# jeffersonfparil/poolgen

Hardware: NVIDIA B200
Metric: loci/sec for ols_iter (f64) (higher is better)
Workload: dtype f64

## Files before the change

poolgen_b200/csrc/pg_api.cu:

```cuda
#include <math.h>
#include <stdarg.h>
#include <stdio.h>
#include <stdlib.h>
#include <string.h>

#include <algorithm>
#include <new>

#include "pg_internal.h"
#include "pg_ptable.h"

namespace pg {
cudaError_t launch_scan_a2(const ScanParams &, int, cudaStream_t);
cudaError_t launch_scan_a3(const ScanParams &, int, cudaStream_t);
cudaError_t launch_scan_a4(const ScanParams &, int, cudaStream_t);
cudaError_t launch_scan_a5(const ScanParams &, int, cudaStream_t);
cudaError_t launch_scan_a6(const ScanParams &, int, cudaStream_t);

cudaError_t launch_scan(const ScanParams &p, int sm_count, cudaStream_t s) {
    switch (p.lay.A) {
        case 2: return launch_scan_a2(p, sm_count, s);
        case 3: return launch_scan_a3(p, sm_count, s);
        case 4: return launch_scan_a4(p, sm_count, s);
        case 5: return launch_scan_a5(p, sm_count, s);
// ... 163 lines not shown
    s->lay = pg::make_layout(n_pools, s->A_dev);
    s->n_slots = regression ? s->A_dev - 1 : 1;
    double S = 0.0;
    for (int i = 0; i < n_pools; i++) S = S + filter->pool_sizes[i];
    s->w_host.assign(s->lay.n_pad, 0.0);
    for (int i = 0; i < n_pools; i++) s->w_host[i] = filter->pool_sizes[i] / S;
    s->weighted = 0;
    for (int i = 1; i < n_pools; i++)
        if (s->w_host[i] != s->w_host[0]) s->weighted = 1;
    s->w_uniform = s->w_host[0];

    if (regression) {
        const int n = n_pools, np = s->lay.n_pad;
        s->yc_host.assign((size_t)k * np, 0.0);
        s->ysum.assign(k, 0.0);
        s->syy.assign(k, 0.0);
        s->ymean.assign(k, 0.0);
        for (int j = 0; j < k; j++) {
            double sum = 0.0;
            int n_valid = 0;
            for (int i = 0; i < n; i++) {
                const double v = phen[(size_t)i * k + j];
                if (v != v) {
                    s->y_has_nan = 1;
                    continue;
                }
                sum += v;
                n_valid++;
            }
            const double mean = n_valid ? sum / n_valid : 0.0;
            double s1 = 0.0, s2 = 0.0;
            for (int i = 0; i < n; i++) {
                const double c = phen[(size_t)i * k + j] - mean;
                s->yc_host[(size_t)j * np + i] = c;
                s1 += c;
                s2 += c * c;
            }
            s->ysum[j] = s1;
            s->ymean[j] = mean;
            s->syy[j] = s2 - s1 * s1 / n;
        }
        if (s->y_has_nan && (kind == PG_KIND_OLS || kind == PG_KIND_MLE)) {
            delete s;
            return fail(ctx, PG_ERR_UNSUPPORTED,
                        "pg_scan_open: missing phenotype values (the reference's ols_iter panics on them, "
                        "src/base/sync.rs:254-257)");
        }
        s->df = (kind != PG_KIND_CORR) ? (double)n - 1.0 : (double)n - 2.0;
        if (kind != PG_KIND_CORR && !(s->df > 0.0)) {
            delete s;
            return fail(ctx, PG_ERR_UNSUPPORTED, "pg_scan_open: ols_iter needs at least 2 pools");
        }
        s->ln_beta = s->df > 0.0 ? pg::statrs::ln_gamma(s->df / 2.0 + 0.5) - pg::statrs::ln_gamma(s->df / 2.0) - pg::statrs::ln_gamma(0.5) : 0.0;
        if ((size_t)2 * np * 8 > 96 * 1024) {
            delete s;
            return fail(ctx, PG_ERR_UNSUPPORTED, "pg_scan_open: %d pools exceed the shared-memory resident phenotype budget (6,144 pools)", n);
        }
        const char *pv_mode = getenv("PG_PVALUE");
        if (s->df > 0.0 && !(pv_mode && strcmp(pv_mode, "cf") == 0)) {
            pg::PTable tab = pg::build_ptable(s->df);
            if (tab.max_err < 2e-9) {
                cudaError_t et = s->d_ptab.reserve(tab.coef.size(), nullptr);
                if (et == cudaSuccess)
                    et = cudaMemcpy(s->d_ptab.get(), tab.coef.data(), tab.coef.size() * 8, cudaMemcpyHostToDevice);
                if (et != cudaSuccess) {
                    delete s;
                    return fail(ctx, PG_ERR_CUDA, "pg_scan_open: p-value table upload: %s", cudaGetErrorString(et));
                }
                s->ptab_M = tab.M;
                s->ptab_isd = tab.inv_sqrt_df;
                s->ptab_bits = tab.bits;
                s->ptab_t1 = tab.t_one;
                s->ptab_t0 = tab.t_zero;
                s->ptab_err = tab.max_err;
            }
        }
        cudaError_t e = s->d_yc.reserve(s->yc_host.size(), nullptr);
        if (e == cudaSuccess) e = cudaMemcpy(s->d_yc.get(), s->yc_host.data(), s->yc_host.size() * 8, cudaMemcpyHostToDevice);
        if (e != cudaSuccess) {
            delete s;
            return fail(ctx, PG_ERR_CUDA, "pg_scan_open: phenotype upload: %s", cudaGetErrorString(e));
        }
    }
    {
        cudaError_t e = s->d_w.reserve(s->w_host.size(), nullptr);
        if (e == cudaSuccess) e = cudaMemcpy(s->d_w.get(), s->w_host.data(), s->w_host.size() * 8, cudaMemcpyHostToDevice);
        if (e != cudaSuccess) {
            delete s;
            return fail(ctx, PG_ERR_CUDA, "pg_scan_open: weight upload: %s", cudaGetErrorString(e));
        }
    }
    if (kind == PG_KIND_MLE || gwalpha) {
        const int np = s->lay.n_pad;
        std::vector<double> raw((size_t)(gwalpha ? 2 : k) * np, 0.0);
        if (gwalpha) {
            for (int i = 0; i < n_pools; i++) {
                raw[i] = gw_bins[i];
                raw[(size_t)np + i] = gw_q[i];
            }
            s->gw_sig = gw_fmt[0 * 3 + 2];
            s->gw_min = gw_fmt[1 * 3 + 2];
            s->gw_max = gw_fmt[2 * 3 + 2];
            (void)gw_rows;
        } else {
            for (int j = 0; j < k; j++)
                for (int i = 0; i < n_pools; i++) raw[(size_t)j * np + i] = phen[(size_t)i * k + j];
        }
        cudaError_t e = s->d_yraw.reserve(raw.size(), nullptr);
        if (e == cudaSuccess) e = cudaMemcpy(s->d_yraw.get(), raw.data(), raw.size() * 8, cudaMemcpyHostToDevice);
        if (e != cudaSuccess) {
            delete s;
            return fail(ctx, PG_ERR_CUDA, "pg_scan_open: phenotype upload: %s", cudaGetErrorString(e));
        }
    }
    {
        cudaError_t e = cudaDeviceSynchronize();
        if (e != cudaSuccess) {
            delete s;
            return fail(ctx, PG_ERR_CUDA, "pg_scan_open: %s", cudaGetErrorString(e));
        }
    }
    *out = s;
    return PG_OK;
}

int pg_scan_close(pg_scan *s) {
    delete s;
    return PG_OK;
}

static bool is_nm(const pg_scan *s) { return s->kind == PG_KIND_MLE || s->kind == PG_KIND_GWALPHA_LS || s->kind == PG_KIND_GWALPHA_ML; }
static bool is_regression(const pg_scan *s) { return s->kind == PG_KIND_OLS || s->kind == PG_KIND_CORR || is_nm(s); }

int pg_batch_create(pg_scan *s, int64_t cap, pg_batch **out) {
    if (!s || !out || cap < 1 || cap > 0x7FFFFFFFLL) return fail(s ? s->ctx : nullptr, PG_ERR_ARG, "pg_batch_create: bad argument (1 <= capacity < 2^31 loci)");
    pg_ctx *ctx = s->ctx;
    *out = nullptr;
    PG_CUDA(ctx, cudaSetDevice(ctx->device));
    pg_batch *b = new (std::nothrow) pg_batch();
    if (!b) return fail(ctx, PG_ERR_ARG, "out of host memory");
    b->scan = s;
    b->cap = cap;
    cudaError_t e = cudaStreamCreateWithFlags(&b->stream, cudaStreamNonBlocking);
    if (e == cudaSuccess) e = cudaEventCreate(&b->ev0);
    if (e == cudaSuccess) e = cudaEventCreate(&b->ev1);
    if (e == cudaSuccess && is_regression(s)) {
        e = b->d_freq.reserve((size_t)cap * s->lay.freq_stride(), b->stream);
        if (e == cudaSuccess) e = b->d_depth.reserve((size_t)cap * s->lay.depth_stride(), b->stream);
        if (e == cudaSuccess) e = b->d_dmin.reserve((size_t)cap, b->stream);
        if (e == cudaSuccess) e = b->d_defer.reserve((size_t)cap + 1, b->stream);
        if (e == cudaSuccess) e = b->d_hint.reserve((size_t)cap, b->stream);
    }
    const size_t S = s->n_slots, K = s->k;
    if (e == cudaSuccess) e = b->d_meta.reserve((size_t)cap, b->stream);
    if (e == cudaSuccess) e = b->d_fmean.reserve((size_t)cap * S, b->stream);
    if (e == cudaSuccess) e = b->d_stats.reserve((size_t)cap * S * K * 4, b->stream);
    if (e != cudaSuccess) {
        delete b;
        return fail(ctx, PG_ERR_CUDA, "pg_batch_create(%lld loci): %s", (long long)cap, cudaGetErrorString(e));
    }
    *out = b;
    return PG_OK;
}

int pg_batch_destroy(pg_batch *b) {
    delete b;
    return PG_OK;
}

static pg::IngestOut ingest_out(pg_batch *b, int64_t first_locus) {
    pg_scan *s = b->scan;
    pg::IngestOut o;
    o.freq = b->d_freq.get() + (size_t)first_locus * s->lay.freq_stride();
    o.depth = b->d_depth.get() + (size_t)first_locus * s->lay.depth_stride();
    o.dmin = b->d_dmin.get() + first_locus;
    o.hint = b->d_hint.get() + first_locus;
    o.w = s->d_w.get();
    o.maf = s->maf;
    o.one_minus_maf = 1.00 - s->maf;
    o.min_depth_f = (double)s->min_depth;
    return o;
}

}

static int ensure_stage(pg_batch *b, size_t bytes) {
    PG_CUDA(b->scan->ctx, b->d_stage.reserve(bytes, b->stream));
    return PG_OK;
}

template <typename CT>
static int upload_counts_t(pg_batch *b, const CT *counts, int64_t n_loci) {
    if (!b || (!counts && n_loci > 0)) return PG_ERR_ARG;
    pg_scan *s = b->scan;
    pg_ctx *ctx = s->ctx;
    if (n_loci < 0 || n_loci > b->cap) return fail(ctx, PG_ERR_ARG, "upload: %lld loci > capacity %lld", (long long)n_loci, (long long)b->cap);
    PG_CUDA(ctx, cudaSetDevice(ctx->device));
    b->n_loci = n_loci;
    b->have_input = 1;
    if (n_loci == 0) return PG_OK;
    const size_t bytes = (size_t)n_loci * s->A_in * s->n * sizeof(CT);
    const bool reg = is_regression(s);
    const size_t wide_bytes = (size_t)b->cap * s->A_in * s->n * 4;
    int rc = ensure_stage(b, reg ? (size_t)b->cap * s->A_in * s->n * sizeof(CT) : wide_bytes + (sizeof(CT) == 4 ? 0 : bytes));
    if (rc) return rc;
    if (reg) {
        PG_CUDA(ctx, cudaMemcpyAsync(b->d_stage.get(), counts, bytes, cudaMemcpyHostToDevice, b->stream));
        if constexpr (sizeof(CT) == 4)
            PG_CUDA(ctx, pg::launch_ingest_u32((const uint32_t *)b->d_stage.get(), n_loci, s->n, s->A_in, s->drop_col, s->lay,
                                               ingest_out(b, 0), b->stream));
        else if constexpr (sizeof(CT) == 1)
            PG_CUDA(ctx, pg::launch_ingest_u8((const uint8_t *)b->d_stage.get(), n_loci, s->n, s->A_in, s->drop_col, s->lay,
                                              ingest_out(b, 0), b->stream));
        else
            PG_CUDA(ctx, pg::launch_ingest_u16((const uint16_t *)b->d_stage.get(), n_loci, s->n, s->A_in, s->drop_col, s->lay,
                                               ingest_out(b, 0), b->stream));
    } else if constexpr (sizeof(CT) == 4) {
        PG_CUDA(ctx, cudaMemcpyAsync(b->d_stage.get(), counts, bytes, cudaMemcpyHostToDevice, b->stream));
    } else {
        void *narrow = (char *)b->d_stage.get() + wide_bytes;
        PG_CUDA(ctx, cudaMemcpyAsync(narrow, counts, bytes, cudaMemcpyHostToDevice, b->stream));
        PG_CUDA(ctx, pg::launch_widen(narrow, (int)sizeof(CT), (uint32_t *)b->d_stage.get(), (size_t)n_loci * s->A_in * s->n,
                                      b->stream));
    }
    b->input_is_counts = 1;
    return PG_OK;
}

extern "C" {

int pg_batch_upload_counts(pg_batch *b, const uint32_t *counts, int64_t n_loci) {
    return upload_counts_t<uint32_t>(b, counts, n_loci);
}
int pg_batch_upload_counts_u16(pg_batch *b, const uint16_t *counts, int64_t n_loci) {
    return upload_counts_t<uint16_t>(b, counts, n_loci);
}
int pg_batch_upload_counts_u8(pg_batch *b, const uint8_t *counts, int64_t n_loci) {
    return upload_counts_t<uint8_t>(b, counts, n_loci);
}

int pg_batch_upload_freq(pg_batch *b, const double *freq, const uint32_t *depth, int64_t n_loci) {
    if (!b || ((!freq || !depth) && n_loci > 0)) return PG_ERR_ARG;
    pg_scan *s = b->scan;
    pg_ctx *ctx = s->ctx;
    if (!is_regression(s)) return fail(ctx, PG_ERR_UNSUPPORTED, "upload_freq: the table tests need counts");
    if (s->drop_col >= 0)
        return fail(ctx, PG_ERR_ARG, "upload_freq: the frequency matrix must not contain the N column when remove_ns is set");
    if (n_loci < 0 || n_loci > b->cap) return fail(ctx, PG_ERR_ARG, "upload: %lld loci > capacity %lld", (long long)n_loci, (long long)b->cap);
    PG_CUDA(ctx, cudaSetDevice(ctx->device));
    b->n_loci = n_loci;
    b->have_input = 1;
    if (n_loci == 0) return PG_OK;
    const size_t fbytes_cap = (size_t)b->cap * s->A_dev * s->n * 8, dbytes_cap = (size_t)b->cap * s->n * 4;
    int rc = ensure_stage(b, fbytes_cap + dbytes_cap);
    if (rc) return rc;
    double *sf = (double *)b->d_stage.get();
    uint32_t *sd = (uint32_t *)((char *)b->d_stage.get() + fbytes_cap);
    PG_CUDA(ctx, cudaMemcpyAsync(sf, freq, (size_t)n_loci * s->A_dev * s->n * 8, cudaMemcpyHostToDevice, b->stream));
    PG_CUDA(ctx, cudaMemcpyAsync(sd, depth, (size_t)n_loci * s->n * 4, cudaMemcpyHostToDevice, b->stream));
    PG_CUDA(ctx, pg::launch_ingest_freq(sf, sd, n_loci, s->n, s->lay, ingest_out(b, 0), b->stream));
    b->input_is_counts = 0;
    return PG_OK;
}

static int text_stage_a(pg_batch *b, const char *text, size_t n_bytes, size_t line_cap) {
    if (!b || (!text && n_bytes > 0)) return PG_ERR_ARG;
    pg_scan *s = b->scan;
    pg_ctx *ctx = s->ctx;
    if (s->A_in != 6) return fail(ctx, PG_ERR_ARG, "upload_sync_text: the scan must be opened with the six sync columns A:T:C:G:N:D");
    for (int j = 0; j < 6; j++)
        if (s->codes_in[j] != j) return fail(ctx, PG_ERR_ARG, "upload_sync_text: allele codes must be 0..5 in sync order");
    PG_CUDA(ctx, cudaSetDevice(ctx->device));
    b->n_loci = 0;
    b->have_input = 1;
    b->input_is_counts = 1;
    b->text_src = text;
    b->text_bytes = n_bytes;
    int rc = ensure_stage(b, (size_t)b->cap * 6 * s->n * 4);
    if (rc) return rc;
    const cudaError_t pe = pg::text_parse_async(&b->text, text, n_bytes, s->n, (uint32_t *)b->d_stage.get(), b->cap, line_cap,
                                                ctx->sm_count, b->stream);
    if (pe != cudaSuccess) {
        b->have_input = 0;
        b->n_loci = 0;
        return fail(ctx, PG_ERR_CUDA, "upload_sync_text: %s", cudaGetErrorString(pe));
    }
    return PG_OK;
}

static int text_stage_b(pg_batch *b, int64_t *n_loci_out) {
    pg_scan *s = b->scan;
    pg_ctx *ctx = s->ctx;
    if (n_loci_out) *n_loci_out = 0;
    cudaError_t ce = cudaSuccess;
    uint64_t at = 0;
    int64_t L = pg::text_parse_finish(&b->text, b->stream, &ce, &at);
    if (L == -5) {
        int rc = text_stage_a(b, b->text_src, b->text_bytes, (size_t)at + 1);
        if (rc) return rc;
        L = pg::text_parse_finish(&b->text, b->stream, &ce, &at);
    }
    if (L < 0) return pg::text_parse_fail(ctx, "upload_sync_text", L, ce, at, s->n, b->cap);
    b->n_loci = L;
    if (n_loci_out) *n_loci_out = L;
    if (L > 0 && is_regression(s))
        PG_CUDA(ctx, pg::launch_ingest_u32((const uint32_t *)b->d_stage.get(), L, s->n, s->A_in, s->drop_col, s->lay,
                                           ingest_out(b, 0), b->stream));
    return PG_OK;
}

int pg_batch_upload_sync_text(pg_batch *b, const char *text, size_t n_bytes, int64_t *n_loci_out) {
    if (n_loci_out) *n_loci_out = 0;
    int rc = text_stage_a(b, text, n_bytes, 0);
    if (rc) return rc;
    rc = text_stage_b(b, n_loci_out);
    if (rc) return rc;
    PG_CUDA(b->scan->ctx, cudaStreamSynchronize(b->stream));
    return PG_OK;
}

int pg_batch_text_labels(pg_batch *b, const uint64_t **line_offsets, const uint64_t **positions) {
    if (!b) return PG_ERR_ARG;
    if (!b->text.parsed) return fail(b->scan->ctx, PG_ERR_STATE, "pg_batch_text_labels before pg_batch_upload_sync_text");
    if (line_offsets) *line_offsets = b->text.h_out_offset.get();
    if (positions) *positions = b->text.h_out_pos.get();
    return PG_OK;
}

int pg_batch_synth(pg_batch *b, uint64_t seed, int64_t first_locus, int64_t n_loci) {
    if (!b) return PG_ERR_ARG;
    pg_scan *s = b->scan;
    pg_ctx *ctx = s->ctx;
    if (n_loci < 0 || n_loci > b->cap) return fail(ctx, PG_ERR_ARG, "synth: %lld loci > capacity %lld", (long long)n_loci, (long long)b->cap);
    PG_CUDA(ctx, cudaSetDevice(ctx->device));
    b->n_loci = n_loci;
    b->have_input = 1;
    if (n_loci == 0) return PG_OK;
    const size_t per_locus = (size_t)s->A_in * s->n * 4;
    if (!is_regression(s)) {
        int rc = ensure_stage(b, (size_t)b->cap * per_locus);
        if (rc) return rc;
        PG_CUDA(ctx, pg::launch_synth(seed, first_locus, n_loci, s->n, s->A_in, (uint32_t *)b->d_stage.get(), b->stream));
        b->input_is_counts = 1;
        return PG_OK;
    }
    int64_t slice = (int64_t)((size_t)256 << 20) / (int64_t)per_locus;
    if (slice < 1) slice = 1;
    if (slice > n_loci) slice = n_loci;
    if (b->d_stage.capacity() < (size_t)slice * per_locus) {
        int rc = ensure_stage(b, (size_t)slice * per_locus);
        if (rc) return rc;
    } else {
        slice = (int64_t)(b->d_stage.capacity() / per_locus);
        if (slice > n_loci) slice = n_loci;
    }
    for (int64_t l0 = 0; l0 < n_loci; l0 += slice) {
        const int64_t m = (n_loci - l0 < slice) ? n_loci - l0 : slice;
        PG_CUDA(ctx, pg::launch_synth(seed, first_locus + l0, m, s->n, s->A_in, (uint32_t *)b->d_stage.get(), b->stream));
        PG_CUDA(ctx, pg::launch_ingest_u32((const uint32_t *)b->d_stage.get(), m, s->n, s->A_in, s->drop_col, s->lay,
                                           ingest_out(b, l0), b->stream));
    }
    b->input_is_counts = 1;
    return PG_OK;
}

static int run_once(pg_batch *b, int *launches) {
    pg_scan *s = b->scan;
    pg_ctx *ctx = s->ctx;
    if (!b->have_input) return fail(ctx, PG_ERR_STATE, "pg_batch_run: no input uploaded");
    if (b->n_loci == 0) return PG_OK;
    if (is_regression(s)) {
        int kpass = pg::max_phen_per_pass(s->A_dev);
        {
            const int fit = (int)((size_t)(96 * 1024) / ((size_t)s->lay.n_pad * 8)) - (s->weighted ? 1 : 0);
            if (kpass > fit) kpass = fit < 1 ? 1 : fit;
        }
        static const int nbuf_env = getenv("PG_NBUF") ? atoi(getenv("PG_NBUF")) : 0;
        static const int warps_env = getenv("PG_WARPS") ? atoi(getenv("PG_WARPS")) : 0;
        static const int g_env = getenv("PG_G") ? atoi(getenv("PG_G")) : 0;
        static const int p_env = getenv("PG_P") ? atoi(getenv("PG_P")) : 0;
        if (is_nm(s)) kpass = 1;
        for (int base = 0; base < (is_nm(s) ? 1 : s->k); base += kpass) {
            pg::ScanParams p;
            memset(&p, 0, sizeof p);
            p.lay = s->lay;
            p.freq = b->d_freq.get();
            p.depth = b->d_depth.get();
            p.dmin = b->d_dmin.get();
            p.hint = b->d_hint.get();
            p.n_loci = b->n_loci;
            p.kind = is_nm(s) ? PG_KIND_OLS : s->kind;
            p.filter_only = is_nm(s) ? 1 : 0;
            p.weighted = s->weighted;
            p.maf = s->maf;
            p.one_minus_maf = 1.00 - s->maf;
            p.max_miss = s->max_miss;
            p.min_depth_f = (double)s->min_depth;
            p.w_uniform = s->w_uniform;
            p.df = s->df;
            p.inv_df = 1.0 / s->df;
            p.inv_n = 1.0 / (double)s->n;
            p.inv_nm2 = 1.0 / ((double)s->n - 2.0);
            p.ln_beta = s->ln_beta;
            p.ptab = s->d_ptab.get();
            p.ptab_isd = s->ptab_isd;
            p.ptab_bits = s->ptab_bits;
            p.ptab_t1 = s->ptab_t1;
            p.ptab_t0 = s->ptab_t0;
            p.ptab_M = s->ptab_M;
            p.K = std::min(kpass, s->k - base);
            p.y_has_nan = s->y_has_nan;
            p.yc = s->d_yc.get() + (size_t)base * s->lay.n_pad;
            p.w = s->d_w.get();
            for (int j = 0; j < p.K; j++) {
                p.ysum[j] = s->ysum[base + j];
                p.syy[j] = s->syy[base + j];
                p.ymean[j] = s->ymean[base + j];
            }
            for (int j = 0; j < s->A_dev; j++) p.codes[j] = s->codes_dev[j];
            p.meta = b->d_meta.get();
            p.freq_mean = b->d_fmean.get();
            p.stats = b->d_stats.get();
            p.defer_list = b->d_defer.get();
            p.defer_count = reinterpret_cast<uint32_t *>(b->d_defer.get() + b->cap);
            p.k_total = s->k;
            p.phen_base = base;
            p.write_meta = base == 0;
            p.nbuf_override = nbuf_env;
            p.warps_override = warps_env;
            p.g_override = g_env;
            p.p_override = p_env;
            PG_CUDA(ctx, pg::launch_scan(p, ctx->sm_count, b->stream));
            if (launches) (*launches) += 2;
        }
        if (is_nm(s)) {
            pg::NmParams q;
            memset(&q, 0, sizeof q);
            q.lay = s->lay;
            q.freq = b->d_freq.get();
            q.depth = b->d_depth.get();
            q.n_loci = b->n_loci;
            q.kind = s->kind;
            q.k = s->k;
            q.yraw = s->d_yraw.get();
            q.gw_sig = s->gw_sig;
            q.gw_min = s->gw_min;
            q.gw_max = s->gw_max;
            q.df = s->df;
            q.ln_beta = s->ln_beta;
            q.ptab = s->d_ptab.get();
            q.ptab_isd = s->ptab_isd;
            q.ptab_bits = s->ptab_bits;
            q.ptab_t1 = s->ptab_t1;
            q.ptab_t0 = s->ptab_t0;
            q.ptab_M = s->ptab_M;
            for (int j = 0; j < s->A_dev; j++) q.codes[j] = s->codes_dev[j];
            q.meta = b->d_meta.get();
            q.stats = b->d_stats.get();
            PG_CUDA(ctx, pg::launch_nm(q, ctx->sm_count, b->stream));
            if (launches) (*launches)++;
        }
    } else {
        pg::TableParams p;
        memset(&p, 0, sizeof p);
        p.counts = (const uint32_t *)b->d_stage.get();
        p.n_loci = b->n_loci;
        p.n = s->n;
        p.A_in = s->A_in;
        p.kind = s->kind;
        p.drop_col = s->drop_col;
        p.maf = s->maf;
        p.one_minus_maf = 1.00 - s->maf;
        p.max_miss = s->max_miss;
        p.min_depth_f = (double)s->min_depth;
        p.w = s->d_w.get();
        for (int j = 0; j < s->A_in; j++) p.codes[j] = s->codes_in[j];
        p.meta = b->d_meta.get();
        p.stats = b->d_stats.get();
        PG_CUDA(ctx, pg::launch_tables(p, ctx->sm_count, b->stream));
        if (launches) (*launches)++;
    }
    return PG_OK;
}

int pg_batch_run(pg_batch *b) {
    if (!b) return PG_ERR_ARG;
    PG_CUDA(b->scan->ctx, cudaSetDevice(b->scan->ctx->device));
    return run_once(b, nullptr);
}

int pg_batch_time_runs(pg_batch *b, int iters, float *ms_total, int *n_launches) {
    if (!b || iters < 1 || !ms_total) return PG_ERR_ARG;
    pg_ctx *ctx = b->scan->ctx;
    PG_CUDA(ctx, cudaSetDevice(ctx->device));
    int launches = 0;
    PG_CUDA(ctx, cudaStreamSynchronize(b->stream));
    PG_CUDA(ctx, cudaEventRecord(b->ev0, b->stream));
    for (int i = 0; i < iters; i++) {
        int rc = run_once(b, &launches);
        if (rc) return rc;
    }
    PG_CUDA(ctx, cudaEventRecord(b->ev1, b->stream));
    PG_CUDA(ctx, cudaEventSynchronize(b->ev1));
    PG_CUDA(ctx, cudaEventElapsedTime(ms_total, b->ev0, b->ev1));
    if (n_launches) *n_launches = launches;
    static const bool report = getenv("PG_REPORT_DEFER") != nullptr;
    if (report && b->d_defer.get() && is_regression(b->scan)) {
        uint32_t count = 0;
        PG_CUDA(ctx, cudaMemcpy(&count, b->d_defer.get() + b->cap, 4, cudaMemcpyDeviceToHost));
        std::vector<uint64_t> list(count);
        if (count) PG_CUDA(ctx, cudaMemcpy(list.data(), b->d_defer.get(), (size_t)count * 8, cudaMemcpyDeviceToHost));
        uint32_t h[8] = {0, 0, 0, 0, 0, 0, 0, 0};
        for (uint64_t e : list) {
            const unsigned why = (unsigned)(e >> 56);
            if (why & 1u) h[0]++;
            if (why & 2u) h[1]++;
            if (why & 4u) h[2]++;
            if (why & 8u) h[3]++;
            if ((why >> 4) >= 1 && (why >> 4) <= 4) h[3 + (why >> 4)]++;
        }
        fprintf(stderr, "[pg] deferred %u of %lld loci (last phenotype pass): threshold %u, removed-with-reads %u, no coverage %u, "
                        "NaN under hint %u, redo ols %u, redo corr %u, corr NaN %u, tie %u\n",
                count, (long long)b->n_loci, h[0], h[1], h[2], h[3], h[4], h[5], h[6], h[7]);
    }
    return PG_OK;
}

int pg_batch_bytes(pg_batch *b, size_t *input_bytes, size_t *result_bytes) {
    if (!b) return PG_ERR_ARG;
    pg_scan *s = b->scan;
    const size_t L = (size_t)b->n_loci;
    if (input_bytes)
        *input_bytes = is_regression(s) ? L * (s->lay.freq_stride() * 8 + 4)
                                        : L * (size_t)s->A_in * s->n * 4;
    if (result_bytes) *result_bytes = L * (8 + (size_t)s->n_slots * 8 + (size_t)s->n_slots * s->k * 32);
    return PG_OK;
}

int pg_batch_download(pg_batch *b) {
    if (!b) return PG_ERR_ARG;
    pg_scan *s = b->scan;
    pg_ctx *ctx = s->ctx;
    PG_CUDA(ctx, cudaSetDevice(ctx->device));
    const size_t S = s->n_slots, K = s->k;
    PG_CUDA(ctx, b->h_meta.reserve((size_t)b->cap, b->stream));
    PG_CUDA(ctx, b->h_fmean.reserve((size_t)b->cap * S, b->stream));
    PG_CUDA(ctx, b->h_stats.reserve((size_t)b->cap * S * K * 4, b->stream));
    const size_t L = (size_t)b->n_loci;
    if (L == 0) return PG_OK;
    PG_CUDA(ctx, cudaMemcpyAsync(b->h_meta.get(), b->d_meta.get(), L * 8, cudaMemcpyDeviceToHost, b->stream));
    PG_CUDA(ctx, cudaMemcpyAsync(b->h_fmean.get(), b->d_fmean.get(), L * S * 8, cudaMemcpyDeviceToHost, b->stream));
    PG_CUDA(ctx, cudaMemcpyAsync(b->h_stats.get(), b->d_stats.get(), L * S * K * 32, cudaMemcpyDeviceToHost, b->stream));
    return PG_OK;
}

int pg_batch_sync(pg_batch *b) {
    if (!b) return PG_ERR_ARG;
    PG_CUDA(b->scan->ctx, cudaStreamSynchronize(b->stream));
    return PG_OK;
}

int pg_batch_results(pg_batch *b, pg_results *out) {
    if (!b || !out) return PG_ERR_ARG;
    if (b->n_loci > 0 && !(b->h_meta.get() && b->h_fmean.get() && b->h_stats.get())) return fail(b->scan->ctx, PG_ERR_STATE, "pg_batch_results before pg_batch_download");
    out->n_loci = b->n_loci;
    out->n_slots = b->scan->n_slots;
    out->n_phen = b->scan->k;
    out->meta = b->h_meta.get();
    out->freq_mean = b->h_fmean.get();
    out->stats = b->h_stats.get();
    return PG_OK;
}

int pg_scan_stream_begin(pg_scan *s, int64_t max_loci) {
    if (!s || max_loci < 1) return PG_ERR_ARG;
    for (int i = 0; i < PG_STREAM_DEPTH; i++) {
        delete s->slabs[i];
        s->slabs[i] = nullptr;
        int rc = pg_batch_create(s, max_loci, &s->slabs[i]);
        if (rc) return rc;
    }
    s->slab_cap = max_loci;
    s->next_slab = 0;
    return PG_OK;
}

static int submit_common(pg_scan *s, int *ticket, pg_batch **b) {
    if (!s || !ticket) return PG_ERR_ARG;
    if (!s->slabs[0]) return fail(s->ctx, PG_ERR_STATE, "pg_scan_submit before pg_scan_stream_begin");
    *ticket = s->next_slab;
    *b = s->slabs[s->next_slab];
    s->next_slab = (s->next_slab + 1) % PG_STREAM_DEPTH;
    return pg_batch_sync(*b);
}

int pg_scan_submit_counts(pg_scan *s, const uint32_t *counts, int64_t n_loci, int *ticket) {
    pg_batch *b = nullptr;
    int rc = submit_common(s, ticket, &b);
    if (rc) return rc;
    if ((rc = pg_batch_upload_counts(b, counts, n_loci))) return rc;
    if ((rc = pg_batch_run(b))) return rc;
    return pg_batch_download(b);
}
int pg_scan_submit_counts_u16(pg_scan *s, const uint16_t *counts, int64_t n_loci, int *ticket) {
    pg_batch *b = nullptr;
    int rc = submit_common(s, ticket, &b);
    if (rc) return rc;
    if ((rc = pg_batch_upload_counts_u16(b, counts, n_loci))) return rc;
    if ((rc = pg_batch_run(b))) return rc;
    return pg_batch_download(b);
}
int pg_scan_submit_counts_u8(pg_scan *s, const uint8_t *counts, int64_t n_loci, int *ticket) {
    pg_batch *b = nullptr;
    int rc = submit_common(s, ticket, &b);
    if (rc) return rc;
    if ((rc = pg_batch_upload_counts_u8(b, counts, n_loci))) return rc;
// ... 46 lines not shown
```

poolgen_b200/csrc/pg_device.cuh:

```cuda
#pragma once
#include <cuda_runtime.h>
#include <stdint.h>

namespace pg {

#define PG_FULL_MASK 0xffffffffu
constexpr double kEps = 2.220446049250313e-16;

__device__ __forceinline__ uint32_t smem_u32(const void *p) {
    return (uint32_t)__cvta_generic_to_shared(p);
}

__device__ __forceinline__ void mbar_init(uint64_t *bar, uint32_t count) {
    asm volatile("mbarrier.init.shared::cta.b64 [%0], %1;" ::"r"(smem_u32(bar)), "r"(count) : "memory");
}
__device__ __forceinline__ void fence_mbar_init() {
    asm volatile("fence.mbarrier_init.release.cluster;" ::: "memory");
}
__device__ __forceinline__ void fence_proxy_async() {
    asm volatile("fence.proxy.async.shared::cta;" ::: "memory");
}
__device__ __forceinline__ void mbar_expect_tx(uint64_t *bar, uint32_t bytes) {
    asm volatile("mbarrier.arrive.expect_tx.shared::cta.b64 _, [%0], %1;" ::"r"(smem_u32(bar)), "r"(bytes)
                 : "memory");
}
__device__ __forceinline__ void bulk_g2s(void *dst_smem, const void *src_gmem, uint32_t bytes, uint64_t *bar) {
    asm volatile(
        "cp.async.bulk.shared::cluster.global.mbarrier::complete_tx::bytes [%0], [%1], %2, [%3];" ::"r"(
            smem_u32(dst_smem)),
        "l"(src_gmem), "r"(bytes), "r"(smem_u32(bar))
        : "memory");
}
__device__ __forceinline__ void mbar_wait(uint64_t *bar, uint32_t parity) {
    asm volatile(
        "{\n"
        ".reg .pred P1;\n"
        "LAB_WAIT:\n"
        "mbarrier.try_wait.parity.shared::cta.b64 P1, [%0], %1;\n"
        "@P1 bra DONE;\n"
        "bra LAB_WAIT;\n"
        "DONE:\n"
        "}\n" ::"r"(smem_u32(bar)),
        "r"(parity)
        : "memory");
}

__device__ __forceinline__ void warp_reduce32(double (&v)[32], int lane) {
#pragma unroll
    for (int off = 16; off >= 1; off >>= 1) {
        const bool upper = (lane & off) != 0;
#pragma unroll
        for (int i = 0; i < off; i++) {
            const double a = v[i], b = v[i + off];
            const double send = upper ? a : b;
            const double keep = upper ? b : a;
            v[i] = keep + __shfl_xor_sync(PG_FULL_MASK, send, off);
        }
    }
}

__device__ __forceinline__ double warp_sum_fixed(double v) {
#pragma unroll
    for (int off = 16; off >= 1; off >>= 1) v += __shfl_xor_sync(PG_FULL_MASK, v, off);
    return v;
}

__device__ __forceinline__ double beta_reg_dev(double a, double b, double x, double ln_beta) {
    double bt;
    if (fabs(x) < 1e-10 || fabs(x - 1.0) <= 4.0 * 1.1102230246251565e-16) {
        bt = 0.0;
    } else {
        bt = exp(ln_beta + a * log(x) + b * log(1.0 - x));
    }
    const bool symm = x >= (a + 1.0) / (a + b + 2.0);
    const double eps = 1.1102230246251565e-16;
    const double fpmin = 2.2250738585072014e-308 / eps;
    if (symm) {
        const double sw = a;
        x = 1.0 - x;
        a = b;
        b = sw;
    }
    const double qab = a + b, qap = a + 1.0, qam = a - 1.0;
    double c = 1.0;
    double d = 1.0 - qab * x / qap;
    if (fabs(d) < fpmin) d = fpmin;
    d = 1.0 / d;
    double h = d;
    for (int mi = 1; mi < 141; mi++) {
        const double m = (double)mi;
        const double m2 = m * 2.0;
        double aa = m * (b - m) * x / ((qam + m2) * (a + m2));
        d = 1.0 + aa * d;
        if (fabs(d) < fpmin) d = fpmin;
        c = 1.0 + aa / c;
        if (fabs(c) < fpmin) c = fpmin;
        d = 1.0 / d;
        h = h * d * c;
        aa = -(a + m) * (qab + m) * x / ((a + m2) * (qap + m2));
        d = 1.0 + aa * d;
        if (fabs(d) < fpmin) d = fpmin;
        c = 1.0 + aa / c;
        if (fabs(c) < fpmin) c = fpmin;
        d = 1.0 / d;
        const double del = d * c;
        h *= del;
        if (fabs(del - 1.0) <= eps) break;
    }
    return symm ? 1.0 - bt * h / a : bt * h / a;
}

static __device__ __noinline__ double student_two_sided(double t_abs, double df, double ln_beta) {
    if (isinf(df)) return 2.0 * (1.0 - 0.5 * erfc(-t_abs / sqrt(2.0)));
    const double h = df / __dadd_rn(df, __dmul_rn(t_abs, t_abs));
    const double ib = 0.5 * beta_reg_dev(df / 2.0, 0.5, h, ln_beta);
    const double cdf = t_abs <= 0.0 ? ib : 1.0 - ib;
    return 2.0 * (1.0 - cdf);
}

struct PTableDev {
    const double4 *coef;
    double inv_sqrt_df, bits;
    double t_one, t_zero;
    int M;
};
__device__ __forceinline__ int ptab_locate(double w, int B, double &s) {
    const int hi = __double2hiint(w);
// ... 92 lines not shown
```

poolgen_b200/csrc/pg_ingest.cu:

```cuda
#include <stdlib.h>

#include "pg_device.cuh"
#include "pg_internal.h"

namespace pg {

struct HintParams {
    double maf, one_minus_maf, min_depth_f;
    int enabled;
};
__device__ __forceinline__ unsigned ambiguous_alleles(const double *q, int A, int n, const HintParams &hp) {
    const double tol_rel = 4.0 * ((double)n + 8.0) * kEps;
    unsigned amb = 0;
    for (int j = 0; j < A; j++) {
        const double tl = tol_rel * fmax(fabs(q[j]), 1.0);
        if (fabs(q[j] - hp.maf) <= tl || fabs(q[j] - hp.one_minus_maf) <= tl) amb |= 1u << j;
    }
    return amb;
}

__device__ __forceinline__ uint8_t locus_hint(const double *q, int A, int n, uint32_t dm, const HintParams &hp,
                                              unsigned exact) {
    if (!hp.enabled) return 0;
    const double tol_rel = 4.0 * ((double)n + 8.0) * kEps;
    unsigned kept = 0;
    bool removed_with_reads = false, safe = true;
    for (int j = 0; j < A; j++) {
        const double tl = tol_rel * fmax(fabs(q[j]), 1.0);
        if (!((exact >> j) & 1u) && (fabs(q[j] - hp.maf) <= tl || fabs(q[j] - hp.one_minus_maf) <= tl)) safe = false;
        if (!((q[j] < hp.maf) | (q[j] > hp.one_minus_maf)))
            kept |= 1u << j;
        else if (q[j] > 0.0)
            removed_with_reads = true;
    }
    const bool depth_ok = dm != 0u && !((double)dm < hp.min_depth_f);
    return (safe && depth_ok && removed_with_reads && __popc(kept) >= 2) ? (uint8_t)(0x80u | kept) : (uint8_t)0;
}

template <typename RowFn>
__device__ __forceinline__ void ingest_loci(int64_t n_loci, const Layout &lay, int P, const double *freq,
                                            const double *__restrict__ w, uint32_t *__restrict__ dmin,
                                            uint8_t *__restrict__ hint, const HintParams &hp, RowFn &&row) {
    const int lane = threadIdx.x & 31, sub = lane / P, q0 = lane % P, lpw = 32 / P;
    const int64_t gw = ((int64_t)blockIdx.x * blockDim.x + threadIdx.x) >> 5;
    const int64_t nw = ((int64_t)gridDim.x * blockDim.x) >> 5;
    for (int64_t l0 = gw * lpw; l0 < n_loci; l0 += nw * lpw) {
        const int64_t locus = l0 + sub;
        double q[PG_MAX_ALLELES] = {0, 0, 0, 0, 0, 0};
        uint32_t dm = 0xFFFFFFFFu;
        if (locus < n_loci)
            for (int i = q0; i < lay.n_pad; i += P) row(locus, i, q, dm);
        for (int off = P >> 1; off >= 1; off >>= 1) {
            for (int j = 0; j < lay.A; j++) q[j] += __shfl_xor_sync(0xFFFFFFFFu, q[j], off);
            dm = min(dm, __shfl_xor_sync(0xFFFFFFFFu, dm, off));
        }
        unsigned amb = (hp.enabled && locus < n_loci && dm != 0u) ? ambiguous_alleles(q, lay.A, lay.n, hp) : 0u;
        if (__any_sync(0xFFFFFFFFu, amb != 0u)) {
            __syncwarp();
            const double *fl = freq + (size_t)(locus < n_loci ? locus : 0) * lay.freq_stride();
            for (int j = 0; j < lay.A; j++) {
                if (!__any_sync(0xFFFFFFFFu, (amb >> j) & 1u)) continue;
                double e = 0.0;
                for (int r0 = 0; r0 < lay.n; r0 += P) {
                    const int i = r0 + q0;
                    double term = 0.0;
                    if (i < lay.n && locus < n_loci) {
                        const double f = __ldcg(fl + lay.freq_off(i, j));
                        term = (f != f) ? 0.0 : __dmul_rn(f, w[i]);
                    }
                    const int m = min(P, lay.n - r0);
                    for (int t = 0; t < m; t++) e = __dadd_rn(e, __shfl_sync(0xFFFFFFFFu, term, t, P));
                }
                if ((amb >> j) & 1u) q[j] = e;
            }
        }
        if (locus < n_loci && q0 == 0) {
            dmin[locus] = dm;
            hint[locus] = locus_hint(q, lay.A, lay.n, dm, hp, amb);
        }
    }
}

template <typename CT>
__global__ void __launch_bounds__(256) ingest_counts_kernel(const CT *__restrict__ counts, int64_t n_loci, int n,
                                                            int A_in, int drop_col, Layout lay, int P,
                                                            double *__restrict__ freq, uint32_t *__restrict__ depth,
                                                            uint32_t *__restrict__ dmin, uint8_t *__restrict__ hint,
                                                            const double *__restrict__ w, HintParams hp) {
    ingest_loci(n_loci, lay, P, freq, w, dmin, hint, hp, [&](int64_t locus, int i, double *q, uint32_t &dm) {
        double *fl = freq + (size_t)locus * lay.freq_stride();
        if (i >= n) {
            for (int j = 0; j < lay.A; j++) fl[lay.freq_off(i, j)] = 0.0;
            depth[(size_t)locus * lay.n_pad + i] = 0xFFFFFFFFu;
            return;
        }
        const CT *cl = counts + (size_t)locus * A_in * n + i;
        uint32_t c[PG_MAX_ALLELES];
        uint64_t d = 0;
        int jj = 0;
        for (int j = 0; j < A_in; j++) {
            if (j == drop_col) continue;
            c[jj] = (uint32_t)cl[(size_t)j * n];
            d += c[jj];
            jj++;
        }
        if (d > 0xFFFFFFFEull) d = 0xFFFFFFFEull;
        const double dd = (double)d, wi = w[i];
        const double rd = __drcp_rn(dd);
        for (int j = 0; j < lay.A; j++) {
            const double cj = (double)c[j];
            const double q0 = __dmul_rn(cj, rd);
            const double f = (d == 0) ? nan("") : __fma_rn(__fma_rn(-q0, dd, cj), rd, q0);
            fl[lay.freq_off(i, j)] = f;
            if (d != 0) q[j] = fma(f, wi, q[j]);
        }
        depth[(size_t)locus * lay.n_pad + i] = (uint32_t)d;
        dm = min(dm, (uint32_t)d);
    });
}

__global__ void __launch_bounds__(256) ingest_freq_kernel(const double *__restrict__ fin, const uint32_t *__restrict__ din,
                                                          int64_t n_loci, int n, Layout lay, int P,
                                                          double *__restrict__ freq, uint32_t *__restrict__ depth,
                                                          uint32_t *__restrict__ dmin, uint8_t *__restrict__ hint,
                                                          const double *__restrict__ w, HintParams hp) {
    ingest_loci(n_loci, lay, P, freq, w, dmin, hint, hp, [&](int64_t locus, int i, double *q, uint32_t &dm) {
        double *fl = freq + (size_t)locus * lay.freq_stride();
        const bool pad = i >= n;
        for (int j = 0; j < lay.A; j++) {
            const double f = pad ? 0.0 : fin[((size_t)locus * lay.A + j) * n + i];
            fl[lay.freq_off(i, j)] = f;
            if (!pad && f == f) q[j] = fma(f, w[i], q[j]);
        }
        const uint32_t d = pad ? 0xFFFFFFFFu : din[(size_t)locus * n + i];
        depth[(size_t)locus * lay.n_pad + i] = d;
        dm = min(dm, d);
    });
}

__global__ void __launch_bounds__(256) synth_kernel(uint64_t seed, int64_t first_locus, int64_t n_loci, int n,
                                                    int A_in, uint32_t *__restrict__ counts) {
    const int64_t total = n_loci * n;
    for (int64_t idx = (int64_t)blockIdx.x * blockDim.x + threadIdx.x; idx < total;
         idx += (int64_t)gridDim.x * blockDim.x) {
        const int64_t l = idx / n;
        const int i = (int)(idx - l * n);
        uint32_t c[PG_MAX_ALLELES];
        synth_counts(seed, first_locus + l, i, A_in, c);
        for (int a = 0; a < A_in; a++) counts[((size_t)l * A_in + a) * n + i] = c[a];
    }
}

static int grid_for(int64_t total) {
    int64_t b = (total + 255) / 256;
    const int64_t cap = 148 * 16;
    return (int)(b < 1 ? 1 : (b > cap ? cap : b));
}

static int ingest_group(const Layout &lay) {
    int P = 32;
    while (P > 1 && (P >> 1) >= lay.n_pad) P >>= 1;
    return P;
}
static HintParams hint_params(const IngestOut &o) {
    static const bool no_hint = getenv("PG_NOHINT") != nullptr;
    HintParams hp;
    hp.maf = o.maf;
    hp.one_minus_maf = o.one_minus_maf;
    hp.min_depth_f = o.min_depth_f;
    hp.enabled = no_hint ? 0 : 1;
    return hp;
}
template <typename CT>
static cudaError_t launch_ingest_t(const CT *counts, int64_t n_loci, int n, int A_in, int drop_col, const Layout &lay,
                                   const IngestOut &o, cudaStream_t s) {
    if (n_loci <= 0) return cudaSuccess;
    const int P = ingest_group(lay);
    ingest_counts_kernel<CT><<<grid_for(n_loci * P), 256, 0, s>>>(counts, n_loci, n, A_in, drop_col, lay, P, o.freq,
                                                                 o.depth, o.dmin, o.hint, o.w, hint_params(o));
    return cudaGetLastError();
}
cudaError_t launch_ingest_u32(const uint32_t *counts, int64_t n_loci, int n, int A_in, int drop_col, const Layout &lay,
                              const IngestOut &o, cudaStream_t s) {
    return launch_ingest_t<uint32_t>(counts, n_loci, n, A_in, drop_col, lay, o, s);
}
cudaError_t launch_ingest_u16(const uint16_t *counts, int64_t n_loci, int n, int A_in, int drop_col, const Layout &lay,
                              const IngestOut &o, cudaStream_t s) {
    return launch_ingest_t<uint16_t>(counts, n_loci, n, A_in, drop_col, lay, o, s);
}
cudaError_t launch_ingest_u8(const uint8_t *counts, int64_t n_loci, int n, int A_in, int drop_col, const Layout &lay,
                             const IngestOut &o, cudaStream_t s) {
    return launch_ingest_t<uint8_t>(counts, n_loci, n, A_in, drop_col, lay, o, s);
}
cudaError_t launch_ingest_freq(const double *fin, const uint32_t *din, int64_t n_loci, int n, const Layout &lay,
                               const IngestOut &o, cudaStream_t s) {
    if (n_loci <= 0) return cudaSuccess;
    const int P = ingest_group(lay);
    ingest_freq_kernel<<<grid_for(n_loci * P), 256, 0, s>>>(fin, din, n_loci, n, lay, P, o.freq, o.depth, o.dmin, o.hint,
                                                            o.w, hint_params(o));
    return cudaGetLastError();
}
template <typename CT>
__global__ void __launch_bounds__(256) widen_kernel(const CT *__restrict__ src, uint32_t *__restrict__ dst, size_t count) {
    for (size_t i = (size_t)blockIdx.x * blockDim.x + threadIdx.x; i < count; i += (size_t)gridDim.x * blockDim.x)
        dst[i] = (uint32_t)src[i];
}
cudaError_t launch_widen(const void *src, int elem_bytes, uint32_t *dst, size_t count, cudaStream_t s) {
    if (count == 0) return cudaSuccess;
    if (elem_bytes == 1)
        widen_kernel<uint8_t><<<grid_for((int64_t)count), 256, 0, s>>>((const uint8_t *)src, dst, count);
    else if (elem_bytes == 2)
        widen_kernel<uint16_t><<<grid_for((int64_t)count), 256, 0, s>>>((const uint16_t *)src, dst, count);
    else
        return cudaErrorInvalidValue;
    return cudaGetLastError();
}
cudaError_t launch_synth(uint64_t seed, int64_t first_locus, int64_t n_loci, int n, int A_in, uint32_t *counts,
                         cudaStream_t s) {
    if (n_loci <= 0) return cudaSuccess;
    synth_kernel<<<grid_for(n_loci * n), 256, 0, s>>>(seed, first_locus, n_loci, n, A_in, counts);
    return cudaGetLastError();
}

}
```

poolgen_b200/csrc/pg_internal.h:

```cpp
#pragma once
#include <cuda_runtime.h>
#include <stdint.h>
#include <string>
#include <utility>
#include <vector>

#include "poolgen_cuda.h"
#include "pg_synth.h"

namespace pg {

__host__ __device__ constexpr int chunk_rows(int A) { return A <= 2 ? 256 : (A == 3 ? 192 : 128); }

struct Layout {
    int n;
    int n_pad;
    int A;
    int rc;
    int n_chunks;
    int rc_last;
    __host__ __device__ size_t freq_stride() const { return (size_t)A * n_pad; }
    __host__ __device__ size_t depth_stride() const { return (size_t)n_pad; }
    __host__ __device__ size_t freq_off(int i, int j) const {
        int c = i / rc, r = i - c * rc;
        int rcc = (c == n_chunks - 1) ? rc_last : rc;
        return (size_t)c * A * rc + (size_t)j * rcc + r;
    }
};

inline Layout make_layout(int n, int A) {
    Layout l;
    l.n = n;
    l.n_pad = (n + 3) & ~3;
    l.A = A;
    const int cr = chunk_rows(A);
    if (l.n_pad <= cr) {
        l.rc = l.n_pad;
        l.n_chunks = 1;
        l.rc_last = l.n_pad;
    } else {
        l.rc = cr;
        l.n_chunks = (l.n_pad + cr - 1) / cr;
        l.rc_last = l.n_pad - (l.n_chunks - 1) * cr;
    }
    return l;
}

constexpr int kMaxPhenPerPass = 4;
inline int max_phen_per_pass(int A) { return A <= 4 ? 4 : (A == 5 ? 3 : 2); }

struct ScanParams {
    Layout lay;
    const double *freq;
    const uint32_t *depth;
    const uint32_t *dmin;
    const uint8_t *hint;
    int64_t n_loci;
    int kind;
    int weighted;
    double maf, one_minus_maf, max_miss;
    double min_depth_f;
    double w_uniform;
    double df;
    double inv_df;
    double inv_n, inv_nm2;
    double ln_beta;
    const void *ptab;
    double ptab_isd, ptab_bits, ptab_t1, ptab_t0;
    int ptab_M;
    const double *yc;
    const double *w;
    double ysum[kMaxPhenPerPass];
    double syy[kMaxPhenPerPass];
    double ymean[kMaxPhenPerPass];
    int y_has_nan;
    int filter_only;
    uint8_t codes[8];
    uint64_t *meta;
    double *freq_mean;
    double *stats;
    uint64_t *defer_list;
    uint32_t *defer_count;
    int k_total, phen_base, K;
    int write_meta;
    uint32_t common_bytes, warp_bytes, stage_bytes;
    int nbuf, block_loci;
    int nbuf_override, warps_override, g_override, p_override;
};

struct TableParams {
    const uint32_t *counts;
    int64_t n_loci;
    int n, A_in;
    int kind;
    int drop_col;
    double maf, one_minus_maf, max_miss, min_depth_f;
    const double *w;
    uint8_t codes[8];
    uint64_t *meta;
    double *stats;
};

struct NmParams {
    Layout lay;
    const double *freq;
    const uint32_t *depth;
    int64_t n_loci;
    int kind;
    int k;
    const double *yraw;
    double gw_sig, gw_min, gw_max;
    double df, ln_beta;
    const void *ptab;
    double ptab_isd, ptab_bits, ptab_t1, ptab_t0;
    int ptab_M;
    uint8_t codes[8];
    uint64_t *meta;
    double *stats;
};
cudaError_t launch_nm(const NmParams &p, int sm_count, cudaStream_t s);

constexpr int kKinMleMaxM = 13;
struct KinMleParams {
    const double *G;
    int64_t P;
    int n, ldg, m, k;
    const double *Z;
    const double *fix;
    double df, ln_beta;
    const void *ptab;
    double ptab_isd, ptab_bits, ptab_t1, ptab_t0;
    int ptab_M;
    double *beta, *var, *pval;
};
cudaError_t launch_kin_mle(const KinMleParams &p, int sm_count, cudaStream_t s);

cudaError_t launch_scan(const ScanParams &p, int sm_count, cudaStream_t s);
cudaError_t launch_tables(const TableParams &p, int sm_count, cudaStream_t s);
struct IngestOut {
    double *freq;
    uint32_t *depth;
    uint32_t *dmin;
    uint8_t *hint;
    const double *w;
    double maf, one_minus_maf, min_depth_f;
};
cudaError_t launch_ingest_u32(const uint32_t *counts, int64_t n_loci, int n, int A_in, int drop_col, const Layout &lay,
                              const IngestOut &o, cudaStream_t s);
cudaError_t launch_ingest_u16(const uint16_t *counts, int64_t n_loci, int n, int A_in, int drop_col, const Layout &lay,
                              const IngestOut &o, cudaStream_t s);
cudaError_t launch_ingest_u8(const uint8_t *counts, int64_t n_loci, int n, int A_in, int drop_col, const Layout &lay,
                             const IngestOut &o, cudaStream_t s);
cudaError_t launch_ingest_freq(const double *freq_in, const uint32_t *depth_in, int64_t n_loci, int n, const Layout &lay,
                               const IngestOut &o, cudaStream_t s);
cudaError_t launch_synth(uint64_t seed, int64_t first_locus, int64_t n_loci, int n, int A_in,
                         uint32_t *counts, cudaStream_t s);
cudaError_t launch_widen(const void *src, int elem_bytes, uint32_t *dst, size_t count, cudaStream_t s);

template <typename T, bool Pinned>
class Buffer {
  public:
    Buffer() = default;
    Buffer(const Buffer &) = delete;
    Buffer &operator=(const Buffer &) = delete;
    Buffer(Buffer &&o) noexcept : p_(o.p_), cap_(o.cap_) { o.p_ = nullptr, o.cap_ = 0; }
    Buffer &operator=(Buffer &&o) noexcept {
        std::swap(p_, o.p_);
        std::swap(cap_, o.cap_);
        return *this;
    }
    ~Buffer() { release(); }

    cudaError_t reserve(size_t count, cudaStream_t stream) {
        if (cap_ >= count) return cudaSuccess;
        cudaError_t e = p_ ? cudaStreamSynchronize(stream) : cudaSuccess;
        release();
        if (e != cudaSuccess) return e;
        void *q = nullptr;
        if constexpr (Pinned)
            e = cudaHostAlloc(&q, count * sizeof(T), cudaHostAllocDefault);
        else
            e = cudaMalloc(&q, count * sizeof(T));
        if (e != cudaSuccess) {
            (void)cudaGetLastError();
            return e;
        }
        p_ = static_cast<T *>(q);
        cap_ = count;
        return cudaSuccess;
    }
    T *get() const { return p_; }
    size_t capacity() const { return cap_; }

  private:
    void release() {
        if constexpr (Pinned) {
            if (p_) cudaFreeHost(p_);
        } else {
            cudaFree(p_);
        }
        p_ = nullptr;
        cap_ = 0;
    }
    T *p_ = nullptr;
    size_t cap_ = 0;
};
template <typename T>
using DeviceBuffer = Buffer<T, false>;
template <typename T>
using PinnedBuffer = Buffer<T, true>;

struct TextScratch {
    DeviceBuffer<char> d_text;
    DeviceBuffer<uint32_t> d_sep;
    DeviceBuffer<uint64_t> d_tok_blk;
    DeviceBuffer<uint32_t> d_nl, d_first, d_grp;
    DeviceBuffer<uint8_t> d_keep;
    DeviceBuffer<uint64_t> d_line_pos;
    DeviceBuffer<uint32_t> d_info;
    PinnedBuffer<uint32_t> h_info;
    DeviceBuffer<uint8_t> d_tmp;
    DeviceBuffer<uint64_t> d_out_offset, d_out_pos;
    PinnedBuffer<uint64_t> h_out_offset, h_out_pos;
    cudaEvent_t parsed = nullptr;
    bool pending = false;
    int64_t max_loci = 0;
    ~TextScratch();
};
cudaError_t text_parse_async(TextScratch *t, const char *text, size_t n_bytes, int n_pools, uint32_t *d_counts,
                             int64_t max_loci, size_t line_cap, int sm_count, cudaStream_t s);
int64_t text_parse_finish(TextScratch *t, cudaStream_t s, cudaError_t *cuda_err, uint64_t *err_offset);

}

struct pg_ctx {
    int device = 0;
    int sm_count = 0;
    int cc_major = 0, cc_minor = 0;
    size_t total_mem = 0;
};

namespace pg {
int fail(pg_ctx *ctx, int code, const char *fmt, ...);
int text_parse_fail(pg_ctx *ctx, const char *who, int64_t status, cudaError_t cuda_err, uint64_t err_offset,
                    int n_pools, int64_t cap);
}

#define PG_CUDA(ctx, call)                                                                              \
    do {                                                                                                \
        cudaError_t e_ = (call);                                                                        \
        if (e_ != cudaSuccess)                                                                          \
            return pg::fail((ctx), PG_ERR_CUDA, "%s failed: %s (%s:%d)", #call, cudaGetErrorString(e_), \
                            __FILE__, __LINE__);                                                        \
    } while (0)

struct pg_scan {
    pg_ctx *ctx = nullptr;
    int kind = 0;
    int n = 0, A_in = 0, A_dev = 0, k = 0;
    int drop_col = -1;
    uint8_t codes_in[8] = {0};
    uint8_t codes_dev[8] = {0};
    pg::Layout lay;
    int remove_ns = 1;
    uint64_t min_depth = 1;
    double maf = 0, max_miss = 0;
    int weighted = 0;
    double w_uniform = 0;
    std::vector<double> w_host;
    std::vector<double> yc_host;
    std::vector<double> ysum, syy, ymean;
    int y_has_nan = 0;
    double df = 0, ln_beta = 0;
    pg::DeviceBuffer<double> d_yc;
    pg::DeviceBuffer<double> d_w;
    pg::DeviceBuffer<double> d_yraw;
    double gw_sig = 0, gw_min = 0, gw_max = 0;
    pg::DeviceBuffer<double> d_ptab;
    double ptab_isd = 0, ptab_bits = 0, ptab_err = 0, ptab_t1 = 0, ptab_t0 = 0;
    int ptab_M = 0;
    int n_slots = 0;
    pg_batch *slabs[PG_STREAM_DEPTH] = {nullptr, nullptr, nullptr};
    int next_slab = 0;
    int64_t slab_cap = 0;
    ~pg_scan();
};

struct pg_batch {
    pg_scan *scan = nullptr;
    int64_t cap = 0, n_loci = 0;
    cudaStream_t stream = nullptr;
    cudaEvent_t ev0 = nullptr, ev1 = nullptr;
    pg::DeviceBuffer<double> d_freq;
    pg::DeviceBuffer<uint32_t> d_depth;
    pg::DeviceBuffer<uint32_t> d_dmin;
    pg::DeviceBuffer<uint64_t> d_defer;
    pg::DeviceBuffer<uint8_t> d_hint;
    pg::DeviceBuffer<uint8_t> d_stage;
    pg::DeviceBuffer<uint64_t> d_meta;
    pg::DeviceBuffer<double> d_fmean;
    pg::DeviceBuffer<double> d_stats;
    pg::PinnedBuffer<uint64_t> h_meta;
    pg::PinnedBuffer<double> h_fmean;
    pg::PinnedBuffer<double> h_stats;
    int have_input = 0;
    int input_is_counts = 0;
    pg::TextScratch text;
    const char *text_src = nullptr;
    size_t text_bytes = 0;
    ~pg_batch();
};
```

poolgen_b200/csrc/pg_nm.cu:

```cuda
#include "pg_device.cuh"
#include "pg_internal.h"

namespace pg {

constexpr int kNmMaxD = 8;

__device__ __forceinline__ double bound_logit(double x, double lo, double hi) { return lo + ((hi - lo) / (1.00 + exp(-x))); }

template <int MAXD, typename Cost>
__device__ void nelder_mead(const Cost &cost, int d, double h, int max_iters, double *best) {
    double v[MAXD + 1][MAXD], c[MAXD + 1];
    const int nv = d + 1;
    for (int i = 0; i < nv; i++)
        for (int j = 0; j < d; j++) v[i][j] = (i == j) ? h + 0.5 : h;
    for (int i = 0; i < nv; i++) c[i] = cost(v[i]);
    auto sort = [&]() {
        for (int a = 1; a < nv; a++) {
            const double ca = c[a];
            double va[MAXD];
            for (int j = 0; j < d; j++) va[j] = v[a][j];
            int b = a - 1;
            while (b >= 0 && ca < c[b]) {
                c[b + 1] = c[b];
                for (int j = 0; j < d; j++) v[b + 1][j] = v[b][j];
// ... 87 lines not shown
    };
    enum { kInit, kReflect, kExpand, kOutside, kInside, kShrink, kDone };
    int state = kInit, idx = 0, it = 0;
    double x0[MAXD], xr[MAXD], xt[MAXD], fr = 0.0;
    auto next_iteration = [&]() {
        double c0 = 0.0;
        for (int i = 0; i < nv; i++) c0 = c0 + c[i];
        c0 = c0 / (double)nv;
        double ss = 0.0;
        for (int i = 0; i < nv; i++) ss = ss + (c[i] - c0) * (c[i] - c0);
        const double sd = sqrt(1.0 / ((double)nv - 1.0) * ss);
        if (sd < kEps || it >= max_iters) {
            state = kDone;
            return;
        }
        it++;
        for (int j = 0; j < d; j++) x0[j] = v[0][j];
        for (int i = 1; i < nv - 1; i++)
            for (int j = 0; j < d; j++) x0[j] = x0[j] + v[i][j];
        const double inv = 1.0 / (double)(nv - 1);
        for (int j = 0; j < d; j++) x0[j] = x0[j] * inv;
        for (int j = 0; j < d; j++) xr[j] = x0[j] + (x0[j] - v[nv - 1][j]) * 1.0;
        state = kReflect;
    };
    auto accept = [&](const double *x, double f) {
        for (int j = 0; j < d; j++) v[nv - 1][j] = x[j];
        c[nv - 1] = f;
        sort();
        next_iteration();
    };
    auto begin_shrink = [&]() {
        for (int i = 1; i < nv; i++)
            for (int j = 0; j < d; j++) v[i][j] = v[0][j] + (v[i][j] - v[0][j]) * 0.5;
        idx = 1;
        state = kShrink;
    };
    while (state != kDone) {
        const double *x = (state == kInit || state == kShrink) ? v[idx] : (state == kReflect ? xr : xt);
        const double f = cost(x);
        if (state == kInit || state == kShrink) {
            c[idx] = f;
            if (++idx == nv) {
                sort();
                next_iteration();
            }
        } else if (state == kReflect) {
            fr = f;
            if (fr < c[nv - 2] && fr >= c[0]) {
                accept(xr, fr);
            } else if (fr < c[0]) {
                for (int j = 0; j < d; j++) xt[j] = x0[j] + (xr[j] - x0[j]) * 2.0;
                state = kExpand;
            } else if (fr >= c[nv - 2]) {
                if (fr < c[nv - 1]) {
                    for (int j = 0; j < d; j++) xt[j] = x0[j] + (xr[j] - x0[j]) * 0.5;
                    state = kOutside;
                } else {
                    for (int j = 0; j < d; j++) xt[j] = x0[j] + (v[nv - 1][j] - x0[j]) * 0.5;
                    state = kInside;
                }
            } else {
                begin_shrink();
            }
        } else if (state == kExpand) {
            if (f < fr)
                accept(xt, f);
            else
                accept(xr, fr);
        } else if (state == kOutside) {
            if (f <= fr)
                accept(xt, f);
            else
                begin_shrink();
        } else {
            if (f < c[nv - 1])
                accept(xt, f);
            else
                begin_shrink();
        }
    }
    for (int j = 0; j < d; j++) best[j] = v[0][j];
}

__device__ __forceinline__ void renorm_generic(const NmParams &p, const double *fl, const uint32_t *dl, int i, unsigned kept,
                                               double *F) {
    const int A = p.lay.A;
    const uint32_t d = dl[i];
    double c[PG_MAX_ALLELES], dk = 0.0;
    for (int j = 0; j < A; j++) {
        c[j] = (d == 0u) ? 0.0 : rint(fl[p.lay.freq_off(i, j)] * (double)d);
        if ((kept >> j) & 1u) dk += c[j];
    }
    for (int j = 0; j < A; j++) F[j] = ((kept >> j) & 1u) ? ((dk == 0.0) ? nan("") : c[j] / dk) : 0.0;
}

__device__ __forceinline__ int col_of_code(const NmParams &p, unsigned code) {
    for (int j = 0; j < p.lay.A; j++)
        if (p.codes[j] == code) return j;
    return 0;
}

constexpr int kMlePhen = 4;
__host__ __device__ inline int mle_mom_stride(int k) { return 20 + (k < kMlePhen ? k : kMlePhen) * 7; }
constexpr int kMleWarps = 4;

__global__ void __launch_bounds__(kMleWarps * 32) mle_kernel(const NmParams p) {
    extern __shared__ __align__(16) double mle_sm[];
    const int lane = threadIdx.x & 31, wib = threadIdx.x >> 5;
    const int stride = mle_mom_stride(p.k);
    double *mom = mle_sm + (size_t)wib * 32 * stride;
    const int64_t warp = (int64_t)blockIdx.x * kMleWarps + wib;
    const int64_t nwarps = (int64_t)gridDim.x * kMleWarps;
    const int n = p.lay.n, n_pad = p.lay.n_pad, S = p.lay.A - 1, k = p.k;
    const PTableDev ptab = {reinterpret_cast<const double4 *>(p.ptab), p.ptab_isd, p.ptab_bits, p.ptab_t1, p.ptab_t0, p.ptab_M};
    const int64_t n_blocks = (p.n_loci + 31) / 32;
    for (int64_t blk = warp; blk < n_blocks; blk += nwarps) {
        const int64_t l0 = blk * 32;
        const int cnt = (int)min((int64_t)32, p.n_loci - l0);
        const uint64_t mv = (lane < cnt) ? p.meta[l0 + lane] : 0ull;
        const bool act = (mv & 0xffu) == PG_LOCUS_OK;
        const int m = (int)((mv >> 8) & 0xffu);
        unsigned colw = 0, kept = 0;
        if (act) {
            for (int s = 0; s < m; s++) {
                const int c = col_of_code(p, (unsigned)((mv >> (16 + 8 * s)) & 0xffu));
                colw |= (unsigned)c << (4 * s);
                kept |= 1u << c;
            }
            kept |= 1u << col_of_code(p, (unsigned)((mv >> (16 + 8 * m)) & 0xffu));
        }
        for (int g = 0; g < cnt; g++) {
            if (!__shfl_sync(PG_FULL_MASK, (int)act, g)) continue;
            const int mg = __shfl_sync(PG_FULL_MASK, m, g);
            const unsigned cg = __shfl_sync(PG_FULL_MASK, colw, g), kg = __shfl_sync(PG_FULL_MASK, kept, g);
            const double *fl = p.freq + (size_t)(l0 + g) * p.lay.freq_stride();
            const uint32_t *dl = p.depth + (size_t)(l0 + g) * p.lay.depth_stride();
            double sx[PG_MAX_SLOTS], lo[PG_MAX_SLOTS], hi[PG_MAX_SLOTS];
            for (int a = 0; a < PG_MAX_SLOTS; a++) sx[a] = 0.0, lo[a] = INFINITY, hi[a] = -INFINITY;
            for (int i = lane; i < n; i += 32) {
                double F[PG_MAX_ALLELES];
                renorm_generic(p, fl, dl, i, kg, F);
                for (int a = 0; a < mg; a++) {
                    const double f = F[(cg >> (4 * a)) & 0xfu];
                    sx[a] += f;
                    lo[a] = fmin(lo[a], f);
                    hi[a] = fmax(hi[a], f);
                }
            }
            double xb[PG_MAX_SLOTS];
            for (int a = 0; a < PG_MAX_SLOTS; a++) {
                if (a >= mg) {
                    xb[a] = 0.0;
                    continue;
                }
                double l = lo[a], h = hi[a];
#pragma unroll
                for (int off = 16; off >= 1; off >>= 1) {
                    l = fmin(l, __shfl_xor_sync(PG_FULL_MASK, l, off));
                    h = fmax(h, __shfl_xor_sync(PG_FULL_MASK, h, off));
                }
                const double mean = warp_sum_fixed(sx[a]) / (double)n;
                xb[a] = (l == h && mean == mean) ? l : mean;
            }
            double sxx[15];
            for (int e = 0; e < 15; e++) sxx[e] = 0.0;
            for (int i = lane; i < n; i += 32) {
                double F[PG_MAX_ALLELES];
                renorm_generic(p, fl, dl, i, kg, F);
                for (int a = 0; a < mg; a++)
                    for (int b = 0; b <= a; b++)
                        sxx[a * (a + 1) / 2 + b] = fma(F[(cg >> (4 * a)) & 0xfu] - xb[a], F[(cg >> (4 * b)) & 0xfu] - xb[b], sxx[a * (a + 1) / 2 + b]);
            }
            for (int e = 0; e < 15; e++) sxx[e] = (e < mg * (mg + 1) / 2) ? warp_sum_fixed(sxx[e]) : 0.0;
            if (lane == 0) {
                double *mo = mom + (size_t)g * stride;
                for (int a = 0; a < PG_MAX_SLOTS; a++) mo[a] = xb[a];
                for (int e = 0; e < 15; e++) mo[5 + e] = sxx[e];
            }
        }
        __syncwarp();
        double xbar[PG_MAX_SLOTS], Sxx[PG_MAX_SLOTS][PG_MAX_SLOTS];
        {
            const double *mo = mom + (size_t)lane * stride;
            for (int a = 0; a < PG_MAX_SLOTS; a++) xbar[a] = act ? mo[a] : 0.0;
            for (int a = 0; a < PG_MAX_SLOTS; a++)
                for (int b = 0; b <= a; b++) Sxx[a][b] = Sxx[b][a] = act ? mo[5 + a * (a + 1) / 2 + b] : 0.0;
        }
        int xc[PG_MAX_SLOTS + 1], pw = m + 1;
        for (int c = 0; c <= PG_MAX_SLOTS; c++) xc[c] = c;
        bool panic = false;
        if (act && pw != 2) {
            long i = 1;
            while (i < pw && !panic) {
                long j = i + 1;
                while (j < pw) {
                    if (i < 0) {
                        panic = true;
                        break;
                    }
                    double cor = nan("");
                    if (xc[i] >= 1 && xc[j] >= 1) {
                        const int a = xc[i] - 1, b = xc[j] - 1;
                        const double r = Sxx[a][b] / (sqrt(Sxx[a][a]) * sqrt(Sxx[b][b]));
                        cor = round(r * 1e7) / 1e7;
                    }
                    if (fabs(cor) >= 0.99) {
                        for (int c = (int)j; c + 1 < pw; c++) xc[c] = xc[c + 1];
                        pw -= 1;
                        i -= 1;
                        j -= 1;
                    }
                    j += 1;
                }
                i += 1;
            }
        }
        int status = !act ? (int)(mv & 0xffu) : (panic ? PG_LOCUS_PANIC : PG_LOCUS_OK);
        if (act && status == PG_LOCUS_OK && n < pw) status = PG_LOCUS_UNSUPPORTED;
        const int q = pw - 1;
        double dgi[PG_MAX_SLOTS + 1];
        for (int c = 0; c <= PG_MAX_SLOTS; c++) dgi[c] = 0.0;
        if (act && status == PG_LOCUS_OK) {
            double M[PG_MAX_SLOTS][2 * PG_MAX_SLOTS];
            for (int a = 0; a < q; a++)
                for (int b = 0; b < q; b++) {
                    M[a][b] = Sxx[xc[a + 1] - 1][xc[b + 1] - 1];
                    M[a][q + b] = a == b ? 1.0 : 0.0;
                }
            for (int c = 0; c < q && status == PG_LOCUS_OK; c++) {
                int pr = c;
                for (int r = c + 1; r < q; r++)
                    if (fabs(M[r][c]) > fabs(M[pr][c])) pr = r;
                if (!(fabs(M[pr][c]) > 0.0)) {
                    status = PG_LOCUS_FAILED;
                    break;
                }
                for (int e = 0; e < 2 * q; e++) {
                    const double tmp = M[c][e];
                    M[c][e] = M[pr][e];
                    M[pr][e] = tmp;
                }
                const double piv = 1.0 / M[c][c];
                for (int e = 0; e < 2 * q; e++) M[c][e] *= piv;
                for (int r = 0; r < q; r++) {
                    if (r == c) continue;
                    const double f = M[r][c];
                    for (int e = 0; e < 2 * q; e++) M[r][e] -= f * M[c][e];
                }
            }
            if (status == PG_LOCUS_OK) {
                double quad = 0.0;
                for (int a = 0; a < q; a++)
                    for (int b = 0; b < q; b++) quad += xbar[xc[a + 1] - 1] * M[a][q + b] * xbar[xc[b + 1] - 1];
                dgi[0] = 1.0 / (double)n + quad;
                for (int a = 0; a < q; a++) dgi[1 + a] = M[a][q + a];
            }
        }
        for (int j0 = 0; j0 < k; j0 += kMlePhen) {
            const int jn = min(kMlePhen, k - j0);
            __syncwarp();
            for (int g = 0; g < cnt; g++) {
                if (!__shfl_sync(PG_FULL_MASK, (int)act, g)) continue;
                const int mg = __shfl_sync(PG_FULL_MASK, m, g);
                const unsigned cg = __shfl_sync(PG_FULL_MASK, colw, g), kg = __shfl_sync(PG_FULL_MASK, kept, g);
                const double *fl = p.freq + (size_t)(l0 + g) * p.lay.freq_stride();
                const uint32_t *dl = p.depth + (size_t)(l0 + g) * p.lay.depth_stride();
                const double *mo = mom + (size_t)g * stride;
                double xb[PG_MAX_SLOTS];
                for (int a = 0; a < PG_MAX_SLOTS; a++) xb[a] = mo[a];
                for (int jj = 0; jj < jn; jj++) {
                    const double *y = p.yraw + (size_t)(j0 + jj) * n_pad;
                    double sy = 0.0;
                    for (int i = lane; i < n; i += 32) sy += y[i];
                    const double ybar = warp_sum_fixed(sy) / (double)n;
                    double syy = 0.0, sxy[PG_MAX_SLOTS];
                    for (int a = 0; a < PG_MAX_SLOTS; a++) sxy[a] = 0.0;
                    for (int i = lane; i < n; i += 32) {
                        double F[PG_MAX_ALLELES];
                        renorm_generic(p, fl, dl, i, kg, F);
                        const double dy = y[i] - ybar;
                        syy = fma(dy, dy, syy);
                        for (int a = 0; a < mg; a++) sxy[a] = fma(F[(cg >> (4 * a)) & 0xfu] - xb[a], dy, sxy[a]);
                    }
                    syy = warp_sum_fixed(syy);
                    for (int a = 0; a < PG_MAX_SLOTS; a++) sxy[a] = (a < mg) ? warp_sum_fixed(sxy[a]) : 0.0;
                    if (lane == 0) {
                        double *o = mom + (size_t)g * stride + 20 + jj * 7;
                        o[0] = ybar;
                        o[1] = syy;
                        for (int a = 0; a < PG_MAX_SLOTS; a++) o[2 + a] = sxy[a];
                    }
                }
            }
            __syncwarp();
            if (lane < cnt && (act || true)) {
                for (int jj = 0; jj < jn; jj++) {
                    const int j = j0 + jj;
                    const double *mo = mom + (size_t)lane * stride + 20 + jj * 7;
                    const double ybar_l = mo[0], syy_l = mo[1];
                    double sxy_l[PG_MAX_SLOTS];
                    for (int a = 0; a < PG_MAX_SLOTS; a++) sxy_l[a] = mo[2 + a];
                    double b[PG_MAX_SLOTS + 1], vb[PG_MAX_SLOTS + 1];
                    for (int c = 0; c <= PG_MAX_SLOTS; c++) b[c] = vb[c] = 0.0;
                    if (act && status == PG_LOCUS_OK) {
                        const double nn = (double)n;
                        auto cost = [&](const double *par) {
                            const double s2 = bound_logit(par[0], kEps, 1e9);
                            double quad = 0.0, lin = 0.0, off = ybar_l - par[1];
                            for (int a = 0; a < q; a++) {
                                const int ia = xc[a + 1] - 1;
                                lin += par[2 + a] * sxy_l[ia];
                                off -= xbar[ia] * par[2 + a];
                                for (int c = 0; c < q; c++) quad += par[2 + a] * Sxx[ia][xc[c + 1] - 1] * par[2 + c];
                            }
                            const double rss = (syy_l - 2.0 * lin + quad) + nn * off * off;
                            return (nn / 2.00) * log(2.00 * 3.14159265358979323846264338327950288 * s2) + (1.00 / s2) * rss;
                        };
                        double par[kNmMaxD];
                        nelder_mead<kNmMaxD>(cost, pw + 1, 1.0, 1000, par);
                        const double ve = bound_logit(par[0], kEps, 1e9);
                        for (int c = 0; c < pw; c++) {
                            b[c] = par[1 + c];
                            vb[c] = ve * dgi[c];
                        }
                    }
                    for (int s = 0; s < S; s++) {
                        double o0 = nan(""), o1 = nan(""), o2 = nan(""), o3 = nan("");
                        if (status == PG_LOCUS_OK && s < m) {
                            const int c = s + 1;
                            const bool filled = c < pw;
                            o0 = filled ? b[c] : 0.0;
                            o1 = filled ? vb[c] : 0.0;
                            if (filled) {
                                o2 = o0 / o1;
                                if (isinf(o2))
                                    o3 = 0.0;
                                else if (o2 != o2)
                                    o3 = 1.0;
                                else
                                    o3 = p.ptab ? student_two_sided_tab(fabs(o2), p.df, ptab) : student_two_sided(fabs(o2), p.df, p.ln_beta);
                            } else {
                                o3 = 0.0;
                            }
                        }
                        double *o = p.stats + (((size_t)(l0 + lane) * S + s) * k + j) * 4;
                        o[0] = o0, o[1] = o1, o[2] = o2, o[3] = o3;
                    }
                }
            }
        }
        if (act && status != PG_LOCUS_OK) p.meta[l0 + lane] = (mv & ~0xffull) | (uint64_t)status;
        __syncwarp();
    }
}

constexpr int kGwMaxPools = 64;

__device__ double nd_sum(const double *xs, int len) {
    double acc = 0.0, p0 = 0, p1 = 0, p2 = 0, p3 = 0, p4 = 0, p5 = 0, p6 = 0, p7 = 0;
    while (len >= 8) {
        p0 = p0 + xs[0], p1 = p1 + xs[1], p2 = p2 + xs[2], p3 = p3 + xs[3];
        p4 = p4 + xs[4], p5 = p5 + xs[5], p6 = p6 + xs[6], p7 = p7 + xs[7];
        xs += 8;
        len -= 8;
    }
    acc = acc + (p0 + p4);
    acc = acc + (p1 + p5);
    acc = acc + (p2 + p6);
    acc = acc + (p3 + p7);
    for (int i = 0; i < len && i < 7; i++) acc = acc + xs[i];
    return acc;
}

__device__ __forceinline__ double beta_cdf_dev(double a, double b, double lnb, double x) {
    if (x < 0.0) return 0.0;
    if (x >= 1.0) return 1.0;
    if (fabs(a - 1.0) <= 4.0 * 1.1102230246251565e-16 && fabs(b - 1.0) <= 4.0 * 1.1102230246251565e-16) return x;
    return beta_reg_dev(a, b, x, lnb);
}

__global__ void __launch_bounds__(128) gwalpha_kernel(const NmParams p) {
    const int S = p.lay.A - 1, n = p.lay.n, n_pad = p.lay.n_pad;
    const int64_t total = p.n_loci * S;
    const double *bins = p.yraw, *q = p.yraw + n_pad;
    for (int64_t item = (int64_t)blockIdx.x * blockDim.x + threadIdx.x; item < total;
         item += (int64_t)gridDim.x * blockDim.x) {
        const int64_t locus = item / S;
        const int s = (int)(item - locus * S);
        const uint64_t mv = p.meta[locus];
        double *o = p.stats + ((size_t)locus * S + s) * 4;
        const int m = (int)((mv >> 8) & 0xffu);
        if ((mv & 0xffu) != PG_LOCUS_OK || s >= m) {
            o[0] = o[1] = o[2] = o[3] = nan("");
            continue;
        }
        unsigned kept = 0;
        for (int a = 0; a <= m; a++) kept |= 1u << col_of_code(p, (unsigned)((mv >> (16 + 8 * a)) & 0xffu));
        const int cj = col_of_code(p, (unsigned)((mv >> (16 + 8 * s)) & 0xffu));
        const double *fl = p.freq + (size_t)locus * p.lay.freq_stride();
        const uint32_t *dl = p.depth + (size_t)locus * p.lay.depth_stride();
        double fa[kGwMaxPools], qp[kGwMaxPools], pa[kGwMaxPools], pb[kGwMaxPools], pa0[kGwMaxPools], pb0[kGwMaxPools];
        double p_a = 0.0;
        for (int i = 0; i < n; i++) {
            double F[PG_MAX_ALLELES];
            renorm_generic(p, fl, dl, i, kept, F);
            fa[i] = F[cj];
        }
        if (m == 1) {
            double prod[kGwMaxPools];
            double s0 = 0.0, ps[8] = {0, 0, 0, 0, 0, 0, 0, 0};
            int len = n, at = 0;
            while (len >= 8) {
                for (int e = 0; e < 8; e++) ps[e] = ps[e] + fa[at + e] * bins[at + e];
                at += 8;
                len -= 8;
            }
            s0 = s0 + (ps[0] + ps[4]);
            s0 = s0 + (ps[1] + ps[5]);
            s0 = s0 + (ps[2] + ps[6]);
            s0 = s0 + (ps[3] + ps[7]);
            for (int i = 0; i < len && i < 7; i++) s0 = s0 + fa[at + i] * bins[at + i];
            p_a = s0;
            (void)prod;
        } else {
            for (int i = 0; i < n; i++) p_a += fa[i] * bins[i];
        }
        qp[0] = 0.0;
        for (int i = 1; i < n; i++) qp[i] = (q[i] - p.gw_min) / (p.gw_max - p.gw_min);
        {
            double ba[kGwMaxPools], bb[kGwMaxPools];
            for (int i = 0; i < n; i++) {
                ba[i] = (fa[i]) * bins[i] / (p_a);
                bb[i] = (1.0 - fa[i]) * bins[i] / (1.0 - p_a);
            }
            pa[0] = ba[0];
            pb[0] = bb[0];
            for (int i = 1; i < n; i++) {
                pa[i] = nd_sum(ba, i + 1);
                pb[i] = nd_sum(bb, i + 1);
            }
        }
        pa0[0] = pb0[0] = 0.0;
        for (int i = 0; i < n - 1; i++) {
            pa0[i + 1] = pa[i];
            pb0[i + 1] = pb[i];
        }
        const bool ml = p.kind == PG_KIND_GWALPHA_ML;
        auto cost = [&](const double *par) {
            double sh[4];
            for (int e = 0; e < 4; e++) sh[e] = bound_logit(par[e], kEps, 10.00);
            const double lna = ln_gamma_dev(sh[0] + sh[1]) - ln_gamma_dev(sh[0]) - ln_gamma_dev(sh[1]);
            const double lnb = ln_gamma_dev(sh[2] + sh[3]) - ln_gamma_dev(sh[2]) - ln_gamma_dev(sh[3]);
            double ra = 0.0, rb = 0.0;
            if (!ml) {
                for (int i = 0; i < n; i++) {
                    const double da = pa[i] - beta_cdf_dev(sh[0], sh[1], lna, qp[i]);
                    const double db = pb[i] - beta_cdf_dev(sh[2], sh[3], lnb, qp[i]);
                    ra += da * da;
                    rb += db * db;
                }
                return ra + rb;
            }
            double lo_a = beta_cdf_dev(sh[0], sh[1], lna, pa0[0]), lo_b = beta_cdf_dev(sh[2], sh[3], lnb, pb0[0]);
            for (int i = 0; i < n; i++) {
                const double hi_a = beta_cdf_dev(sh[0], sh[1], lna, pa[i]), hi_b = beta_cdf_dev(sh[2], sh[3], lnb, pb[i]);
                double da = hi_a - lo_a;
                double db = hi_b - lo_b;
                lo_a = hi_a;
                lo_b = hi_b;
                if (da < kEps) da = kEps;
                if (db < kEps) db = kEps;
                ra += log10(da);
                rb += log10(db);
            }
            return -ra - rb;
        };
        double par[kNmMaxD];
        nelder_mead_one_site<kNmMaxD>(cost, 4, 1.0, 1000, par);
        double sol[4];
        for (int e = 0; e < 4; e++) sol[e] = bound_logit(par[e], kEps, 10.00);
        const double a_mu = p.gw_min + (p.gw_max - p.gw_min) * (sol[0] / (sol[0] + sol[1]));
        const double b_mu = p.gw_min + (p.gw_max - p.gw_min) * (sol[2] / (sol[2] + sol[3]));
        const double alpha = (2.00 * sqrt(p_a * (1.0 - p_a))) * (a_mu - b_mu) / p.gw_sig;
        o[0] = alpha;
        o[1] = p_a;
        o[2] = nan("");
        o[3] = nan("");
    }
// ... 142 lines not shown
```

poolgen_b200/csrc/pg_scan.cuh:

```cuda
#pragma once
#include "pg_device.cuh"
#include "pg_internal.h"

namespace pg {

constexpr int kScanWarps = 12;
constexpr int kRedPitch = 33;

template <int A, int K, bool W>
struct Acc {
    static constexpr int S0 = 0;
    static constexpr int P0 = S0 + A;
    static constexpr int C0 = P0 + A * (A + 1) / 2;
    static constexpr int Q0 = C0 + A * K;
    static constexpr int N = Q0 + (W ? A : 0);
    static constexpr int NP = N | 1;
    __host__ __device__ static constexpr int tri(int j, int l) {
        return P0 + j * A - j * (j - 1) / 2 + (l - j);
    }
};

template <int A, int K, bool W, bool NANAWARE>
__device__ __forceinline__ void accum_row(double (&acc)[Acc<A, K, W>::N], const double (&f)[A], const double (&y)[K],
                                          double w) {
    using AC = Acc<A, K, W>;
#pragma unroll
    for (int j = 0; j < A; j++) {
        if (NANAWARE)
            acc[AC::S0 + j] += (f[j] != f[j]) ? 0.0 : f[j];
        else
            acc[AC::S0 + j] += f[j];
    }
#pragma unroll
    for (int j = 0; j < A; j++)
#pragma unroll
        for (int l = j; l < A; l++) acc[AC::tri(j, l)] = fma(f[j], f[l], acc[AC::tri(j, l)]);
#pragma unroll
    for (int j = 0; j < A; j++)
#pragma unroll
        for (int k = 0; k < K; k++) acc[AC::C0 + j * K + k] = fma(f[j], y[k], acc[AC::C0 + j * K + k]);
    if (W) {
#pragma unroll
        for (int j = 0; j < A; j++) acc[AC::Q0 + j] = fma(f[j], w, acc[AC::Q0 + j]);
    }
}

template <int A, int K, bool W>
__device__ __forceinline__ void accum_pair(double (&acc)[Acc<A, K, W>::N], const double2 (&f2)[A],
                                           const double2 (&y2)[K], double2 w2) {
    double fa[A], ya[K];
#pragma unroll
    for (int j = 0; j < A; j++) fa[j] = f2[j].x;
#pragma unroll
    for (int k = 0; k < K; k++) ya[k] = y2[k].x;
    accum_row<A, K, W, false>(acc, fa, ya, w2.x);
#pragma unroll
    for (int j = 0; j < A; j++) fa[j] = f2[j].y;
#pragma unroll
    for (int k = 0; k < K; k++) ya[k] = y2[k].y;
    accum_row<A, K, W, false>(acc, fa, ya, w2.y);
}

template <int N, int NP, int P>
__device__ __forceinline__ void reduce_to_tot(const double (&acc)[N], double *red, int red_rows, double *tot,
                                              int lane) {
    constexpr int LPS = 32 / P;
    if (red_rows >= N) {
#pragma unroll
        for (int i = 0; i < N; i++) red[i * kRedPitch + lane] = acc[i];
        __syncwarp();
#pragma unroll
        for (int t0 = 0; t0 < N * LPS; t0 += 32) {
            const int t = t0 + lane;
            if (t < N * LPS) {
                const int u = (LPS == 1) ? 0 : t / N;
                const int a = t - u * N;
                const double *row = red + a * kRedPitch + u * P;
                double s0 = row[0], s1 = row[1], s2 = row[2], s3 = row[3];
#pragma unroll
                for (int i = 4; i < P; i += 4) {
                    s0 += row[i];
                    s1 += row[i + 1];
                    s2 += row[i + 2];
                    s3 += row[i + 3];
                }
                tot[u * NP + a] = (s0 + s1) + (s2 + s3);
            }
        }
        __syncwarp();
        return;
    }
    for (int b0 = 0; b0 < N; b0 += red_rows) {
        if (b0) __syncwarp();
#pragma unroll
        for (int i = 0; i < N; i++)
            if (i >= b0 && i < b0 + red_rows) red[(i - b0) * kRedPitch + lane] = acc[i];
        __syncwarp();
        const int nb = min(red_rows, N - b0);
        for (int t = lane; t < nb * LPS; t += 32) {
            const int u = (LPS == 1) ? 0 : t / nb;
            const int a = t - u * nb;
            const double *row = red + a * kRedPitch + u * P;
            double s0 = row[0], s1 = row[1], s2 = row[2], s3 = row[3];
#pragma unroll
            for (int i = 4; i < P; i += 4) {
                s0 += row[i];
                s1 += row[i + 1];
                s2 += row[i + 2];
                s3 += row[i + 3];
            }
            tot[u * NP + b0 + a] = (s0 + s1) + (s2 + s3);
        }
    }
    __syncwarp();
}

static __device__ __noinline__ double exact_q(const ScanParams &p, int64_t locus, int j, const double *ws, int lane) {
    const Layout &lay = p.lay;
    const double *fl = p.freq + (size_t)locus * lay.freq_stride();
    double q = 0.0;
    int i0 = 0;
    for (int c = 0; c < lay.n_chunks; c++) {
        const int rcc = (c == lay.n_chunks - 1) ? lay.rc_last : lay.rc;
        const double *col = fl + (size_t)c * lay.A * lay.rc + (size_t)j * rcc;
        const int rows = min(rcc, lay.n - i0);
        for (int r0 = 0; r0 < rows; r0 += 32) {
            const int r = r0 + lane;
            double term = 0.0;
            if (r < rows) {
                const double f = col[r];
                const double w = ws ? ws[i0 + r] : p.w_uniform;
                term = (f != f) ? 0.0 : __dmul_rn(f, w);
            }
            const int m = min(32, rows - r0);
            for (int t = 0; t < m; t++) q = __dadd_rn(q, __shfl_sync(PG_FULL_MASK, term, t));
        }
        i0 += rcc;
    }
    return q;
}

template <int A>
__device__ __forceinline__ void renorm_row(const double (&f)[A], uint32_t d, unsigned kept, double (&F)[A]) {
    double c[A];
    double dk = 0.0;
#pragma unroll
    for (int j = 0; j < A; j++) {
        c[j] = (d == 0u) ? 0.0 : rint(f[j] * (double)d);
        if ((kept >> j) & 1u) dk += c[j];
    }
#pragma unroll
    for (int j = 0; j < A; j++) {
        if ((kept >> j) & 1u)
            F[j] = (dk == 0.0) ? nan("") : c[j] / dk;
        else
            F[j] = 0.0;
    }
}

template <int A>
__device__ __forceinline__ void renorm_row_fast(const double (&f)[A], uint32_t d, unsigned kept, double (&F)[A]) {
    double c[A];
    double dk = 0.0;
#pragma unroll
    for (int j = 0; j < A; j++) {
        c[j] = (d == 0u) ? 0.0 : rint(f[j] * (double)d);
        if ((kept >> j) & 1u) dk += c[j];
    }
    const double inv = (dk == 0.0) ? nan("") : 1.0 / dk;
#pragma unroll
    for (int j = 0; j < A; j++) F[j] = ((kept >> j) & 1u) ? c[j] * inv : 0.0;
}

__device__ __forceinline__ double rcp_fast(double x) {
    double r;
    asm("rcp.approx.ftz.f64 %0, %1;" : "=d"(r) : "d"(x));
    double e = fma(-x, r, 1.0);
    r = fma(r, e, r);
    e = fma(-x, r, 1.0);
    return fma(r, e, r);
}

template <int A>
__device__ __forceinline__ void renorm_pair(double2 (&f2)[A], unsigned kept, int row, int n) {
    double sx = 0.0, sy = 0.0;
#pragma unroll
    for (int j = 0; j < A; j++)
        if ((kept >> j) & 1u) {
            sx += f2[j].x;
            sy += f2[j].y;
        }
    const double ix = (row < n) ? rcp_fast(sx) : 0.0, iy = (row + 1 < n) ? rcp_fast(sy) : 0.0;
#pragma unroll
    for (int j = 0; j < A; j++)
        f2[j] = ((kept >> j) & 1u) ? make_double2(f2[j].x * ix, f2[j].y * iy) : make_double2(0.0, 0.0);
}

template <int A>
__device__ __noinline__ double exact_colsum(const ScanParams &p, int64_t locus, int jsel, unsigned kept) {
    const Layout &lay = p.lay;
    const double *fl = p.freq + (size_t)locus * lay.freq_stride();
    const uint32_t *dl = p.depth + (size_t)locus * lay.depth_stride();
    double s = 0.0;
    int i0 = 0;
    for (int c = 0; c < lay.n_chunks; c++) {
        const int rcc = (c == lay.n_chunks - 1) ? lay.rc_last : lay.rc;
        const double *blk = fl + (size_t)c * lay.A * lay.rc;
        const int rows = min(rcc, lay.n - i0);
        for (int r = 0; r < rows; r++) {
            double f[A], F[A];
#pragma unroll
            for (int j = 0; j < A; j++) f[j] = blk[(size_t)j * rcc + r];
            renorm_row<A>(f, dl[i0 + r], kept, F);
            double v = 0.0;
#pragma unroll
            for (int j = 0; j < A; j++)
                if (j == jsel) v = F[j];
            if (v == v) s = __dadd_rn(s, v);
        }
        i0 += rcc;
    }
    return s;
}

template <int A, typename Fn>
__device__ __forceinline__ void for_rows_coop(const ScanParams &p, int64_t locus, int lane, Fn &&fn) {
    const Layout &lay = p.lay;
    const double *fl = p.freq + (size_t)locus * lay.freq_stride();
    const uint32_t *dl = p.depth + (size_t)locus * lay.depth_stride();
    int i0 = 0;
    for (int c = 0; c < lay.n_chunks; c++) {
        const int rcc = (c == lay.n_chunks - 1) ? lay.rc_last : lay.rc;
        const double *blk = fl + (size_t)c * lay.A * lay.rc;
        const int rows = min(rcc, lay.n - i0);
        for (int r0 = 0; r0 < rows; r0 += 128) {
            double f[4][A];
            uint32_t d[4];
#pragma unroll
            for (int i = 0; i < 4; i++) {
                const int r = r0 + lane + 32 * i;
                const bool ok = r < rows;
#pragma unroll
                for (int j = 0; j < A; j++) f[i][j] = ok ? blk[(size_t)j * rcc + r] : 0.0;
                d[i] = ok ? dl[i0 + r] : 1u;
            }
#pragma unroll
            for (int i = 0; i < 4; i++) {
                const int r = r0 + lane + 32 * i;
                if (r < rows) fn(i0 + r, f[i], d[i]);
            }
        }
        i0 += rcc;
    }
}

template <int A, int K, bool W>
__device__ __noinline__ int slow_locus(const ScanParams &p, int64_t locus, const double *ys, const double *ws,
                                       double *tot, int lane, bool decide, unsigned &kept_out) {
    using AC = Acc<A, K, W>;
    const Layout &lay = p.lay;
    const uint32_t *dl = p.depth + (size_t)locus * lay.depth_stride();
    unsigned kept = kept_out;
    if (decide) {
        kept = 0;
        for (int j = 0; j < A; j++) {
            const double q = exact_q(p, locus, j, ws, lane);
            if (!((q < p.maf) | (q > p.one_minus_maf))) kept |= 1u << j;
        }
        kept_out = kept;
        if (__popc(kept) < 2) return PG_LOCUS_FILTERED;
        int miss = 0;
        for (int i = lane; i < lay.n; i += 32) miss += (dl[i] == 0u) ? 1 : 0;
        miss = __reduce_add_sync(PG_FULL_MASK, miss);
        if (miss == lay.n) return PG_LOCUS_FILTERED;
        if (((double)miss / (double)lay.n) > p.max_miss) return PG_LOCUS_FILTERED;
    }
    double acc[AC::N];
#pragma unroll
    for (int i = 0; i < AC::N; i++) acc[i] = 0.0;
    const int n_pad = lay.n_pad;
    for_rows_coop<A>(p, locus, lane, [&](int i, const double(&f)[A], uint32_t d) {
        double F[A], y[K];
        renorm_row_fast<A>(f, d, kept, F);
#pragma unroll
        for (int k = 0; k < K; k++) y[k] = ys[k * n_pad + i];
        accum_row<A, K, W, true>(acc, F, y, 0.0);
    });
#pragma unroll
    for (int i = 0; i < AC::N; i++) {
        const double v = warp_sum_fixed(acc[i]);
        if (lane == 0) tot[i] = v;
    }
    __syncwarp();
    return PG_LOCUS_OK;
}

__device__ __forceinline__ bool chol_inv(int m, const double (&S)[PG_MAX_SLOTS][PG_MAX_SLOTS],
                                         double (&Li)[PG_MAX_SLOTS][PG_MAX_SLOTS], double (&dg)[PG_MAX_SLOTS]) {
    double Lm[PG_MAX_SLOTS][PG_MAX_SLOTS];
    bool ok = true;
    for (int a = 0; a < m; a++)
        for (int b = 0; b <= a; b++) {
            double s = S[a][b];
            for (int c = 0; c < b; c++) s -= Lm[a][c] * Lm[b][c];
            if (a == b) {
                if (!(s > 0.0)) {
                    ok = false;
                    s = 1.0;
                }
                Lm[a][a] = sqrt(s);
            } else {
                Lm[a][b] = s / Lm[b][b];
            }
        }
    for (int a = 0; a < m; a++) {
        Li[a][a] = 1.0 / Lm[a][a];
        for (int b = 0; b < a; b++) {
            double s = 0.0;
            for (int c = b; c < a; c++) s -= Lm[a][c] * Li[c][b];
            Li[a][b] = s / Lm[a][a];
        }
    }
    for (int b = 0; b < m; b++) {
        double s = 0.0;
        for (int a = b; a < m; a++) s += Li[a][b] * Li[a][b];
        dg[b] = s;
    }
    return ok;
}

__device__ __forceinline__ double solve_rhs(int m, const double (&Li)[PG_MAX_SLOTS][PG_MAX_SLOTS],
                                            const double (&sxy)[PG_MAX_SLOTS], double (&beta)[PG_MAX_SLOTS]) {
    double z[PG_MAX_SLOTS];
    double zz = 0.0;
    for (int a = 0; a < m; a++) {
        double s = 0.0;
        for (int b = 0; b <= a; b++) s += Li[a][b] * sxy[b];
        z[a] = s;
        zz += s * s;
    }
    for (int b = 0; b < m; b++) {
        double s = 0.0;
        for (int a = b; a < m; a++) s += Li[a][b] * z[a];
        beta[b] = s;
    }
    return zz;
}

__device__ __forceinline__ int slot_col(unsigned cb, int s) { return (int)((cb >> (4 * s)) & 0xfu); }

enum { REDO_NONE = 0, REDO_OLS = 1, REDO_CORR = 2, REDO_CORR_NAN = 3, REDO_DEFER = 4, REDO_MINNORM = 5 };

template <int KIND>
__device__ __forceinline__ bool kind_is_ols(const ScanParams &p) {
    if constexpr (KIND >= 0) return KIND == PG_KIND_OLS;
    else return p.kind == PG_KIND_OLS;
}

template <int A, int K>
__device__ __noinline__ int redo_locus(const ScanParams &p, int64_t locus, unsigned kept, int m, unsigned cb, int mode,
                                       const double *ys, double *out, int lane) {
    constexpr int MS = A - 1;
    const Layout &lay = p.lay;
    const int n_pad = lay.n_pad;
    const double nn = (double)lay.n;
    double xbar[MS], ybar[K];
    double cntv = nn;
    {
        double sx[MS], sy[K], cnt = 0.0;
#pragma unroll
        for (int a = 0; a < MS; a++) sx[a] = 0.0;
#pragma unroll
        for (int k = 0; k < K; k++) sy[k] = 0.0;
        for_rows_coop<A>(p, locus, lane, [&](int i, const double(&f)[A], uint32_t d) {
            double F[A], x[MS];
            renorm_row<A>(f, d, kept, F);
            bool valid = true;
#pragma unroll
            for (int a = 0; a < MS; a++) {
                double v = 0.0;
#pragma unroll
                for (int j = 0; j < A; j++)
                    if (a < m && j == slot_col(cb, a)) v = F[j];
                x[a] = v;
                valid &= (v == v);
            }
            if (mode == REDO_CORR_NAN && !valid) return;
            cnt += 1.0;
#pragma unroll
            for (int a = 0; a < MS; a++) sx[a] += x[a];
#pragma unroll
            for (int k = 0; k < K; k++) sy[k] += ys[k * n_pad + i];
        });
        cntv = warp_sum_fixed(cnt);
#pragma unroll
        for (int a = 0; a < MS; a++) xbar[a] = warp_sum_fixed(sx[a]) / cntv;
#pragma unroll
        for (int k = 0; k < K; k++) ybar[k] = warp_sum_fixed(sy[k]) / cntv;
    }
    double S[PG_MAX_SLOTS][PG_MAX_SLOTS], sxy[K][PG_MAX_SLOTS], syy[K];
    {
        double Sa[MS * (MS + 1) / 2], sxya[K][MS], syya[K];
#pragma unroll
        for (int i = 0; i < MS * (MS + 1) / 2; i++) Sa[i] = 0.0;
#pragma unroll
        for (int k = 0; k < K; k++) {
            syya[k] = 0.0;
#pragma unroll
            for (int a = 0; a < MS; a++) sxya[k][a] = 0.0;
        }
        for_rows_coop<A>(p, locus, lane, [&](int i, const double(&f)[A], uint32_t d) {
            double F[A], x[MS];
            renorm_row<A>(f, d, kept, F);
            bool valid = true;
#pragma unroll
            for (int a = 0; a < MS; a++) {
                double v = 0.0;
#pragma unroll
                for (int j = 0; j < A; j++)
                    if (a < m && j == slot_col(cb, a)) v = F[j];
                valid &= (v == v);
                x[a] = v - xbar[a];
            }
            if (mode == REDO_CORR_NAN && !valid) return;
#pragma unroll
            for (int a = 0; a < MS; a++)
#pragma unroll
                for (int b = 0; b <= a; b++) Sa[a * (a + 1) / 2 + b] = fma(x[a], x[b], Sa[a * (a + 1) / 2 + b]);
#pragma unroll
            for (int k = 0; k < K; k++) {
                const double dy = ys[k * n_pad + i] - ybar[k];
                syya[k] = fma(dy, dy, syya[k]);
#pragma unroll
                for (int a = 0; a < MS; a++) sxya[k][a] = fma(x[a], dy, sxya[k][a]);
            }
        });
#pragma unroll
        for (int a = 0; a < PG_MAX_SLOTS; a++)
#pragma unroll
            for (int b = 0; b < PG_MAX_SLOTS; b++) S[a][b] = 0.0;
#pragma unroll
        for (int a = 0; a < MS; a++)
#pragma unroll
            for (int b = 0; b <= a; b++) S[a][b] = warp_sum_fixed(Sa[a * (a + 1) / 2 + b]);
#pragma unroll
        for (int k = 0; k < K; k++) {
            syy[k] = warp_sum_fixed(syya[k]);
#pragma unroll
            for (int a = 0; a < PG_MAX_SLOTS; a++) sxy[k][a] = 0.0;
#pragma unroll
            for (int a = 0; a < MS; a++) sxy[k][a] = warp_sum_fixed(sxya[k][a]);
        }
    }
    if (mode != REDO_OLS) {
        if (lane == 0)
            for (int a = 0; a < m; a++)
                for (int k = 0; k < K; k++) {
                    const double den = (mode == REDO_CORR_NAN) ? sqrt(S[a][a]) * sqrt(syy[k])
                                                                : sqrt(S[a][a]) * sqrt(p.syy[k]);
                    out[(a * K + k) * 2 + 0] = sxy[k][a] / den;
                    out[(a * K + k) * 2 + 1] = 0.0;
                }
        __syncwarp();
        return PG_LOCUS_OK;
    }
    double Li[PG_MAX_SLOTS][PG_MAX_SLOTS], dg[PG_MAX_SLOTS], beta[K][PG_MAX_SLOTS];
    if (!chol_inv(m, S, Li, dg)) return PG_LOCUS_FAILED;
    for (int k = 0; k < K; k++) solve_rhs(m, Li, sxy[k], beta[k]);
    double rss[K];
    {
        double ra[K];
#pragma unroll
        for (int k = 0; k < K; k++) ra[k] = 0.0;
        for_rows_coop<A>(p, locus, lane, [&](int i, const double(&f)[A], uint32_t d) {
            double F[A], x[MS];
            renorm_row<A>(f, d, kept, F);
#pragma unroll
            for (int a = 0; a < MS; a++) {
                double v = 0.0;
#pragma unroll
                for (int j = 0; j < A; j++)
                    if (a < m && j == slot_col(cb, a)) v = F[j];
                x[a] = v - xbar[a];
            }
#pragma unroll
            for (int k = 0; k < K; k++) {
                double e = ys[k * n_pad + i] - ybar[k];
#pragma unroll
                for (int a = 0; a < MS; a++)
                    if (a < m) e -= beta[k][a] * x[a];
                ra[k] = fma(e, e, ra[k]);
            }
        });
#pragma unroll
        for (int k = 0; k < K; k++) rss[k] = warp_sum_fixed(ra[k]);
    }
    if (lane == 0) {
        const double dfe = nn - (double)(m + 1);
        for (int k = 0; k < K; k++) {
            const double ve = rss[k] / dfe;
            for (int b = 0; b < m; b++) {
                out[(b * K + k) * 2 + 0] = beta[k][b];
                out[(b * K + k) * 2 + 1] = ve * dg[b];
            }
        }
    }
    __syncwarp();
    return PG_LOCUS_OK;
}

template <int A, int K>
__device__ __noinline__ int corr_pairwise_locus(const ScanParams &p, int64_t locus, unsigned kept, int m, unsigned cb,
                                                const double *ys, double *out, int lane) {
    constexpr int MS = A - 1;
    const int n_pad = p.lay.n_pad;
    double xbar[K][MS], ybar[K];
    {
        double cnt[K], sx[K][MS], sy[K];
#pragma unroll
        for (int k = 0; k < K; k++) {
            cnt[k] = sy[k] = 0.0;
#pragma unroll
            for (int a = 0; a < MS; a++) sx[k][a] = 0.0;
        }
        for_rows_coop<A>(p, locus, lane, [&](int i, const double(&f)[A], uint32_t d) {
            double F[A], x[MS];
            renorm_row<A>(f, d, kept, F);
            bool xv = true;
#pragma unroll
            for (int a = 0; a < MS; a++) {
                double v = 0.0;
#pragma unroll
                for (int j = 0; j < A; j++)
                    if (a < m && j == slot_col(cb, a)) v = F[j];
                x[a] = v;
                xv &= (v == v);
            }
#pragma unroll
            for (int k = 0; k < K; k++) {
                const double y = ys[k * n_pad + i];
                if (xv && y == y) {
                    cnt[k] += 1.0;
                    sy[k] += y;
#pragma unroll
                    for (int a = 0; a < MS; a++) sx[k][a] += x[a];
                }
            }
        });
#pragma unroll
        for (int k = 0; k < K; k++) {
            const double c = warp_sum_fixed(cnt[k]);
            ybar[k] = warp_sum_fixed(sy[k]) / c;
#pragma unroll
            for (int a = 0; a < MS; a++) xbar[k][a] = warp_sum_fixed(sx[k][a]) / c;
        }
    }
    double sxx[K][MS], sxy[K][MS], syy[K];
#pragma unroll
    for (int k = 0; k < K; k++) {
        syy[k] = 0.0;
#pragma unroll
        for (int a = 0; a < MS; a++) sxx[k][a] = sxy[k][a] = 0.0;
    }
    for_rows_coop<A>(p, locus, lane, [&](int i, const double(&f)[A], uint32_t d) {
        double F[A], x[MS];
        renorm_row<A>(f, d, kept, F);
        bool xv = true;
#pragma unroll
        for (int a = 0; a < MS; a++) {
            double v = 0.0;
#pragma unroll
            for (int j = 0; j < A; j++)
                if (a < m && j == slot_col(cb, a)) v = F[j];
            x[a] = v;
            xv &= (v == v);
        }
#pragma unroll
        for (int k = 0; k < K; k++) {
            const double y = ys[k * n_pad + i];
            if (xv && y == y) {
                const double dy = y - ybar[k];
                syy[k] = fma(dy, dy, syy[k]);
#pragma unroll
                for (int a = 0; a < MS; a++) {
                    const double dx = x[a] - xbar[k][a];
                    sxx[k][a] = fma(dx, dx, sxx[k][a]);
                    sxy[k][a] = fma(dx, dy, sxy[k][a]);
                }
            }
        }
    });
#pragma unroll
    for (int k = 0; k < K; k++) {
        const double yy = warp_sum_fixed(syy[k]);
#pragma unroll
        for (int a = 0; a < MS; a++) {
            const double xx = warp_sum_fixed(sxx[k][a]), xy = warp_sum_fixed(sxy[k][a]);
            if (lane == 0 && a < m) {
                out[(a * K + k) * 2 + 0] = xy / (sqrt(xx) * sqrt(yy));
                out[(a * K + k) * 2 + 1] = 0.0;
            }
        }
    }
    __syncwarp();
    return PG_LOCUS_OK;
}

template <int A, int K>
__device__ __noinline__ int minnorm_locus(const ScanParams &p, int64_t locus, unsigned kept, int m, unsigned cb,
                                          const double *ys, double *out, int lane) {
    constexpr int MS = A - 1, PX = A, NR = 5;
    const int n = p.lay.n, n_pad = p.lay.n_pad, px = m + 1;
    double xrow[PX];
#pragma unroll
    for (int c = 0; c < PX; c++) xrow[c] = 0.0;
    for_rows_coop<A>(p, locus, lane, [&](int i, const double(&f)[A], uint32_t d) {
        double F[A];
        renorm_row<A>(f, d, kept, F);
        xrow[0] = 1.0;
#pragma unroll
        for (int a = 0; a < MS; a++) {
            double v = 0.0;
#pragma unroll
            for (int j = 0; j < A; j++)
                if (a < m && j == slot_col(cb, a)) v = F[j];
            xrow[1 + a] = v;
        }
    });
    double X[NR][PX], Y[NR][K];
#pragma unroll
    for (int i = 0; i < NR; i++) {
#pragma unroll
        for (int c = 0; c < PX; c++) X[i][c] = __shfl_sync(PG_FULL_MASK, xrow[c], i);
#pragma unroll
        for (int k = 0; k < K; k++) Y[i][k] = (i < n) ? ys[k * n_pad + i] + p.ymean[k] : 0.0;
    }
    double M[NR][NR];
#pragma unroll
    for (int i = 0; i < NR; i++)
#pragma unroll
        for (int j = 0; j < NR; j++) {
            double s = 0.0;
#pragma unroll
            for (int c = 0; c < PX; c++)
                if (c < px) s += X[i][c] * X[j][c];
            M[i][j] = (i < n && j < n) ? s : (i == j ? 1.0 : 0.0);
        }
    constexpr int NB = K + MS;
    double B[NR][NB];
#pragma unroll
    for (int i = 0; i < NR; i++) {
#pragma unroll
        for (int k = 0; k < K; k++) B[i][k] = Y[i][k];
#pragma unroll
        for (int a = 0; a < MS; a++) B[i][K + a] = (i < n) ? X[i][1 + a] : 0.0;
    }
    bool singular = false;
#pragma unroll
    for (int j = 0; j < NR; j++) {
        int jp = j;
        double amax = fabs(M[j][j]);
#pragma unroll
        for (int i = j + 1; i < NR; i++) {
            const double v = fabs(M[i][j]);
            if (v > amax) {
                amax = v;
                jp = i;
            }
        }
#pragma unroll
        for (int i = j + 1; i < NR; i++)
            if (i == jp) {
#pragma unroll
                for (int c = 0; c < NR; c++) {
                    const double t = M[j][c];
                    M[j][c] = M[i][c];
                    M[i][c] = t;
                }
#pragma unroll
                for (int c = 0; c < NB; c++) {
                    const double t = B[j][c];
                    B[j][c] = B[i][c];
                    B[i][c] = t;
                }
            }
        if (!(fabs(M[j][j]) > 0.0)) {
            singular = true;
            M[j][j] = 1.0;
        }
        const double r = 1.0 / M[j][j];
#pragma unroll
        for (int i = j + 1; i < NR; i++) {
            const double l = M[i][j] * r;
#pragma unroll
            for (int c = j + 1; c < NR; c++) M[i][c] -= l * M[j][c];
#pragma unroll
            for (int c = 0; c < NB; c++) B[i][c] -= l * B[j][c];
        }
    }
    if (singular) return PG_LOCUS_FAILED;
#pragma unroll
// ... 452 lines not shown
        while (need) {
            const int src = __ffs(need) - 1;
            need &= need - 1;
            const bool dec = __shfl_sync(PG_FULL_MASK, (int)slow_decide, src) != 0;
            unsigned kk = __shfl_sync(PG_FULL_MASK, kept, src);
            const int64_t lsrc = __shfl_sync(PG_FULL_MASK, locus, src);
            const int st = slow_locus<A, K, W>(p, lsrc, ys, ws, tot + (size_t)src * AC::NP, lane, dec, kk);
            if (lane == src) {
                status = st;
                kept = kk;
            }
        }
        __syncwarp();
    }
    int m = 0, redo_mode = REDO_NONE;
    unsigned cb = 0;
    if (act && status == PG_LOCUS_OK && !deferred)
        solve_locus<A, K, W, DEFER, KIND>(p, locus, tg, status, kept, m, cb, redo_mode);
    if (DEFER) {
        uint64_t why = (exact_bits != 0u ? 1u : 0u) | ((slow && !slow_decide) ? 2u : 0u) | (slow_decide ? 4u : 0u) |
                       ((deferred && pre_kept) ? 8u : 0u);
        if (redo_mode != REDO_NONE) {
            deferred = true;
            why |= (uint64_t)redo_mode << 4;
        }
        if (deferred)
            p.defer_list[atomicAdd(p.defer_count, 1u)] =
                (uint64_t)locus | (kept_known ? ((uint64_t)kept << 40) : 0ull) | (why << 56);
    } else {
        unsigned need = __ballot_sync(PG_FULL_MASK, redo_mode != REDO_NONE);
        while (need) {
            const int src = __ffs(need) - 1;
            need &= need - 1;
            const int md = __shfl_sync(PG_FULL_MASK, redo_mode, src);
            const unsigned kk = __shfl_sync(PG_FULL_MASK, kept, src);
            const int mm = __shfl_sync(PG_FULL_MASK, m, src);
            const unsigned cc = __shfl_sync(PG_FULL_MASK, cb, src);
            const int64_t lsrc = __shfl_sync(PG_FULL_MASK, locus, src);
            __syncwarp();
            const int st = (md == REDO_CORR_NAN)
                               ? corr_pairwise_locus<A, K>(p, lsrc, kk, mm, cc, ys, tot + (size_t)src * AC::NP, lane)
                           : (md == REDO_MINNORM)
                               ? minnorm_locus<A, K>(p, lsrc, kk, mm, cc, ys, tot + (size_t)src * AC::NP, lane)
                               : redo_locus<A, K>(p, lsrc, kk, mm, cc, md, ys, tot + (size_t)src * AC::NP, lane);
            if (lane == src) status = st;
        }
        __syncwarp();
    }
    if (act && !deferred) write_records<A, K, KIND>(p, ptab, locus, status, m, cb, tg);
    __syncwarp();
}

constexpr int kFixWarps = 8;

template <int A, int K, bool W>
__global__ void __launch_bounds__(kFixWarps * 32) fixup_kernel(const __grid_constant__ ScanParams p) {
    using AC = Acc<A, K, W>;
    extern __shared__ __align__(16) unsigned char fsm[];
    __shared__ __align__(16) ScanParams sp_storage;
    for (int i = threadIdx.x; i < (int)(sizeof(ScanParams) / 4); i += blockDim.x)
        reinterpret_cast<uint32_t *>(&sp_storage)[i] = reinterpret_cast<const uint32_t *>(&p)[i];
    __syncthreads();
    const ScanParams &sp = sp_storage;
    const int warp = threadIdx.x >> 5, lane = threadIdx.x & 31;
    const uint32_t count = *p.defer_count;
    const int n_pad = p.lay.n_pad;
    const double *ys = p.yc;
    const double *ws = W ? p.w : nullptr;
    const uint32_t per_blk = min(32u, max(1u, (count + gridDim.x - 1) / gridDim.x));
    const uint32_t n_blocks = (count + per_blk - 1) / per_blk;
    int it = 0;
    for (uint32_t blk = blockIdx.x; blk < n_blocks; blk += gridDim.x, it++) {
        double *tot = reinterpret_cast<double *>(fsm) + (size_t)(it & 1) * 32 * AC::NP;
        const uint32_t e0 = blk * per_blk;
        const int cnt = (int)min(per_blk, count - e0);
        for (int g = warp; g < cnt; g += kFixWarps) {
            const uint64_t e = p.defer_list[e0 + g];
            const int64_t locus = (int64_t)(e & 0xFFFFFFFFFFull);
            const unsigned kept = (unsigned)(e >> 40) & 0x3fu;
            double acc[AC::N];
#pragma unroll
            for (int a = 0; a < AC::N; a++) acc[a] = 0.0;
            if (kept) {
                for_rows_coop<A>(sp, locus, lane, [&](int r, const double(&f)[A], uint32_t d) {
                    double F[A], y[K];
                    renorm_row_fast<A>(f, d, kept, F);
#pragma unroll
                    for (int k = 0; k < K; k++) y[k] = ys[k * n_pad + r];
                    accum_row<A, K, W, true>(acc, F, y, 0.0);
                });
            } else {
                for_rows_coop<A>(sp, locus, lane, [&](int r, const double(&f)[A], uint32_t) {
                    double y[K];
#pragma unroll
                    for (int k = 0; k < K; k++) y[k] = ys[k * n_pad + r];
                    accum_row<A, K, W, false>(acc, f, y, W ? ws[r] : 0.0);
                });
            }
#pragma unroll
            for (int a = 0; a < AC::N; a++) {
                const double v = warp_sum_fixed(acc[a]);
                if (lane == 0) tot[(size_t)g * AC::NP + a] = v;
            }
        }
        __syncthreads();
        if (warp == (it % kFixWarps)) {
            const uint64_t mine = (lane < cnt) ? p.defer_list[e0 + lane] : 0ull;
            const int64_t locus = (int64_t)(mine & 0xFFFFFFFFFFull);
            const unsigned dm = (lane < cnt) ? __ldg(p.dmin + locus) : 0xFFFFFFFFu;
            epilogue<A, K, W, false, -1>(sp, locus, lane < cnt, tot, ys, ws, lane, dm, (unsigned)(mine >> 40) & 0x3fu);
        }
    }
}

template <int A, int K, bool W, int P, int KIND>
__global__ void __launch_bounds__(kScanWarps * 32, 1) scan_kernel(const __grid_constant__ ScanParams p) {
    using AC = Acc<A, K, W>;
    constexpr int LPS = 32 / P;
    constexpr int RC = chunk_rows(A);
    extern __shared__ __align__(128) unsigned char smem[];
    __shared__ __align__(16) ScanParams sp_storage;
    for (int i = threadIdx.x; i < (int)(sizeof(ScanParams) / 4); i += blockDim.x)
        reinterpret_cast<uint32_t *>(&sp_storage)[i] = reinterpret_cast<const uint32_t *>(&p)[i];
    const ScanParams &sp = sp_storage;
    const Layout lay = p.lay;
    const int n_pad = lay.n_pad;
    const int G = p.block_loci;
    const int warp = threadIdx.x >> 5, lane = threadIdx.x & 31, nwarps = blockDim.x >> 5;
    double *ys = reinterpret_cast<double *>(smem);
    double *ws = W ? ys + (size_t)K * n_pad : nullptr;
    unsigned char *wb = smem + p.common_bytes + (size_t)warp * p.warp_bytes;
    uint64_t *bars = reinterpret_cast<uint64_t *>(wb);
    unsigned char *stage0 = wb + 64;
    double *tot = reinterpret_cast<double *>(stage0 + (size_t)p.nbuf * p.stage_bytes);
    const int nbuf = p.nbuf;
    const int red_rows = max(1, min((int)(p.stage_bytes / (kRedPitch * 8)), AC::N));

    for (int i = threadIdx.x; i < K * n_pad; i += blockDim.x) ys[i] = p.yc[i];
    if (W)
        for (int i = threadIdx.x; i < n_pad; i += blockDim.x) ws[i] = p.w[i];
    if (lane == 0) {
        for (int b = 0; b < nbuf; b++) mbar_init(&bars[b], 1);
        fence_mbar_init();
    }
    __syncthreads();

    const int64_t L = p.n_loci;
    const int64_t NB = (L + G - 1) / G;
    const int64_t gw = (int64_t)blockIdx.x * nwarps + warp;
    const int64_t TW = (int64_t)gridDim.x * nwarps;
    if (gw >= NB) return;
    const int n_chunks = lay.n_chunks;
    const size_t fstride = lay.freq_stride();
    const uint32_t full_bytes = (uint32_t)(A * lay.rc * 8), last_bytes = (uint32_t)(A * lay.rc_last * 8);
    const uint32_t locus_bytes = (uint32_t)(fstride * 8);

    int64_t i_blk = gw;
    const unsigned char *i_src = reinterpret_cast<const unsigned char *>(p.freq + (size_t)(gw * G) * fstride);
    int i_left = (int)min((int64_t)G, L - gw * G);
    int i_chunk = 0;
    bool i_done = false;
    auto issue_next = [&](int b, bool scratch_used) {
        if (i_done) return;
        uint32_t bytes;
        int nl = 1;
        if (P == 32) {
            bytes = (i_chunk == n_chunks - 1) ? last_bytes : full_bytes;
        } else {
            nl = min(LPS, i_left);
            bytes = (uint32_t)nl * locus_bytes;
        }
        if (lane == 0) {
            if (scratch_used) fence_proxy_async();
            mbar_expect_tx(&bars[b], bytes);
            bulk_g2s(stage0 + (size_t)b * p.stage_bytes, i_src, bytes, &bars[b]);
        }
        i_src += bytes;
        if (P == 32) {
            if (++i_chunk == n_chunks) {
                i_chunk = 0;
                i_left--;
            }
        } else {
            i_left -= nl;
        }
        if (i_left == 0) {
            i_blk += TW;
            if (i_blk >= NB) {
                i_done = true;
            } else {
                i_src = reinterpret_cast<const unsigned char *>(p.freq + (size_t)(i_blk * G) * fstride);
                i_left = (int)min((int64_t)G, L - i_blk * G);
            }
        }
    };
    for (int b = 0; b < nbuf; b++) issue_next(b, false);

    int buf = 0;
    uint32_t parity = 0;
    auto load_meta = [&](int64_t b, unsigned &dm_o, unsigned &hl_o) {
        const int64_t m0 = b * G;
        const bool in = b < NB && lane < (int)min((int64_t)G, L - m0);
        dm_o = in ? __ldg(p.dmin + m0 + lane) : 0xFFFFFFFFu;
        hl_o = in ? (unsigned)__ldg(p.hint + m0 + lane) : 0u;
    };
    unsigned dm_next, hl_next;
    load_meta(gw, dm_next, hl_next);
    for (int64_t blk = gw; blk < NB; blk += TW) {
        const int64_t l0 = blk * G;
        const int cnt = (int)min((int64_t)G, L - l0);
        const unsigned dm = dm_next, hl = hl_next;
        load_meta(blk + TW, dm_next, hl_next);
        if (P == 32) {
            for (int g = 0; g < cnt; g++) {
                const unsigned hk = __shfl_sync(PG_FULL_MASK, hl, g);
                const bool hinted = (hk & 0x80u) != 0u;
                const unsigned hkept = hk & 0x3fu;
                double acc[AC::N];
#pragma unroll
                for (int i = 0; i < AC::N; i++) acc[i] = 0.0;
                for (int chunk = 0; chunk < n_chunks; chunk++) {
                    const double *yrow = ys + chunk * RC + 2 * lane;
                    const double *wrow = W ? ws + chunk * RC + 2 * lane : nullptr;
                    mbar_wait(&bars[buf], parity);
                    double *fb = reinterpret_cast<double *>(stage0 + (size_t)buf * p.stage_bytes);
                    if (chunk < n_chunks - 1 || lay.rc_last == RC) {
                        const double *fl = fb + 2 * lane;
#pragma unroll
                        for (int it = 0; it < RC / 64; it++) {
                            double2 f2[A], y2[K];
#pragma unroll
                            for (int j = 0; j < A; j++) f2[j] = *reinterpret_cast<const double2 *>(fl + j * RC + it * 64);
#pragma unroll
                            for (int k = 0; k < K; k++)
                                y2[k] = *reinterpret_cast<const double2 *>(yrow + (size_t)k * n_pad + it * 64);
                            double2 w2 = make_double2(0.0, 0.0);
                            if (W) w2 = *reinterpret_cast<const double2 *>(wrow + it * 64);
                            if (hinted) renorm_pair<A>(f2, hkept, chunk * RC + it * 64 + 2 * lane, lay.n);
                            accum_pair<A, K, W>(acc, f2, y2, w2);
                        }
                    } else {
                        const int rcc = lay.rc_last;
                        for (int r = 2 * lane; r < rcc; r += 64) {
                            double2 f2[A], y2[K];
#pragma unroll
                            for (int j = 0; j < A; j++) f2[j] = *reinterpret_cast<const double2 *>(fb + (size_t)j * rcc + r);
#pragma unroll
                            for (int k = 0; k < K; k++)
                                y2[k] = *reinterpret_cast<const double2 *>(ys + chunk * RC + (size_t)k * n_pad + r);
                            double2 w2 = make_double2(0.0, 0.0);
                            if (W) w2 = *reinterpret_cast<const double2 *>(ws + chunk * RC + r);
                            if (hinted) renorm_pair<A>(f2, hkept, chunk * RC + r, lay.n);
                            accum_pair<A, K, W>(acc, f2, y2, w2);
                        }
                    }
                    __syncwarp();
                    if (chunk == n_chunks - 1)
                        reduce_to_tot<AC::N, AC::NP, 32>(acc, fb, red_rows, tot + (size_t)g * AC::NP, lane);
                    issue_next(buf, chunk == n_chunks - 1);
                    if (++buf == nbuf) {
                        buf = 0;
                        parity ^= 1u;
                    }
                }
            }
        } else {
            const int u = lane / P, q0 = lane % P;
            const int nsteps = (cnt + LPS - 1) / LPS;
            for (int s = 0; s < nsteps; s++) {
                double acc[AC::N];
#pragma unroll
                for (int i = 0; i < AC::N; i++) acc[i] = 0.0;
                const unsigned hk = __shfl_sync(PG_FULL_MASK, hl, min(s * LPS + u, 31));
                const bool hinted = (hk & 0x80u) != 0u;
                const unsigned hkept = hk & 0x3fu;
                mbar_wait(&bars[buf], parity);
                double *fb = reinterpret_cast<double *>(stage0 + (size_t)buf * p.stage_bytes);
                const double *fl = fb + (size_t)u * fstride;
                if (__any_sync(PG_FULL_MASK, hinted)) {
                    if (s * LPS + u < cnt) {
#pragma unroll 1
                        for (int r = 2 * q0; r < n_pad; r += 2 * P) {
                            double2 f2[A], y2[K];
#pragma unroll
                            for (int j = 0; j < A; j++)
                                f2[j] = *reinterpret_cast<const double2 *>(fl + (size_t)j * n_pad + r);
#pragma unroll
                            for (int k = 0; k < K; k++)
                                y2[k] = *reinterpret_cast<const double2 *>(ys + (size_t)k * n_pad + r);
                            double2 w2 = make_double2(0.0, 0.0);
                            if (W) w2 = *reinterpret_cast<const double2 *>(ws + r);
                            if (hinted) renorm_pair<A>(f2, hkept, r, lay.n);
                            accum_pair<A, K, W>(acc, f2, y2, w2);
                        }
                    }
                } else if (s * LPS + u < cnt) {
#pragma unroll 2
                    for (int r = 2 * q0; r < n_pad; r += 2 * P) {
                        double2 f2[A], y2[K];
#pragma unroll
                        for (int j = 0; j < A; j++) f2[j] = *reinterpret_cast<const double2 *>(fl + (size_t)j * n_pad + r);
#pragma unroll
                        for (int k = 0; k < K; k++) y2[k] = *reinterpret_cast<const double2 *>(ys + (size_t)k * n_pad + r);
                        double2 w2 = make_double2(0.0, 0.0);
                        if (W) w2 = *reinterpret_cast<const double2 *>(ws + r);
                        accum_pair<A, K, W>(acc, f2, y2, w2);
                    }
                }
                __syncwarp();
                reduce_to_tot<AC::N, AC::NP, P>(acc, fb, red_rows, tot + (size_t)(s * LPS) * AC::NP, lane);
                issue_next(buf, true);
                if (++buf == nbuf) {
                    buf = 0;
                    parity ^= 1u;
                }
            }
        }
        epilogue<A, K, W, true, KIND>(sp, l0 + lane, lane < cnt, tot, ys, ws, lane, dm, (hl & 0x80u) ? (hl & 0x3fu) : 0u);
    }
}

template <int A, int K, bool W, int P>
cudaError_t launch_scan_p(ScanParams p, int sm_count, cudaStream_t s) {
    using AC = Acc<A, K, W>;
    const Layout &lay = p.lay;
    const size_t avail = 227 * 1024 - 512;
    size_t common = (size_t)(K + (W ? 1 : 0)) * lay.n_pad * 8;
    common = (common + 127) / 128 * 128;
    size_t stage = (P == 32) ? (size_t)A * lay.rc * 8 : (size_t)(32 / P) * lay.freq_stride() * 8;
    stage = (stage + 127) / 128 * 128;
    if (stage < (size_t)kRedPitch * 8) stage = ((size_t)kRedPitch * 8 + 127) / 128 * 128;
    int G = 32, nbuf = 3, nwarps = 0;
    size_t wbytes = 0;
    auto fit = [&](int g, int nb) {
        const size_t tot_bytes = ((size_t)g * AC::NP * 8 + 127) / 128 * 128;
        wbytes = 64 + (size_t)nb * stage + tot_bytes;
        nwarps = common + wbytes <= avail ? (int)((avail - common) / wbytes) : 0;
        if (nwarps > kScanWarps) nwarps = kScanWarps;
        return nwarps;
    };
    const int g_min = (P == 32) ? 16 : 32;
    if (p.nbuf_override >= 1 || p.g_override >= 1) {
        G = (p.g_override == 16 || p.g_override == 32) && P == 32 ? p.g_override : 32;
        nbuf = (p.nbuf_override >= 1 && p.nbuf_override <= 8) ? p.nbuf_override : 2;
        fit(G, nbuf);
    } else if (fit(32, 3) >= kScanWarps) {
        G = 32, nbuf = 3;
    } else if (fit(32, 2) >= kScanWarps) {
        G = 32, nbuf = 2;
    } else if (fit(g_min, 2) >= kScanWarps) {
        G = g_min, nbuf = 2;
    } else {
        G = 32, nbuf = 2;
        fit(G, nbuf);
    }
    if (p.warps_override >= 1 && p.warps_override < nwarps) nwarps = p.warps_override;
    if (nwarps < 1) return cudaErrorInvalidConfiguration;
    if (p.g_override < 1 && p.n_loci > 0) {
        const int64_t gw = (int64_t)sm_count * nwarps;
        const int step = (P == 32) ? 1 : 32 / P;
        const int64_t r = (p.n_loci + gw * G - 1) / (gw * G);
        int64_t g = (p.n_loci + gw * r - 1) / (gw * r);
        g = (g + step - 1) / step * step;
        if (g < step) g = step;
        if (g < G) G = (int)g;
    }
    p.common_bytes = (uint32_t)common;
    p.warp_bytes = (uint32_t)wbytes;
    p.stage_bytes = (uint32_t)stage;
    p.nbuf = nbuf;
    p.block_loci = G;
    const size_t smem = common + (size_t)nwarps * wbytes;
    auto kern = (p.kind == PG_KIND_OLS) ? scan_kernel<A, K, W, P, PG_KIND_OLS> : scan_kernel<A, K, W, P, PG_KIND_CORR>;
    cudaError_t e = cudaFuncSetAttribute(kern, cudaFuncAttributeMaxDynamicSharedMemorySize, (int)smem);
    if (e != cudaSuccess) return e;
    const int64_t NB = (p.n_loci + G - 1) / G;
    int64_t ctas = (NB + nwarps - 1) / nwarps;
    if (ctas > sm_count) ctas = sm_count;
    if (ctas < 1) ctas = 1;
    e = cudaMemsetAsync(p.defer_count, 0, 4, s);
    if (e != cudaSuccess) return e;
    kern<<<(unsigned)ctas, nwarps * 32, smem, s>>>(p);
    e = cudaGetLastError();
    if (e != cudaSuccess) return e;
    auto fix = fixup_kernel<A, K, W>;
    const size_t fsmem = (size_t)2 * 32 * AC::NP * 8;
    e = cudaFuncSetAttribute(fix, cudaFuncAttributeMaxDynamicSharedMemorySize, (int)fsmem);
    if (e != cudaSuccess) return e;
    fix<<<sm_count * 8, kFixWarps * 32, fsmem, s>>>(p);
    return cudaGetLastError();
}

template <int A, int K, bool W>
cudaError_t launch_scan_t(const ScanParams &p, int sm_count, cudaStream_t s) {
    if (p.lay.n_chunks == 1) {
        const int P = p.p_override ? p.p_override : (p.lay.n_pad > 64 ? 16 : 8);
        if (P == 16) return launch_scan_p<A, K, W, 16>(p, sm_count, s);
        return launch_scan_p<A, K, W, 8>(p, sm_count, s);
    }
    return launch_scan_p<A, K, W, 32>(p, sm_count, s);
}

template <int A>
cudaError_t launch_scan_a(const ScanParams &p, int sm_count, cudaStream_t s) {
    const bool w = p.weighted != 0;
    switch (p.K) {
        case 1: return w ? launch_scan_t<A, 1, true>(p, sm_count, s) : launch_scan_t<A, 1, false>(p, sm_count, s);
        case 2: return w ? launch_scan_t<A, 2, true>(p, sm_count, s) : launch_scan_t<A, 2, false>(p, sm_count, s);
        case 3:
            if constexpr (A <= 5) return w ? launch_scan_t<A, 3, true>(p, sm_count, s) : launch_scan_t<A, 3, false>(p, sm_count, s);
            else return cudaErrorInvalidValue;
        case 4:
            if constexpr (A <= 4) return w ? launch_scan_t<A, 4, true>(p, sm_count, s) : launch_scan_t<A, 4, false>(p, sm_count, s);
            else return cudaErrorInvalidValue;
        default: return cudaErrorInvalidValue;
    }
}

}
```

poolgen_b200/csrc/pg_text.cu:

```cuda
#include <cub/device/device_scan.cuh>

#include "pg_device.cuh"
#include "pg_internal.h"

namespace pg {

enum { TEXT_OK = 0, TEXT_ERR_POOLS = 1, TEXT_ERR_FIELD = 2, TEXT_ERR_LINES = 3, TEXT_ERR_LOCI = 4 };

constexpr int kTokThreads = 256;
constexpr int kTokBytes = 16;
constexpr int kTokBlock = kTokThreads * kTokBytes;
constexpr int kLineGroup = 256;

struct TextParams {
    const char *text;
    uint32_t n_bytes;
    uint32_t *sep;
    uint32_t *nl;
    uint64_t *tok_blk;
    uint32_t n_tok_blocks;
    uint32_t line_cap;
    uint32_t max_loci;
    int n_pools;
    uint8_t *keep;
// ... 80 lines not shown
            ms &= ms - 1;
            p.sep[o_sep++] = base + b;
        }
        while (mn) {
            const int b = __ffs(mn) - 1;
            mn &= mn - 1;
            if (o_nl < p.line_cap) p.nl[o_nl] = base + b;
            o_nl++;
        }
    }
}

__global__ void __launch_bounds__(kLineGroup) text_lines_kernel(const TextParams p) {
    const uint32_t n_lines = min(p.info[3], p.line_cap);
    const uint32_t n_sep = (uint32_t)(p.tok_blk[p.n_tok_blocks] >> 32);
    const uint32_t n_groups = (n_lines + kLineGroup - 1) / kLineGroup;
    for (uint32_t g = blockIdx.x; g < n_groups; g += gridDim.x) {
        const uint32_t l = g * kLineGroup + threadIdx.x;
        uint32_t keep = 0;
        if (l < n_lines) {
            const uint32_t start = l ? p.nl[l - 1] + 1 : 0u, end = p.nl[l];
            uint32_t lo = 0, hi = n_sep;
            while (lo < hi) {
                const uint32_t mid = (lo + hi) >> 1;
                if (p.sep[mid] < end) lo = mid + 1; else hi = mid;
            }
            const uint32_t nl_rank = lo;
            uint32_t lo2 = 0, hi2 = nl_rank;
            while (lo2 < hi2) {
                const uint32_t mid = (lo2 + hi2) >> 1;
                if (p.sep[mid] < start) lo2 = mid + 1; else hi2 = mid;
            }
            const uint32_t first = lo2;
            const uint32_t n_tabs = nl_rank - first;
            p.first_sep[l] = first;
            if (end > start && p.text[start] != '#' && n_tabs >= 2) {
                uint32_t a = p.sep[first] + 1, b = p.sep[first + 1];
                if (a < b && p.text[a] == '+') a++;
                bool ok = a < b;
                uint64_t v = 0;
                for (uint32_t i = a; i < b && ok; i++) {
                    const unsigned d = (unsigned)(p.text[i] - '0');
                    if (d > 9u || v > (0xFFFFFFFFFFFFFFFFull - d) / 10ull) ok = false;
                    v = v * 10ull + d;
                }
                if (ok) {
                    keep = 1;
                    p.line_pos[l] = v;
                    if ((int)n_tabs != p.n_pools + 2) text_error(p, TEXT_ERR_POOLS, start);
                }
            }
            p.keep[l] = (uint8_t)keep;
        }
        const int c = __syncthreads_count((int)keep);
        if (threadIdx.x == 0) p.grp[g] = (uint32_t)c;
    }
}

__global__ void __launch_bounds__(256) text_parse_kernel(const TextParams p) {
    const int lane = threadIdx.x & 31;
    const uint32_t warp = (blockIdx.x * blockDim.x + threadIdx.x) >> 5, nwarps = (gridDim.x * blockDim.x) >> 5;
    const int n = p.n_pools;
    const uint32_t n_lines = min(p.info[3], p.line_cap);
    const uint32_t n_loci = p.grp[p.n_groups_max];
    if (warp == 0 && lane == 0) {
        p.info[0] = n_loci;
        if (n_loci > p.max_loci) text_error(p, TEXT_ERR_LOCI, n_loci);
    }
    for (uint32_t l = warp; l < n_lines; l += nwarps) {
        if (!p.keep[l]) continue;
        const uint32_t g0 = l & ~(uint32_t)(kLineGroup - 1);
        uint32_t before = 0;
        for (uint32_t j = g0 + lane; j < l; j += 32) before += p.keep[j];
        const uint32_t ord = p.grp[l / kLineGroup] + __reduce_add_sync(PG_FULL_MASK, before);
        if (ord >= p.max_loci) continue;
        const uint32_t start = l ? p.nl[l - 1] + 1 : 0u;
        const uint32_t first = p.first_sep[l];
        if (lane == 0) {
            p.out_offset[ord] = start;
            p.out_pos[ord] = p.line_pos[l];
        }
        const uint32_t end_rank = (l + 1 < n_lines) ? p.first_sep[l + 1] : (uint32_t)(p.tok_blk[p.n_tok_blocks] >> 32);
        uint32_t *out = p.counts + (size_t)ord * 6 * n;
        for (int i = lane; i < n; i += 32) {
            if (first + 3 + i >= end_rank) break;
            uint32_t a = p.sep[first + 2 + i] + 1, b = p.sep[first + 3 + i];
            if (b > a && p.text[b - 1] == '\r') b--;
            int j = 0;
            uint64_t v = 0;
            bool digits = false, bad = false, plus = false;
            for (uint32_t q = a; q <= b; q++) {
                const char c = (q < b) ? p.text[q] : ':';
                if (c == ':') {
                    if (!digits) bad = true;
                    if (j < 6) out[(size_t)j * n + i] = v > 0xFFFFFFFFull ? 0xFFFFFFFFu : (uint32_t)v;
                    j++;
                    v = 0;
                    digits = false;
                    plus = false;
                } else if (c == '+' && !digits && !plus) {
                    plus = true;
                } else {
                    const unsigned d = (unsigned)(c - '0');
                    if (d > 9u) bad = true;
                    v = v * 10ull + d;
                    if (v > 0xFFFFFFFFFFFFull) v = 0xFFFFFFFFFFFFull;
                    digits = true;
                }
            }
            if (bad || j < 6) text_error(p, TEXT_ERR_FIELD, a);
        }
    }
}

TextScratch::~TextScratch() {
    if (parsed) cudaEventDestroy(parsed);
}

static size_t with_headroom(size_t need) { return need + need / 8 + 65536; }

#define TCK(call)                      \
    do {                               \
        cudaError_t e_ = (call);       \
        if (e_ != cudaSuccess) return e_; \
    } while (0)

static cudaError_t text_parse_enqueue(TextScratch *t, const char *text, size_t n_bytes, int n_pools, uint32_t *d_counts,
                                      int64_t max_loci, size_t line_cap, int sm_count, cudaStream_t s) {
    t->max_loci = max_loci;
    if (!t->parsed) TCK(cudaEventCreateWithFlags(&t->parsed, cudaEventDisableTiming));
    TCK(t->d_info.reserve(4, s));
    TCK(t->h_info.reserve(4, s));
    TCK(cudaMemsetAsync(t->d_info.get(), 0, 16, s));
    if (n_bytes >= 0xFFFFFFF0ull) return cudaErrorInvalidValue;
    if (n_bytes == 0) {
        TCK(cudaMemcpyAsync(t->h_info.get(), t->d_info.get(), 16, cudaMemcpyDeviceToHost, s));
        return cudaEventRecord(t->parsed, s);
    }
    const bool add_nl = text[n_bytes - 1] != '\n';
    const size_t nb = n_bytes + (add_nl ? 1 : 0);
    if (line_cap == 0) line_cap = (size_t)max_loci + (size_t)max_loci / 4 + 4096;
    if (line_cap > nb) line_cap = nb;
    if (t->d_text.capacity() < nb + 32) TCK(t->d_text.reserve(with_headroom(nb + 32), s));
    TCK(cudaMemcpyAsync(t->d_text.get(), text, n_bytes, cudaMemcpyHostToDevice, s));
    if (add_nl) TCK(cudaMemsetAsync(t->d_text.get() + n_bytes, '\n', 1, s));
    const size_t n_tok = (nb + kTokBlock - 1) / kTokBlock;
    const size_t n_grp = (line_cap + kLineGroup - 1) / kLineGroup;
    if (t->d_sep.capacity() < nb) TCK(t->d_sep.reserve(with_headroom(nb), s));
    if (t->d_tok_blk.capacity() < n_tok + 1) TCK(t->d_tok_blk.reserve(with_headroom(n_tok + 1), s));
    TCK(t->d_nl.reserve(line_cap, s));
    TCK(t->d_keep.reserve(line_cap, s));
    TCK(t->d_first.reserve(line_cap, s));
    TCK(t->d_line_pos.reserve(line_cap, s));
    TCK(t->d_grp.reserve(n_grp + 2, s));
    TCK(t->d_out_offset.reserve((size_t)max_loci, s));
    TCK(t->d_out_pos.reserve((size_t)max_loci, s));
    TCK(t->h_out_offset.reserve((size_t)max_loci, s));
    TCK(t->h_out_pos.reserve((size_t)max_loci, s));
    size_t tmp1 = 0, tmp2 = 0;
    cub::DeviceScan::ExclusiveSum(nullptr, tmp1, (uint64_t *)nullptr, (uint64_t *)nullptr, (int)(n_tok + 1), s);
    cub::DeviceScan::ExclusiveSum(nullptr, tmp2, (uint32_t *)nullptr, (uint32_t *)nullptr, (int)(n_grp + 1), s);
    TCK(t->d_tmp.reserve(std::max(tmp1, tmp2), s));
    TextParams tp;
    tp.text = t->d_text.get();
    tp.n_bytes = (uint32_t)nb;
    tp.sep = t->d_sep.get();
    tp.nl = t->d_nl.get();
    tp.tok_blk = t->d_tok_blk.get();
    tp.n_tok_blocks = (uint32_t)n_tok;
    tp.line_cap = (uint32_t)line_cap;
    tp.max_loci = (uint32_t)std::min<int64_t>(max_loci, 0xFFFFFFFFll);
    tp.n_pools = n_pools;
    tp.keep = t->d_keep.get();
    tp.first_sep = t->d_first.get();
    tp.line_pos = t->d_line_pos.get();
    tp.grp = t->d_grp.get();
    tp.n_groups_max = (uint32_t)n_grp;
    tp.counts = d_counts;
    tp.out_offset = t->d_out_offset.get();
    tp.out_pos = t->d_out_pos.get();
    tp.info = t->d_info.get();
    const int grid_tok = (int)std::min<size_t>(n_tok, (size_t)sm_count * 16);
    TCK(cudaMemsetAsync(t->d_tok_blk.get() + n_tok, 0, 8, s));
    tok_count_kernel<<<grid_tok, kTokThreads, 0, s>>>(tp);
    TCK(cudaGetLastError());
    size_t tb = t->d_tmp.capacity();
    TCK(cub::DeviceScan::ExclusiveSum(t->d_tmp.get(), tb, t->d_tok_blk.get(), t->d_tok_blk.get(), (int)(n_tok + 1), s));
    tok_scatter_kernel<<<grid_tok, kTokThreads, 0, s>>>(tp);
    TCK(cudaGetLastError());
    TCK(cudaMemsetAsync(t->d_grp.get(), 0, (n_grp + 2) * 4, s));
    const int grid_lines = (int)std::min<size_t>(n_grp, (size_t)sm_count * 8);
    text_lines_kernel<<<grid_lines, kLineGroup, 0, s>>>(tp);
    TCK(cudaGetLastError());
    tb = t->d_tmp.capacity();
    TCK(cub::DeviceScan::ExclusiveSum(t->d_tmp.get(), tb, t->d_grp.get(), t->d_grp.get(), (int)(n_grp + 1), s));
    const int grid_parse = (int)std::min<uint64_t>(((uint64_t)line_cap * 32 + 255) / 256, (uint64_t)sm_count * 8);
    text_parse_kernel<<<grid_parse, 256, 0, s>>>(tp);
    TCK(cudaGetLastError());
    TCK(cudaMemcpyAsync(t->h_info.get(), t->d_info.get(), 16, cudaMemcpyDeviceToHost, s));
    return cudaEventRecord(t->parsed, s);
}
#undef TCK

cudaError_t text_parse_async(TextScratch *t, const char *text, size_t n_bytes, int n_pools, uint32_t *d_counts,
                             int64_t max_loci, size_t line_cap, int sm_count, cudaStream_t s) {
    t->pending = false;
    const cudaError_t e = text_parse_enqueue(t, text, n_bytes, n_pools, d_counts, max_loci, line_cap, sm_count, s);
    t->pending = (e == cudaSuccess);
    return e;
}

int64_t text_parse_finish(TextScratch *t, cudaStream_t s, cudaError_t *cuda_err, uint64_t *err_offset) {
    if (!t->pending) return 0;
    t->pending = false;
    cudaError_t e = cudaEventSynchronize(t->parsed);
    if (e != cudaSuccess) {
        *cuda_err = e;
        return -1;
    }
    const uint32_t *info = t->h_info.get();
    const uint32_t n_loci = info[0], code = info[1];
    *err_offset = info[2];
    if (code == TEXT_ERR_LINES) return -5;
    if (code == TEXT_ERR_POOLS) return -3;
    if (code == TEXT_ERR_FIELD) return -4;
    if (code == TEXT_ERR_LOCI || (int64_t)n_loci > t->max_loci) return -2;
    if (n_loci == 0) return 0;
    e = cudaMemcpyAsync(t->h_out_offset.get(), t->d_out_offset.get(), (size_t)n_loci * 8, cudaMemcpyDeviceToHost, s);
    if (e == cudaSuccess)
        e = cudaMemcpyAsync(t->h_out_pos.get(), t->d_out_pos.get(), (size_t)n_loci * 8, cudaMemcpyDeviceToHost, s);
    if (e != cudaSuccess) {
        *cuda_err = e;
        return -1;
    }
    return (int64_t)n_loci;
}

int text_parse_fail(pg_ctx *ctx, const char *who, int64_t status, cudaError_t cuda_err, uint64_t err_offset,
                    int n_pools, int64_t cap) {
    const unsigned long long at = err_offset;
    if (status == -1) return fail(ctx, PG_ERR_CUDA, "%s: %s", who, cudaGetErrorString(cuda_err));
    if (status == -2) return fail(ctx, PG_ERR_ARG, "%s: more loci in the chunk than the capacity %lld", who, (long long)cap);
    if (status == -3)
        return fail(ctx, PG_ERR_ARG, "%s: the line at byte %llu does not hold %d pools (the reference asserts the pool count, "
                                     "src/base/sync.rs:254-257)", who, at, n_pools);
    if (status == -4)
        return fail(ctx, PG_ERR_ARG, "%s: malformed pool field at byte %llu (the reference panics: allele counts are not "
                                     "valid integers, src/base/sync.rs:146)", who, at);
    return fail(ctx, PG_ERR_ARG, "%s: the chunk could not be parsed (%lld)", who, (long long)status);
}

}
```

Before: 213.5 million.

## Store resident allele counts as u16 and rebuild frequencies in scan kernel

For count inputs whose values fit in 16 bits, the batch now keeps raw u16 allele counts in device memory instead of f64 frequencies plus a separate depth array. Frequencies are recomputed in the scan kernel from the counts using a reciprocal table and a correctly rounded quotient. This cuts the bytes streamed per locus by the bandwidth-bound OLS scan, at the price of extra arithmetic per element and more template instantiations. The text parser now tracks the maximum count so it can choose the format.

Result: slower. 206.2 million (median of 6 runs) (-3.4%).

```diff
diff --git a/poolgen_b200/csrc/pg_api.cu b/poolgen_b200/csrc/pg_api.cu
--- a/poolgen_b200/csrc/pg_api.cu
+++ b/poolgen_b200/csrc/pg_api.cu
@@ -269,6 +269,16 @@
             return fail(ctx, PG_ERR_CUDA, "pg_scan_open: phenotype upload: %s", cudaGetErrorString(e));
         }
     }
+    if (regression) {
+        std::vector<double2> rcp(pg::kRcpTab);
+        for (int d = 0; d < pg::kRcpTab; d++) rcp[d] = make_double2(1.0 / (double)d, (double)d);
+        cudaError_t e = s->d_rcp.reserve(rcp.size(), nullptr);
+        if (e == cudaSuccess) e = cudaMemcpy(s->d_rcp.get(), rcp.data(), rcp.size() * 16, cudaMemcpyHostToDevice);
+        if (e != cudaSuccess) {
+            delete s;
+            return fail(ctx, PG_ERR_CUDA, "pg_scan_open: reciprocal table upload: %s", cudaGetErrorString(e));
+        }
+    }
     {
         cudaError_t e = s->d_w.reserve(s->w_host.size(), nullptr);
         if (e == cudaSuccess) e = cudaMemcpy(s->d_w.get(), s->w_host.data(), s->w_host.size() * 8, cudaMemcpyHostToDevice);
@@ -328,6 +338,7 @@
     if (!b) return fail(ctx, PG_ERR_ARG, "out of host memory");
     b->scan = s;
     b->cap = cap;
+    b->lay = s->lay;
     cudaError_t e = cudaStreamCreateWithFlags(&b->stream, cudaStreamNonBlocking);
     if (e == cudaSuccess) e = cudaEventCreate(&b->ev0);
     if (e == cudaSuccess) e = cudaEventCreate(&b->ev1);
@@ -355,11 +366,27 @@
     return PG_OK;
 }
 
+enum class Input { Counts8, Counts16, Counts32, Synth, Text, Freq };
+static int resident_format(const pg_scan *s, Input in, uint32_t max_count = 0) {
+    if (pg::several_loci_per_stage(s->lay)) return pg::FMT_F64;
+    switch (in) {
+        case Input::Counts8:
+        case Input::Counts16:
+        case Input::Synth: return pg::FMT_U16;
+        case Input::Text: return max_count <= 0xFFFFu ? pg::FMT_U16 : pg::FMT_F64;
+        default: return pg::FMT_F64;
+    }
+}
+static void set_input(pg_batch *b, Input in, uint32_t max_count = 0) {
+    b->lay = pg::make_layout(b->scan->n, b->scan->A_dev, resident_format(b->scan, in, max_count));
+}
+
 static pg::IngestOut ingest_out(pg_batch *b, int64_t first_locus) {
     pg_scan *s = b->scan;
     pg::IngestOut o;
-    o.freq = b->d_freq.get() + (size_t)first_locus * s->lay.freq_stride();
-    o.depth = b->d_depth.get() + (size_t)first_locus * s->lay.depth_stride();
+    o.lay = b->lay;
+    o.rows = reinterpret_cast<char *>(b->d_freq.get()) + (size_t)first_locus * b->lay.freq_stride() * b->lay.elem_bytes();
+    o.depth = b->d_depth.get() + (size_t)first_locus * b->lay.depth_stride();
     o.dmin = b->d_dmin.get() + first_locus;
     o.hint = b->d_hint.get() + first_locus;
     o.w = s->d_w.get();
@@ -388,19 +415,20 @@
     if (n_loci == 0) return PG_OK;
     const size_t bytes = (size_t)n_loci * s->A_in * s->n * sizeof(CT);
     const bool reg = is_regression(s);
+    set_input(b, sizeof(CT) == 1 ? Input::Counts8 : (sizeof(CT) == 2 ? Input::Counts16 : Input::Counts32));
     const size_t wide_bytes = (size_t)b->cap * s->A_in * s->n * 4;
     int rc = ensure_stage(b, reg ? (size_t)b->cap * s->A_in * s->n * sizeof(CT) : wide_bytes + (sizeof(CT) == 4 ? 0 : bytes));
     if (rc) return rc;
     if (reg) {
         PG_CUDA(ctx, cudaMemcpyAsync(b->d_stage.get(), counts, bytes, cudaMemcpyHostToDevice, b->stream));
         if constexpr (sizeof(CT) == 4)
-            PG_CUDA(ctx, pg::launch_ingest_u32((const uint32_t *)b->d_stage.get(), n_loci, s->n, s->A_in, s->drop_col, s->lay,
+            PG_CUDA(ctx, pg::launch_ingest_u32((const uint32_t *)b->d_stage.get(), n_loci, s->n, s->A_in, s->drop_col,
                                                ingest_out(b, 0), b->stream));
         else if constexpr (sizeof(CT) == 1)
-            PG_CUDA(ctx, pg::launch_ingest_u8((const uint8_t *)b->d_stage.get(), n_loci, s->n, s->A_in, s->drop_col, s->lay,
+            PG_CUDA(ctx, pg::launch_ingest_u8((const uint8_t *)b->d_stage.get(), n_loci, s->n, s->A_in, s->drop_col,
                                               ingest_out(b, 0), b->stream));
         else
-            PG_CUDA(ctx, pg::launch_ingest_u16((const uint16_t *)b->d_stage.get(), n_loci, s->n, s->A_in, s->drop_col, s->lay,
+            PG_CUDA(ctx, pg::launch_ingest_u16((const uint16_t *)b->d_stage.get(), n_loci, s->n, s->A_in, s->drop_col,
                                                ingest_out(b, 0), b->stream));
     } else if constexpr (sizeof(CT) == 4) {
         PG_CUDA(ctx, cudaMemcpyAsync(b->d_stage.get(), counts, bytes, cudaMemcpyHostToDevice, b->stream));
@@ -437,6 +465,7 @@
     PG_CUDA(ctx, cudaSetDevice(ctx->device));
     b->n_loci = n_loci;
     b->have_input = 1;
+    set_input(b, Input::Freq);
     if (n_loci == 0) return PG_OK;
     const size_t fbytes_cap = (size_t)b->cap * s->A_dev * s->n * 8, dbytes_cap = (size_t)b->cap * s->n * 4;
     int rc = ensure_stage(b, fbytes_cap + dbytes_cap);
@@ -445,7 +474,7 @@
     uint32_t *sd = (uint32_t *)((char *)b->d_stage.get() + fbytes_cap);
     PG_CUDA(ctx, cudaMemcpyAsync(sf, freq, (size_t)n_loci * s->A_dev * s->n * 8, cudaMemcpyHostToDevice, b->stream));
     PG_CUDA(ctx, cudaMemcpyAsync(sd, depth, (size_t)n_loci * s->n * 4, cudaMemcpyHostToDevice, b->stream));
-    PG_CUDA(ctx, pg::launch_ingest_freq(sf, sd, n_loci, s->n, s->lay, ingest_out(b, 0), b->stream));
+    PG_CUDA(ctx, pg::launch_ingest_freq(sf, sd, n_loci, s->n, ingest_out(b, 0), b->stream));
     b->input_is_counts = 0;
     return PG_OK;
 }
@@ -490,8 +519,9 @@
     if (L < 0) return pg::text_parse_fail(ctx, "upload_sync_text", L, ce, at, s->n, b->cap);
     b->n_loci = L;
     if (n_loci_out) *n_loci_out = L;
+    set_input(b, Input::Text, L > 0 ? b->text.max_count() : 0u);
     if (L > 0 && is_regression(s))
-        PG_CUDA(ctx, pg::launch_ingest_u32((const uint32_t *)b->d_stage.get(), L, s->n, s->A_in, s->drop_col, s->lay,
+        PG_CUDA(ctx, pg::launch_ingest_u32((const uint32_t *)b->d_stage.get(), L, s->n, s->A_in, s->drop_col,
                                            ingest_out(b, 0), b->stream));
     return PG_OK;
 }
@@ -522,6 +552,7 @@
     PG_CUDA(ctx, cudaSetDevice(ctx->device));
     b->n_loci = n_loci;
     b->have_input = 1;
+    set_input(b, Input::Synth);
     if (n_loci == 0) return PG_OK;
     const size_t per_locus = (size_t)s->A_in * s->n * 4;
     if (!is_regression(s)) {
@@ -544,7 +575,7 @@
     for (int64_t l0 = 0; l0 < n_loci; l0 += slice) {
         const int64_t m = (n_loci - l0 < slice) ? n_loci - l0 : slice;
         PG_CUDA(ctx, pg::launch_synth(seed, first_locus + l0, m, s->n, s->A_in, (uint32_t *)b->d_stage.get(), b->stream));
-        PG_CUDA(ctx, pg::launch_ingest_u32((const uint32_t *)b->d_stage.get(), m, s->n, s->A_in, s->drop_col, s->lay,
+        PG_CUDA(ctx, pg::launch_ingest_u32((const uint32_t *)b->d_stage.get(), m, s->n, s->A_in, s->drop_col,
                                            ingest_out(b, l0), b->stream));
     }
     b->input_is_counts = 1;
@@ -570,9 +601,10 @@
         for (int base = 0; base < (is_nm(s) ? 1 : s->k); base += kpass) {
             pg::ScanParams p;
             memset(&p, 0, sizeof p);
-            p.lay = s->lay;
-            p.freq = b->d_freq.get();
+            p.lay = b->lay;
+            p.rows = b->d_freq.get();
             p.depth = b->d_depth.get();
+            p.rcp_tab = s->d_rcp.get();
             p.dmin = b->d_dmin.get();
             p.hint = b->d_hint.get();
             p.n_loci = b->n_loci;
@@ -623,8 +655,8 @@
         if (is_nm(s)) {
             pg::NmParams q;
             memset(&q, 0, sizeof q);
-            q.lay = s->lay;
-            q.freq = b->d_freq.get();
+            q.lay = b->lay;
+            q.rows = b->d_freq.get();
             q.depth = b->d_depth.get();
             q.n_loci = b->n_loci;
             q.kind = s->kind;
@@ -718,7 +750,7 @@
     pg_scan *s = b->scan;
     const size_t L = (size_t)b->n_loci;
     if (input_bytes)
-        *input_bytes = is_regression(s) ? L * (s->lay.freq_stride() * 8 + 4)
+        *input_bytes = is_regression(s) ? L * (b->lay.freq_stride() * b->lay.elem_bytes() + 5)
                                         : L * (size_t)s->A_in * s->n * 4;
     if (result_bytes) *result_bytes = L * (8 + (size_t)s->n_slots * 8 + (size_t)s->n_slots * s->k * 32);
     return PG_OK;
diff --git a/poolgen_b200/csrc/pg_device.cuh b/poolgen_b200/csrc/pg_device.cuh
--- a/poolgen_b200/csrc/pg_device.cuh
+++ b/poolgen_b200/csrc/pg_device.cuh
@@ -1,6 +1,8 @@
 #pragma once
 #include <cuda_runtime.h>
 #include <stdint.h>
+
+#include "pg_internal.h"
 
 namespace pg {
 
@@ -43,6 +45,44 @@
         "}\n" ::"r"(smem_u32(bar)),
         "r"(parity)
         : "memory");
+}
+
+__device__ __forceinline__ double count_quotient_nz(double c, double d, double rd) {
+    const double q0 = __dmul_rn(c, rd);
+    return __fma_rn(__fma_rn(-q0, d, c), rd, q0);
+}
+__device__ __forceinline__ double count_quotient(double c, double d, double rd) {
+    return (d == 0.0) ? nan("") : count_quotient_nz(c, d, rd);
+}
+
+template <int NA>
+__device__ __forceinline__ uint32_t pool_row(const Layout &lay, const void *rows, const uint32_t *depth, int64_t locus,
+                                             int i, double (&f)[NA], double (&c)[NA]) {
+    const size_t base = (size_t)locus * lay.freq_stride();
+    if (lay.fmt == FMT_U16) {
+        const uint16_t *cl = static_cast<const uint16_t *>(rows) + base;
+        uint32_t ci[NA], d = 0;
+#pragma unroll
+        for (int j = 0; j < NA; j++) {
+            ci[j] = (j < lay.A) ? cl[lay.freq_off(i, j)] : 0u;
+            d += ci[j];
+        }
+        const double dd = (double)d, rd = __drcp_rn(dd);
+#pragma unroll
+        for (int j = 0; j < NA; j++) {
+            c[j] = (double)ci[j];
+            f[j] = count_quotient(c[j], dd, rd);
+        }
+        return d;
+    }
+    const double *fl = static_cast<const double *>(rows) + base;
+    const uint32_t d = depth[(size_t)locus * lay.depth_stride() + i];
+#pragma unroll
+    for (int j = 0; j < NA; j++) {
+        f[j] = (j < lay.A) ? fl[lay.freq_off(i, j)] : 0.0;
+        c[j] = (d == 0u) ? 0.0 : rint(f[j] * (double)d);
+    }
+    return d;
 }
 
 __device__ __forceinline__ void warp_reduce32(double (&v)[32], int lane) {
diff --git a/poolgen_b200/csrc/pg_ingest.cu b/poolgen_b200/csrc/pg_ingest.cu
--- a/poolgen_b200/csrc/pg_ingest.cu
+++ b/poolgen_b200/csrc/pg_ingest.cu
@@ -37,10 +37,10 @@
     return (safe && depth_ok && removed_with_reads && __popc(kept) >= 2) ? (uint8_t)(0x80u | kept) : (uint8_t)0;
 }
 
-template <typename RowFn>
-__device__ __forceinline__ void ingest_loci(int64_t n_loci, const Layout &lay, int P, const double *freq,
-                                            const double *__restrict__ w, uint32_t *__restrict__ dmin,
-                                            uint8_t *__restrict__ hint, const HintParams &hp, RowFn &&row) {
+template <typename RowFn, typename FreqFn>
+__device__ __forceinline__ void ingest_loci(int64_t n_loci, const Layout &lay, int P, const double *__restrict__ w,
+                                            uint32_t *__restrict__ dmin, uint8_t *__restrict__ hint,
+                                            const HintParams &hp, RowFn &&row, FreqFn &&freq_of) {
     const int lane = threadIdx.x & 31, sub = lane / P, q0 = lane % P, lpw = 32 / P;
     const int64_t gw = ((int64_t)blockIdx.x * blockDim.x + threadIdx.x) >> 5;
     const int64_t nw = ((int64_t)gridDim.x * blockDim.x) >> 5;
@@ -56,8 +56,6 @@
         }
         unsigned amb = (hp.enabled && locus < n_loci && dm != 0u) ? ambiguous_alleles(q, lay.A, lay.n, hp) : 0u;
         if (__any_sync(0xFFFFFFFFu, amb != 0u)) {
-            __syncwarp();
-            const double *fl = freq + (size_t)(locus < n_loci ? locus : 0) * lay.freq_stride();
             for (int j = 0; j < lay.A; j++) {
                 if (!__any_sync(0xFFFFFFFFu, (amb >> j) & 1u)) continue;
                 double e = 0.0;
@@ -65,7 +63,7 @@
                     const int i = r0 + q0;
                     double term = 0.0;
                     if (i < lay.n && locus < n_loci) {
-                        const double f = __ldcg(fl + lay.freq_off(i, j));
+                        const double f = freq_of(locus, i, j);
                         term = (f != f) ? 0.0 : __dmul_rn(f, w[i]);
                     }
                     const int m = min(P, lay.n - r0);
@@ -82,41 +80,61 @@
 }
 
 template <typename CT>
+__device__ __forceinline__ uint32_t row_counts(const CT *__restrict__ cl, int n, int A_in, int drop_col,
+                                               uint32_t (&c)[PG_MAX_ALLELES]) {
+    uint64_t d = 0;
+    int jj = 0;
+    for (int j = 0; j < A_in; j++) {
+        if (j == drop_col) continue;
+        c[jj] = (uint32_t)cl[(size_t)j * n];
+        d += c[jj];
+        jj++;
+    }
+    if (d > 0xFFFFFFFEull) d = 0xFFFFFFFEull;
+    return (uint32_t)d;
+}
+
+template <typename CT, int FMT>
 __global__ void __launch_bounds__(256) ingest_counts_kernel(const CT *__restrict__ counts, int64_t n_loci, int n,
                                                             int A_in, int drop_col, Layout lay, int P,
-                                                            double *__restrict__ freq, uint32_t *__restrict__ depth,
+                                                            void *__restrict__ rows, uint32_t *__restrict__ depth,
                                                             uint32_t *__restrict__ dmin, uint8_t *__restrict__ hint,
                                                             const double *__restrict__ w, HintParams hp) {
-    ingest_loci(n_loci, lay, P, freq, w, dmin, hint, hp, [&](int64_t locus, int i, double *q, uint32_t &dm) {
-        double *fl = freq + (size_t)locus * lay.freq_stride();
+    auto row = [&](int64_t locus, int i, double *q, uint32_t &dm) {
+        double *fl = static_cast<double *>(rows) + (size_t)locus * lay.freq_stride();
+        uint16_t *cl16 = static_cast<uint16_t *>(rows) + (size_t)locus * lay.freq_stride();
         if (i >= n) {
-            for (int j = 0; j < lay.A; j++) fl[lay.freq_off(i, j)] = 0.0;
-            depth[(size_t)locus * lay.n_pad + i] = 0xFFFFFFFFu;
+            for (int j = 0; j < lay.A; j++) {
+                if (FMT == FMT_U16)
+                    cl16[lay.freq_off(i, j)] = 0;
+                else
+                    fl[lay.freq_off(i, j)] = 0.0;
+            }
+            if (FMT == FMT_F64) depth[(size_t)locus * lay.n_pad + i] = 0xFFFFFFFFu;
             return;
         }
-        const CT *cl = counts + (size_t)locus * A_in * n + i;
         uint32_t c[PG_MAX_ALLELES];
-        uint64_t d = 0;
-        int jj = 0;
-        for (int j = 0; j < A_in; j++) {
-            if (j == drop_col) continue;
-            c[jj] = (uint32_t)cl[(size_t)j * n];
-            d += c[jj];
-            jj++;
-        }
-        if (d > 0xFFFFFFFEull) d = 0xFFFFFFFEull;
+        const uint32_t d = row_counts(counts + (size_t)locus * A_in * n + i, n, A_in, drop_col, c);
         const double dd = (double)d, wi = w[i];
         const double rd = __drcp_rn(dd);
         for (int j = 0; j < lay.A; j++) {
-            const double cj = (double)c[j];
-            const double q0 = __dmul_rn(cj, rd);
-            const double f = (d == 0) ? nan("") : __fma_rn(__fma_rn(-q0, dd, cj), rd, q0);
-            fl[lay.freq_off(i, j)] = f;
+            const double f = count_quotient((double)c[j], dd, rd);
+            if (FMT == FMT_U16)
+                cl16[lay.freq_off(i, j)] = (uint16_t)c[j];
+            else
+                fl[lay.freq_off(i, j)] = f;
             if (d != 0) q[j] = fma(f, wi, q[j]);
         }
-        depth[(size_t)locus * lay.n_pad + i] = (uint32_t)d;
-        dm = min(dm, (uint32_t)d);
-    });
+        if (FMT == FMT_F64) depth[(size_t)locus * lay.n_pad + i] = d;
+        dm = min(dm, d);
+    };
+    auto freq_of = [&](int64_t locus, int i, int j) {
+        uint32_t c[PG_MAX_ALLELES];
+        const uint32_t d = row_counts(counts + (size_t)locus * A_in * n + i, n, A_in, drop_col, c);
+        const double dd = (double)d;
+        return count_quotient((double)c[j], dd, __drcp_rn(dd));
+    };
+    ingest_loci(n_loci, lay, P, w, dmin, hint, hp, row, freq_of);
 }
 
 __global__ void __launch_bounds__(256) ingest_freq_kernel(const double *__restrict__ fin, const uint32_t *__restrict__ din,
@@ -124,7 +142,7 @@
                                                           double *__restrict__ freq, uint32_t *__restrict__ depth,
                                                           uint32_t *__restrict__ dmin, uint8_t *__restrict__ hint,
                                                           const double *__restrict__ w, HintParams hp) {
-    ingest_loci(n_loci, lay, P, freq, w, dmin, hint, hp, [&](int64_t locus, int i, double *q, uint32_t &dm) {
+    auto row = [&](int64_t locus, int i, double *q, uint32_t &dm) {
         double *fl = freq + (size_t)locus * lay.freq_stride();
         const bool pad = i >= n;
         for (int j = 0; j < lay.A; j++) {
@@ -135,7 +153,9 @@
         const uint32_t d = pad ? 0xFFFFFFFFu : din[(size_t)locus * n + i];
         depth[(size_t)locus * lay.n_pad + i] = d;
         dm = min(dm, d);
-    });
+    };
+    auto freq_of = [&](int64_t locus, int i, int j) { return fin[((size_t)locus * lay.A + j) * n + i]; };
+    ingest_loci(n_loci, lay, P, w, dmin, hint, hp, row, freq_of);
 }
 
 __global__ void __launch_bounds__(256) synth_kernel(uint64_t seed, int64_t first_locus, int64_t n_loci, int n,
@@ -172,32 +192,35 @@
     return hp;
 }
 template <typename CT>
-static cudaError_t launch_ingest_t(const CT *counts, int64_t n_loci, int n, int A_in, int drop_col, const Layout &lay,
-                                   const IngestOut &o, cudaStream_t s) {
+static cudaError_t launch_ingest_t(const CT *counts, int64_t n_loci, int n, int A_in, int drop_col, const IngestOut &o,
+                                   cudaStream_t s) {
     if (n_loci <= 0) return cudaSuccess;
+    const Layout &lay = o.lay;
     const int P = ingest_group(lay);
-    ingest_counts_kernel<CT><<<grid_for(n_loci * P), 256, 0, s>>>(counts, n_loci, n, A_in, drop_col, lay, P, o.freq,
-                                                                 o.depth, o.dmin, o.hint, o.w, hint_params(o));
-    return cudaGetLastError();
-}
-cudaError_t launch_ingest_u32(const uint32_t *counts, int64_t n_loci, int n, int A_in, int drop_col, const Layout &lay,
-                              const IngestOut &o, cudaStream_t s) {
-    return launch_ingest_t<uint32_t>(counts, n_loci, n, A_in, drop_col, lay, o, s);
-}
-cudaError_t launch_ingest_u16(const uint16_t *counts, int64_t n_loci, int n, int A_in, int drop_col, const Layout &lay,
-                              const IngestOut &o, cudaStream_t s) {
-    return launch_ingest_t<uint16_t>(counts, n_loci, n, A_in, drop_col, lay, o, s);
-}
-cudaError_t launch_ingest_u8(const uint8_t *counts, int64_t n_loci, int n, int A_in, int drop_col, const Layout &lay,
-                             const IngestOut &o, cudaStream_t s) {
-    return launch_ingest_t<uint8_t>(counts, n_loci, n, A_in, drop_col, lay, o, s);
-}
-cudaError_t launch_ingest_freq(const double *fin, const uint32_t *din, int64_t n_loci, int n, const Layout &lay,
-                               const IngestOut &o, cudaStream_t s) {
+    auto kern = (lay.fmt == FMT_U16) ? ingest_counts_kernel<CT, FMT_U16> : ingest_counts_kernel<CT, FMT_F64>;
+    kern<<<grid_for(n_loci * P), 256, 0, s>>>(counts, n_loci, n, A_in, drop_col, lay, P, o.rows, o.depth, o.dmin, o.hint,
+                                              o.w, hint_params(o));
+    return cudaGetLastError();
+}
+cudaError_t launch_ingest_u32(const uint32_t *counts, int64_t n_loci, int n, int A_in, int drop_col, const IngestOut &o,
+                              cudaStream_t s) {
+    return launch_ingest_t<uint32_t>(counts, n_loci, n, A_in, drop_col, o, s);
+}
+cudaError_t launch_ingest_u16(const uint16_t *counts, int64_t n_loci, int n, int A_in, int drop_col, const IngestOut &o,
+                              cudaStream_t s) {
+    return launch_ingest_t<uint16_t>(counts, n_loci, n, A_in, drop_col, o, s);
+}
+cudaError_t launch_ingest_u8(const uint8_t *counts, int64_t n_loci, int n, int A_in, int drop_col, const IngestOut &o,
+                             cudaStream_t s) {
+    return launch_ingest_t<uint8_t>(counts, n_loci, n, A_in, drop_col, o, s);
+}
+cudaError_t launch_ingest_freq(const double *fin, const uint32_t *din, int64_t n_loci, int n, const IngestOut &o,
+                               cudaStream_t s) {
     if (n_loci <= 0) return cudaSuccess;
-    const int P = ingest_group(lay);
-    ingest_freq_kernel<<<grid_for(n_loci * P), 256, 0, s>>>(fin, din, n_loci, n, lay, P, o.freq, o.depth, o.dmin, o.hint,
-                                                            o.w, hint_params(o));
+    if (o.lay.fmt != FMT_F64) return cudaErrorInvalidValue;
+    const int P = ingest_group(o.lay);
+    ingest_freq_kernel<<<grid_for(n_loci * P), 256, 0, s>>>(fin, din, n_loci, n, o.lay, P, static_cast<double *>(o.rows),
+                                                            o.depth, o.dmin, o.hint, o.w, hint_params(o));
     return cudaGetLastError();
 }
 template <typename CT>
diff --git a/poolgen_b200/csrc/pg_internal.h b/poolgen_b200/csrc/pg_internal.h
--- a/poolgen_b200/csrc/pg_internal.h
+++ b/poolgen_b200/csrc/pg_internal.h
@@ -10,7 +10,10 @@
 
 namespace pg {
 
-__host__ __device__ constexpr int chunk_rows(int A) { return A <= 2 ? 256 : (A == 3 ? 192 : 128); }
+enum { FMT_F64 = 0, FMT_U16 = 1 };
+__host__ __device__ constexpr int chunk_rows(int A, int fmt = FMT_F64) {
+    return (fmt == FMT_U16 ? 4 : 1) * (A <= 2 ? 256 : (A == 3 ? 192 : 128));
+}
 
 struct Layout {
     int n;
@@ -19,6 +22,8 @@
     int rc;
     int n_chunks;
     int rc_last;
+    int fmt;
+    __host__ __device__ int elem_bytes() const { return fmt == FMT_U16 ? 2 : 8; }
     __host__ __device__ size_t freq_stride() const { return (size_t)A * n_pad; }
     __host__ __device__ size_t depth_stride() const { return (size_t)n_pad; }
     __host__ __device__ size_t freq_off(int i, int j) const {
@@ -28,12 +33,13 @@
     }
 };
 
-inline Layout make_layout(int n, int A) {
+inline Layout make_layout(int n, int A, int fmt = FMT_F64) {
     Layout l;
     l.n = n;
-    l.n_pad = (n + 3) & ~3;
+    l.n_pad = (n + 7) & ~7;
     l.A = A;
-    const int cr = chunk_rows(A);
+    l.fmt = fmt;
+    const int cr = chunk_rows(A, fmt);
     if (l.n_pad <= cr) {
         l.rc = l.n_pad;
         l.n_chunks = 1;
@@ -45,14 +51,18 @@
     }
     return l;
 }
+__host__ __device__ inline bool several_loci_per_stage(const Layout &l) { return l.n_pad <= chunk_rows(l.A); }
+
+constexpr int kRcpTab = 4096;
 
 constexpr int kMaxPhenPerPass = 4;
 inline int max_phen_per_pass(int A) { return A <= 4 ? 4 : (A == 5 ? 3 : 2); }
 
 struct ScanParams {
     Layout lay;
-    const double *freq;
+    const void *rows;
     const uint32_t *depth;
+    const double2 *rcp_tab;
     const uint32_t *dmin;
     const uint8_t *hint;
     int64_t n_loci;
@@ -103,7 +113,7 @@
 
 struct NmParams {
     Layout lay;
-    const double *freq;
+    const void *rows;
     const uint32_t *depth;
     int64_t n_loci;
     int kind;
@@ -138,20 +148,21 @@
 cudaError_t launch_scan(const ScanParams &p, int sm_count, cudaStream_t s);
 cudaError_t launch_tables(const TableParams &p, int sm_count, cudaStream_t s);
 struct IngestOut {
-    double *freq;
+    Layout lay;
+    void *rows;
     uint32_t *depth;
     uint32_t *dmin;
     uint8_t *hint;
     const double *w;
     double maf, one_minus_maf, min_depth_f;
 };
-cudaError_t launch_ingest_u32(const uint32_t *counts, int64_t n_loci, int n, int A_in, int drop_col, const Layout &lay,
+cudaError_t launch_ingest_u32(const uint32_t *counts, int64_t n_loci, int n, int A_in, int drop_col,
                               const IngestOut &o, cudaStream_t s);
-cudaError_t launch_ingest_u16(const uint16_t *counts, int64_t n_loci, int n, int A_in, int drop_col, const Layout &lay,
+cudaError_t launch_ingest_u16(const uint16_t *counts, int64_t n_loci, int n, int A_in, int drop_col,
                               const IngestOut &o, cudaStream_t s);
-cudaError_t launch_ingest_u8(const uint8_t *counts, int64_t n_loci, int n, int A_in, int drop_col, const Layout &lay,
+cudaError_t launch_ingest_u8(const uint8_t *counts, int64_t n_loci, int n, int A_in, int drop_col,
                              const IngestOut &o, cudaStream_t s);
-cudaError_t launch_ingest_freq(const double *freq_in, const uint32_t *depth_in, int64_t n_loci, int n, const Layout &lay,
+cudaError_t launch_ingest_freq(const double *freq_in, const uint32_t *depth_in, int64_t n_loci, int n,
                                const IngestOut &o, cudaStream_t s);
 cudaError_t launch_synth(uint64_t seed, int64_t first_locus, int64_t n_loci, int n, int A_in,
                          uint32_t *counts, cudaStream_t s);
@@ -226,6 +237,7 @@
     bool pending = false;
     int64_t max_loci = 0;
     ~TextScratch();
+    uint32_t max_count() const { return h_info.get()[4]; }
 };
 cudaError_t text_parse_async(TextScratch *t, const char *text, size_t n_bytes, int n_pools, uint32_t *d_counts,
                              int64_t max_loci, size_t line_cap, int sm_count, cudaStream_t s);
@@ -274,6 +286,7 @@
     double df = 0, ln_beta = 0;
     pg::DeviceBuffer<double> d_yc;
     pg::DeviceBuffer<double> d_w;
+    pg::DeviceBuffer<double2> d_rcp;
     pg::DeviceBuffer<double> d_yraw;
     double gw_sig = 0, gw_min = 0, gw_max = 0;
     pg::DeviceBuffer<double> d_ptab;
@@ -291,6 +304,7 @@
     int64_t cap = 0, n_loci = 0;
     cudaStream_t stream = nullptr;
     cudaEvent_t ev0 = nullptr, ev1 = nullptr;
+    pg::Layout lay;
     pg::DeviceBuffer<double> d_freq;
     pg::DeviceBuffer<uint32_t> d_depth;
     pg::DeviceBuffer<uint32_t> d_dmin;
diff --git a/poolgen_b200/csrc/pg_nm.cu b/poolgen_b200/csrc/pg_nm.cu
--- a/poolgen_b200/csrc/pg_nm.cu
+++ b/poolgen_b200/csrc/pg_nm.cu
@@ -193,15 +193,12 @@
     for (int j = 0; j < d; j++) best[j] = v[0][j];
 }
 
-__device__ __forceinline__ void renorm_generic(const NmParams &p, const double *fl, const uint32_t *dl, int i, unsigned kept,
-                                               double *F) {
+__device__ __forceinline__ void renorm_generic(const NmParams &p, int64_t locus, int i, unsigned kept, double *F) {
     const int A = p.lay.A;
-    const uint32_t d = dl[i];
-    double c[PG_MAX_ALLELES], dk = 0.0;
-    for (int j = 0; j < A; j++) {
-        c[j] = (d == 0u) ? 0.0 : rint(fl[p.lay.freq_off(i, j)] * (double)d);
+    double f[PG_MAX_ALLELES], c[PG_MAX_ALLELES], dk = 0.0;
+    pool_row(p.lay, p.rows, p.depth, locus, i, f, c);
+    for (int j = 0; j < A; j++)
         if ((kept >> j) & 1u) dk += c[j];
-    }
     for (int j = 0; j < A; j++) F[j] = ((kept >> j) & 1u) ? ((dk == 0.0) ? nan("") : c[j] / dk) : 0.0;
 }
 
@@ -244,13 +241,11 @@
             if (!__shfl_sync(PG_FULL_MASK, (int)act, g)) continue;
             const int mg = __shfl_sync(PG_FULL_MASK, m, g);
             const unsigned cg = __shfl_sync(PG_FULL_MASK, colw, g), kg = __shfl_sync(PG_FULL_MASK, kept, g);
-            const double *fl = p.freq + (size_t)(l0 + g) * p.lay.freq_stride();
-            const uint32_t *dl = p.depth + (size_t)(l0 + g) * p.lay.depth_stride();
             double sx[PG_MAX_SLOTS], lo[PG_MAX_SLOTS], hi[PG_MAX_SLOTS];
             for (int a = 0; a < PG_MAX_SLOTS; a++) sx[a] = 0.0, lo[a] = INFINITY, hi[a] = -INFINITY;
             for (int i = lane; i < n; i += 32) {
                 double F[PG_MAX_ALLELES];
-                renorm_generic(p, fl, dl, i, kg, F);
+                renorm_generic(p, l0 + g, i, kg, F);
                 for (int a = 0; a < mg; a++) {
                     const double f = F[(cg >> (4 * a)) & 0xfu];
                     sx[a] += f;
@@ -277,7 +272,7 @@
             for (int e = 0; e < 15; e++) sxx[e] = 0.0;
             for (int i = lane; i < n; i += 32) {
                 double F[PG_MAX_ALLELES];
-                renorm_generic(p, fl, dl, i, kg, F);
+                renorm_generic(p, l0 + g, i, kg, F);
                 for (int a = 0; a < mg; a++)
                     for (int b = 0; b <= a; b++)
                         sxx[a * (a + 1) / 2 + b] = fma(F[(cg >> (4 * a)) & 0xfu] - xb[a], F[(cg >> (4 * b)) & 0xfu] - xb[b], sxx[a * (a + 1) / 2 + b]);
@@ -374,8 +369,6 @@
                 if (!__shfl_sync(PG_FULL_MASK, (int)act, g)) continue;
                 const int mg = __shfl_sync(PG_FULL_MASK, m, g);
                 const unsigned cg = __shfl_sync(PG_FULL_MASK, colw, g), kg = __shfl_sync(PG_FULL_MASK, kept, g);
-                const double *fl = p.freq + (size_t)(l0 + g) * p.lay.freq_stride();
-                const uint32_t *dl = p.depth + (size_t)(l0 + g) * p.lay.depth_stride();
                 const double *mo = mom + (size_t)g * stride;
                 double xb[PG_MAX_SLOTS];
                 for (int a = 0; a < PG_MAX_SLOTS; a++) xb[a] = mo[a];
@@ -388,7 +381,7 @@
                     for (int a = 0; a < PG_MAX_SLOTS; a++) sxy[a] = 0.0;
                     for (int i = lane; i < n; i += 32) {
                         double F[PG_MAX_ALLELES];
-                        renorm_generic(p, fl, dl, i, kg, F);
+                        renorm_generic(p, l0 + g, i, kg, F);
                         const double dy = y[i] - ybar;
                         syy = fma(dy, dy, syy);
                         for (int a = 0; a < mg; a++) sxy[a] = fma(F[(cg >> (4 * a)) & 0xfu] - xb[a], dy, sxy[a]);
@@ -508,13 +501,11 @@
         unsigned kept = 0;
         for (int a = 0; a <= m; a++) kept |= 1u << col_of_code(p, (unsigned)((mv >> (16 + 8 * a)) & 0xffu));
         const int cj = col_of_code(p, (unsigned)((mv >> (16 + 8 * s)) & 0xffu));
-        const double *fl = p.freq + (size_t)locus * p.lay.freq_stride();
-        const uint32_t *dl = p.depth + (size_t)locus * p.lay.depth_stride();
         double fa[kGwMaxPools], qp[kGwMaxPools], pa[kGwMaxPools], pb[kGwMaxPools], pa0[kGwMaxPools], pb0[kGwMaxPools];
         double p_a = 0.0;
         for (int i = 0; i < n; i++) {
             double F[PG_MAX_ALLELES];
-            renorm_generic(p, fl, dl, i, kept, F);
+            renorm_generic(p, locus, i, kept, F);
             fa[i] = F[cj];
         }
         if (m == 1) {
diff --git a/poolgen_b200/csrc/pg_scan.cuh b/poolgen_b200/csrc/pg_scan.cuh
--- a/poolgen_b200/csrc/pg_scan.cuh
+++ b/poolgen_b200/csrc/pg_scan.cuh
@@ -4,6 +4,9 @@
 
 namespace pg {
 
+#ifndef PG_U16_UNROLL
+#define PG_U16_UNROLL 2
+#endif
 constexpr int kScanWarps = 12;
 constexpr int kRedPitch = 33;
 
@@ -117,38 +120,32 @@
 
 static __device__ __noinline__ double exact_q(const ScanParams &p, int64_t locus, int j, const double *ws, int lane) {
     const Layout &lay = p.lay;
-    const double *fl = p.freq + (size_t)locus * lay.freq_stride();
     double q = 0.0;
-    int i0 = 0;
-    for (int c = 0; c < lay.n_chunks; c++) {
-        const int rcc = (c == lay.n_chunks - 1) ? lay.rc_last : lay.rc;
-        const double *col = fl + (size_t)c * lay.A * lay.rc + (size_t)j * rcc;
-        const int rows = min(rcc, lay.n - i0);
-        for (int r0 = 0; r0 < rows; r0 += 32) {
-            const int r = r0 + lane;
-            double term = 0.0;
-            if (r < rows) {
-                const double f = col[r];
-                const double w = ws ? ws[i0 + r] : p.w_uniform;
-                term = (f != f) ? 0.0 : __dmul_rn(f, w);
-            }
-            const int m = min(32, rows - r0);
-            for (int t = 0; t < m; t++) q = __dadd_rn(q, __shfl_sync(PG_FULL_MASK, term, t));
-        }
-        i0 += rcc;
+    for (int r0 = 0; r0 < lay.n; r0 += 32) {
+        const int i = r0 + lane;
+        double term = 0.0;
+        if (i < lay.n) {
+            double f[PG_MAX_ALLELES], c[PG_MAX_ALLELES];
+            pool_row(lay, p.rows, p.depth, locus, i, f, c);
+            double fj = 0.0;
+#pragma unroll
+            for (int a = 0; a < PG_MAX_ALLELES; a++)
+                if (a == j) fj = f[a];
+            const double w = ws ? ws[i] : p.w_uniform;
+            term = (fj != fj) ? 0.0 : __dmul_rn(fj, w);
+        }
+        const int m = min(32, lay.n - r0);
+        for (int t = 0; t < m; t++) q = __dadd_rn(q, __shfl_sync(PG_FULL_MASK, term, t));
     }
     return q;
 }
 
 template <int A>
-__device__ __forceinline__ void renorm_row(const double (&f)[A], uint32_t d, unsigned kept, double (&F)[A]) {
-    double c[A];
+__device__ __forceinline__ void renorm_row(const double (&c)[A], unsigned kept, double (&F)[A]) {
     double dk = 0.0;
 #pragma unroll
-    for (int j = 0; j < A; j++) {
-        c[j] = (d == 0u) ? 0.0 : rint(f[j] * (double)d);
+    for (int j = 0; j < A; j++)
         if ((kept >> j) & 1u) dk += c[j];
-    }
 #pragma unroll
     for (int j = 0; j < A; j++) {
         if ((kept >> j) & 1u)
@@ -159,14 +156,11 @@
 }
 
 template <int A>
-__device__ __forceinline__ void renorm_row_fast(const double (&f)[A], uint32_t d, unsigned kept, double (&F)[A]) {
-    double c[A];
+__device__ __forceinline__ void renorm_row_fast(const double (&c)[A], unsigned kept, double (&F)[A]) {
     double dk = 0.0;
 #pragma unroll
-    for (int j = 0; j < A; j++) {
-        c[j] = (d == 0u) ? 0.0 : rint(f[j] * (double)d);
+    for (int j = 0; j < A; j++)
         if ((kept >> j) & 1u) dk += c[j];
-    }
     const double inv = (dk == 0.0) ? nan("") : 1.0 / dk;
 #pragma unroll
     for (int j = 0; j < A; j++) F[j] = ((kept >> j) & 1u) ? c[j] * inv : 0.0;
@@ -198,59 +192,35 @@
 
 template <int A>
 __device__ __noinline__ double exact_colsum(const ScanParams &p, int64_t locus, int jsel, unsigned kept) {
-    const Layout &lay = p.lay;
-    const double *fl = p.freq + (size_t)locus * lay.freq_stride();
-    const uint32_t *dl = p.depth + (size_t)locus * lay.depth_stride();
     double s = 0.0;
-    int i0 = 0;
-    for (int c = 0; c < lay.n_chunks; c++) {
-        const int rcc = (c == lay.n_chunks - 1) ? lay.rc_last : lay.rc;
-        const double *blk = fl + (size_t)c * lay.A * lay.rc;
-        const int rows = min(rcc, lay.n - i0);
-        for (int r = 0; r < rows; r++) {
-            double f[A], F[A];
-#pragma unroll
-            for (int j = 0; j < A; j++) f[j] = blk[(size_t)j * rcc + r];
-            renorm_row<A>(f, dl[i0 + r], kept, F);
-            double v = 0.0;
-#pragma unroll
-            for (int j = 0; j < A; j++)
-                if (j == jsel) v = F[j];
-            if (v == v) s = __dadd_rn(s, v);
-        }
-        i0 += rcc;
+    for (int i = 0; i < p.lay.n; i++) {
+        double f[A], c[A], F[A];
+        pool_row(p.lay, p.rows, p.depth, locus, i, f, c);
+        renorm_row<A>(c, kept, F);
+        double v = 0.0;
+#pragma unroll
+        for (int j = 0; j < A; j++)
+            if (j == jsel) v = F[j];
+        if (v == v) s = __dadd_rn(s, v);
     }
     return s;
 }
 
 template <int A, typename Fn>
 __device__ __forceinline__ void for_rows_coop(const ScanParams &p, int64_t locus, int lane, Fn &&fn) {
-    const Layout &lay = p.lay;
-    const double *fl = p.freq + (size_t)locus * lay.freq_stride();
-    const uint32_t *dl = p.depth + (size_t)locus * lay.depth_stride();
-    int i0 = 0;
-    for (int c = 0; c < lay.n_chunks; c++) {
-        const int rcc = (c == lay.n_chunks - 1) ? lay.rc_last : lay.rc;
-        const double *blk = fl + (size_t)c * lay.A * lay.rc;
-        const int rows = min(rcc, lay.n - i0);
-        for (int r0 = 0; r0 < rows; r0 += 128) {
-            double f[4][A];
-            uint32_t d[4];
-#pragma unroll
-            for (int i = 0; i < 4; i++) {
-                const int r = r0 + lane + 32 * i;
-                const bool ok = r < rows;
-#pragma unroll
-                for (int j = 0; j < A; j++) f[i][j] = ok ? blk[(size_t)j * rcc + r] : 0.0;
-                d[i] = ok ? dl[i0 + r] : 1u;
-            }
-#pragma unroll
-            for (int i = 0; i < 4; i++) {
-                const int r = r0 + lane + 32 * i;
-                if (r < rows) fn(i0 + r, f[i], d[i]);
-            }
-        }
-        i0 += rcc;
+    const int n = p.lay.n;
+    for (int r0 = 0; r0 < n; r0 += 128) {
+        double f[4][A], c[4][A];
+#pragma unroll
+        for (int i = 0; i < 4; i++) {
+            const int r = r0 + lane + 32 * i;
+            if (r < n) pool_row(p.lay, p.rows, p.depth, locus, r, f[i], c[i]);
+        }
+#pragma unroll
+        for (int i = 0; i < 4; i++) {
+            const int r = r0 + lane + 32 * i;
+            if (r < n) fn(r, f[i], c[i]);
+        }
     }
 }
 
@@ -259,7 +229,6 @@
                                        double *tot, int lane, bool decide, unsigned &kept_out) {
     using AC = Acc<A, K, W>;
     const Layout &lay = p.lay;
-    const uint32_t *dl = p.depth + (size_t)locus * lay.depth_stride();
     unsigned kept = kept_out;
     if (decide) {
         kept = 0;
@@ -270,7 +239,10 @@
         kept_out = kept;
         if (__popc(kept) < 2) return PG_LOCUS_FILTERED;
         int miss = 0;
-        for (int i = lane; i < lay.n; i += 32) miss += (dl[i] == 0u) ? 1 : 0;
+        for (int i = lane; i < lay.n; i += 32) {
+            double f[A], c[A];
+            miss += (pool_row(lay, p.rows, p.depth, locus, i, f, c) == 0u) ? 1 : 0;
+        }
         miss = __reduce_add_sync(PG_FULL_MASK, miss);
         if (miss == lay.n) return PG_LOCUS_FILTERED;
         if (((double)miss / (double)lay.n) > p.max_miss) return PG_LOCUS_FILTERED;
@@ -279,9 +251,9 @@
 #pragma unroll
     for (int i = 0; i < AC::N; i++) acc[i] = 0.0;
     const int n_pad = lay.n_pad;
-    for_rows_coop<A>(p, locus, lane, [&](int i, const double(&f)[A], uint32_t d) {
+    for_rows_coop<A>(p, locus, lane, [&](int i, const double(&)[A], const double(&c)[A]) {
         double F[A], y[K];
-        renorm_row_fast<A>(f, d, kept, F);
+        renorm_row_fast<A>(c, kept, F);
 #pragma unroll
         for (int k = 0; k < K; k++) y[k] = ys[k * n_pad + i];
         accum_row<A, K, W, true>(acc, F, y, 0.0);
@@ -372,9 +344,9 @@
         for (int a = 0; a < MS; a++) sx[a] = 0.0;
 #pragma unroll
         for (int k = 0; k < K; k++) sy[k] = 0.0;
-        for_rows_coop<A>(p, locus, lane, [&](int i, const double(&f)[A], uint32_t d) {
+        for_rows_coop<A>(p, locus, lane, [&](int i, const double(&)[A], const double(&c)[A]) {
             double F[A], x[MS];
-            renorm_row<A>(f, d, kept, F);
+            renorm_row<A>(c, kept, F);
             bool valid = true;
 #pragma unroll
             for (int a = 0; a < MS; a++) {
@@ -409,9 +381,9 @@
 #pragma unroll
             for (int a = 0; a < MS; a++) sxya[k][a] = 0.0;
         }
-        for_rows_coop<A>(p, locus, lane, [&](int i, const double(&f)[A], uint32_t d) {
+        for_rows_coop<A>(p, locus, lane, [&](int i, const double(&)[A], const double(&c)[A]) {
             double F[A], x[MS];
-            renorm_row<A>(f, d, kept, F);
+            renorm_row<A>(c, kept, F);
             bool valid = true;
 #pragma unroll
             for (int a = 0; a < MS; a++) {
@@ -472,9 +444,9 @@
         double ra[K];
 #pragma unroll
         for (int k = 0; k < K; k++) ra[k] = 0.0;
-        for_rows_coop<A>(p, locus, lane, [&](int i, const double(&f)[A], uint32_t d) {
+        for_rows_coop<A>(p, locus, lane, [&](int i, const double(&)[A], const double(&c)[A]) {
             double F[A], x[MS];
-            renorm_row<A>(f, d, kept, F);
+            renorm_row<A>(c, kept, F);
 #pragma unroll
             for (int a = 0; a < MS; a++) {
                 double v = 0.0;
@@ -523,9 +495,9 @@
 #pragma unroll
             for (int a = 0; a < MS; a++) sx[k][a] = 0.0;
         }
-        for_rows_coop<A>(p, locus, lane, [&](int i, const double(&f)[A], uint32_t d) {
+        for_rows_coop<A>(p, locus, lane, [&](int i, const double(&)[A], const double(&c)[A]) {
             double F[A], x[MS];
-            renorm_row<A>(f, d, kept, F);
+            renorm_row<A>(c, kept, F);
             bool xv = true;
 #pragma unroll
             for (int a = 0; a < MS; a++) {
@@ -562,9 +534,9 @@
 #pragma unroll
         for (int a = 0; a < MS; a++) sxx[k][a] = sxy[k][a] = 0.0;
     }
-    for_rows_coop<A>(p, locus, lane, [&](int i, const double(&f)[A], uint32_t d) {
+    for_rows_coop<A>(p, locus, lane, [&](int i, const double(&)[A], const double(&c)[A]) {
         double F[A], x[MS];
-        renorm_row<A>(f, d, kept, F);
+        renorm_row<A>(c, kept, F);
         bool xv = true;
 #pragma unroll
         for (int a = 0; a < MS; a++) {
@@ -614,9 +586,9 @@
     double xrow[PX];
 #pragma unroll
     for (int c = 0; c < PX; c++) xrow[c] = 0.0;
-    for_rows_coop<A>(p, locus, lane, [&](int i, const double(&f)[A], uint32_t d) {
+    for_rows_coop<A>(p, locus, lane, [&](int i, const double(&)[A], const double(&c)[A]) {
         double F[A];
-        renorm_row<A>(f, d, kept, F);
+        renorm_row<A>(c, kept, F);
         xrow[0] = 1.0;
 #pragma unroll
         for (int a = 0; a < MS; a++) {
@@ -1235,15 +1207,15 @@
 #pragma unroll
             for (int a = 0; a < AC::N; a++) acc[a] = 0.0;
             if (kept) {
-                for_rows_coop<A>(sp, locus, lane, [&](int r, const double(&f)[A], uint32_t d) {
+                for_rows_coop<A>(sp, locus, lane, [&](int r, const double(&)[A], const double(&c)[A]) {
                     double F[A], y[K];
-                    renorm_row_fast<A>(f, d, kept, F);
+                    renorm_row_fast<A>(c, kept, F);
 #pragma unroll
                     for (int k = 0; k < K; k++) y[k] = ys[k * n_pad + r];
                     accum_row<A, K, W, true>(acc, F, y, 0.0);
                 });
             } else {
-                for_rows_coop<A>(sp, locus, lane, [&](int r, const double(&f)[A], uint32_t) {
+                for_rows_coop<A>(sp, locus, lane, [&](int r, const double(&f)[A], const double(&)[A]) {
                     double y[K];
 #pragma unroll
                     for (int k = 0; k < K; k++) y[k] = ys[k * n_pad + r];
@@ -1266,11 +1238,44 @@
     }
 }
 
-template <int A, int K, bool W, int P, int KIND>
+__device__ __forceinline__ double2 rcp_depth(const double2 *tab, uint32_t d) {
+    if (d < (uint32_t)kRcpTab) return __ldg(tab + d);
+    const double dd = (double)d;
+    return make_double2(__drcp_rn(dd), dd);
+}
+template <int A, int FMT>
+__device__ __forceinline__ void stage_pair(const unsigned char *blk, int rcc, int r, int row, int n, const double2 *rtab,
+                                           double2 (&f2)[A]) {
+    if constexpr (FMT == FMT_F64) {
+        const double *fb = reinterpret_cast<const double *>(blk);
+#pragma unroll
+        for (int j = 0; j < A; j++) f2[j] = *reinterpret_cast<const double2 *>(fb + (size_t)j * rcc + r);
+    } else {
+        const uint16_t *cb = reinterpret_cast<const uint16_t *>(blk);
+        uint32_t v[A], dx = 0, dy = 0;
+#pragma unroll
+        for (int j = 0; j < A; j++) {
+            v[j] = *reinterpret_cast<const uint32_t *>(cb + (size_t)j * rcc + r);
+            dx += v[j] & 0xFFFFu;
+            dy += v[j] >> 16;
+        }
+        if (row >= n) dx = 1u;
+        if (row + 1 >= n) dy = 1u;
+        const double2 rx = rcp_depth(rtab, dx), ry = rcp_depth(rtab, dy);
+#pragma unroll
+        for (int j = 0; j < A; j++)
+            f2[j] = make_double2(count_quotient_nz((double)(v[j] & 0xFFFFu), rx.y, rx.x),
+                                 count_quotient_nz((double)(v[j] >> 16), ry.y, ry.x));
+    }
+}
+
+template <int A, int K, bool W, int P, int KIND, int FMT>
 __global__ void __launch_bounds__(kScanWarps * 32, 1) scan_kernel(const __grid_constant__ ScanParams p) {
     using AC = Acc<A, K, W>;
     constexpr int LPS = 32 / P;
-    constexpr int RC = chunk_rows(A);
+    constexpr int RC = chunk_rows(A, FMT);
+    constexpr int EB = (FMT == FMT_U16) ? 2 : 8;
+    constexpr int UNROLL = (FMT == FMT_U16) ? PG_U16_UNROLL : RC / 64;
     extern __shared__ __align__(128) unsigned char smem[];
     __shared__ __align__(16) ScanParams sp_storage;
     for (int i = threadIdx.x; i < (int)(sizeof(ScanParams) / 4); i += blockDim.x)
@@ -1305,11 +1310,12 @@
     if (gw >= NB) return;
     const int n_chunks = lay.n_chunks;
     const size_t fstride = lay.freq_stride();
-    const uint32_t full_bytes = (uint32_t)(A * lay.rc * 8), last_bytes = (uint32_t)(A * lay.rc_last * 8);
-    const uint32_t locus_bytes = (uint32_t)(fstride * 8);
+    const uint32_t full_bytes = (uint32_t)(A * lay.rc * EB), last_bytes = (uint32_t)(A * lay.rc_last * EB);
+    const uint32_t locus_bytes = (uint32_t)(fstride * EB);
+    const unsigned char *rows = static_cast<const unsigned char *>(p.rows);
 
     int64_t i_blk = gw;
-    const unsigned char *i_src = reinterpret_cast<const unsigned char *>(p.freq + (size_t)(gw * G) * fstride);
+    const unsigned char *i_src = rows + (size_t)(gw * G) * locus_bytes;
     int i_left = (int)min((int64_t)G, L - gw * G);
     int i_chunk = 0;
     bool i_done = false;
@@ -1342,7 +1348,7 @@
             if (i_blk >= NB) {
                 i_done = true;
             } else {
-                i_src = reinterpret_cast<const unsigned char *>(p.freq + (size_t)(i_blk * G) * fstride);
+                i_src = rows + (size_t)(i_blk * G) * locus_bytes;
                 i_left = (int)min((int64_t)G, L - i_blk * G);
             }
         }
@@ -1376,14 +1382,13 @@
                     const double *yrow = ys + chunk * RC + 2 * lane;
                     const double *wrow = W ? ws + chunk * RC + 2 * lane : nullptr;
                     mbar_wait(&bars[buf], parity);
-                    double *fb = reinterpret_cast<double *>(stage0 + (size_t)buf * p.stage_bytes);
+                    unsigned char *sb = stage0 + (size_t)buf * p.stage_bytes;
+                    double *fb = reinterpret_cast<double *>(sb);
                     if (chunk < n_chunks - 1 || lay.rc_last == RC) {
-                        const double *fl = fb + 2 * lane;
-#pragma unroll
+#pragma unroll UNROLL
                         for (int it = 0; it < RC / 64; it++) {
                             double2 f2[A], y2[K];
-#pragma unroll
-                            for (int j = 0; j < A; j++) f2[j] = *reinterpret_cast<const double2 *>(fl + j * RC + it * 64);
+                            stage_pair<A, FMT>(sb, RC, it * 64 + 2 * lane, chunk * RC + it * 64 + 2 * lane, lay.n, p.rcp_tab, f2);
 #pragma unroll
                             for (int k = 0; k < K; k++)
                                 y2[k] = *reinterpret_cast<const double2 *>(yrow + (size_t)k * n_pad + it * 64);
@@ -1396,8 +1401,7 @@
                         const int rcc = lay.rc_last;
                         for (int r = 2 * lane; r < rcc; r += 64) {
                             double2 f2[A], y2[K];
-#pragma unroll
-                            for (int j = 0; j < A; j++) f2[j] = *reinterpret_cast<const double2 *>(fb + (size_t)j * rcc + r);
+                            stage_pair<A, FMT>(sb, rcc, r, chunk * RC + r, lay.n, p.rcp_tab, f2);
 #pragma unroll
                             for (int k = 0; k < K; k++)
                                 y2[k] = *reinterpret_cast<const double2 *>(ys + chunk * RC + (size_t)k * n_pad + r);
@@ -1429,15 +1433,13 @@
                 const unsigned hkept = hk & 0x3fu;
                 mbar_wait(&bars[buf], parity);
                 double *fb = reinterpret_cast<double *>(stage0 + (size_t)buf * p.stage_bytes);
-                const double *fl = fb + (size_t)u * fstride;
+                const unsigned char *fl = stage0 + (size_t)buf * p.stage_bytes + (size_t)u * locus_bytes;
                 if (__any_sync(PG_FULL_MASK, hinted)) {
                     if (s * LPS + u < cnt) {
 #pragma unroll 1
                         for (int r = 2 * q0; r < n_pad; r += 2 * P) {
                             double2 f2[A], y2[K];
-#pragma unroll
-                            for (int j = 0; j < A; j++)
-                                f2[j] = *reinterpret_cast<const double2 *>(fl + (size_t)j * n_pad + r);
+                            stage_pair<A, FMT>(fl, n_pad, r, r, lay.n, p.rcp_tab, f2);
 #pragma unroll
                             for (int k = 0; k < K; k++)
                                 y2[k] = *reinterpret_cast<const double2 *>(ys + (size_t)k * n_pad + r);
@@ -1451,8 +1453,7 @@
 #pragma unroll 2
                     for (int r = 2 * q0; r < n_pad; r += 2 * P) {
                         double2 f2[A], y2[K];
-#pragma unroll
-                        for (int j = 0; j < A; j++) f2[j] = *reinterpret_cast<const double2 *>(fl + (size_t)j * n_pad + r);
+                        stage_pair<A, FMT>(fl, n_pad, r, r, lay.n, p.rcp_tab, f2);
 #pragma unroll
                         for (int k = 0; k < K; k++) y2[k] = *reinterpret_cast<const double2 *>(ys + (size_t)k * n_pad + r);
                         double2 w2 = make_double2(0.0, 0.0);
@@ -1473,14 +1474,15 @@
     }
 }
 
-template <int A, int K, bool W, int P>
+template <int A, int K, bool W, int P, int FMT>
 cudaError_t launch_scan_p(ScanParams p, int sm_count, cudaStream_t s) {
     using AC = Acc<A, K, W>;
     const Layout &lay = p.lay;
+    const size_t eb = (size_t)lay.elem_bytes();
     const size_t avail = 227 * 1024 - 512;
     size_t common = (size_t)(K + (W ? 1 : 0)) * lay.n_pad * 8;
     common = (common + 127) / 128 * 128;
-    size_t stage = (P == 32) ? (size_t)A * lay.rc * 8 : (size_t)(32 / P) * lay.freq_stride() * 8;
+    size_t stage = (P == 32) ? (size_t)A * lay.rc * eb : (size_t)(32 / P) * lay.freq_stride() * 8;
     stage = (stage + 127) / 128 * 128;
     if (stage < (size_t)kRedPitch * 8) stage = ((size_t)kRedPitch * 8 + 127) / 128 * 128;
     int G = 32, nbuf = 3, nwarps = 0;
@@ -1524,7 +1526,7 @@
     p.nbuf = nbuf;
     p.block_loci = G;
     const size_t smem = common + (size_t)nwarps * wbytes;
-    auto kern = (p.kind == PG_KIND_OLS) ? scan_kernel<A, K, W, P, PG_KIND_OLS> : scan_kernel<A, K, W, P, PG_KIND_CORR>;
+    auto kern = (p.kind == PG_KIND_OLS) ? scan_kernel<A, K, W, P, PG_KIND_OLS, FMT> : scan_kernel<A, K, W, P, PG_KIND_CORR, FMT>;
     cudaError_t e = cudaFuncSetAttribute(kern, cudaFuncAttributeMaxDynamicSharedMemorySize, (int)smem);
     if (e != cudaSuccess) return e;
     const int64_t NB = (p.n_loci + G - 1) / G;
@@ -1544,14 +1546,19 @@
     return cudaGetLastError();
 }
 
+template <int A, int K, bool W, int FMT>
+cudaError_t launch_scan_f(const ScanParams &p, int sm_count, cudaStream_t s) {
+    if (several_loci_per_stage(p.lay)) {
+        const int P = p.p_override ? p.p_override : (p.lay.n_pad > 64 ? 16 : 8);
+        if (P == 16) return launch_scan_p<A, K, W, 16, FMT>(p, sm_count, s);
+        return launch_scan_p<A, K, W, 8, FMT>(p, sm_count, s);
+    }
+    return launch_scan_p<A, K, W, 32, FMT>(p, sm_count, s);
+}
 template <int A, int K, bool W>
 cudaError_t launch_scan_t(const ScanParams &p, int sm_count, cudaStream_t s) {
-    if (p.lay.n_chunks == 1) {
-        const int P = p.p_override ? p.p_override : (p.lay.n_pad > 64 ? 16 : 8);
-        if (P == 16) return launch_scan_p<A, K, W, 16>(p, sm_count, s);
-        return launch_scan_p<A, K, W, 8>(p, sm_count, s);
-    }
-    return launch_scan_p<A, K, W, 32>(p, sm_count, s);
+    return (p.lay.fmt == FMT_U16) ? launch_scan_f<A, K, W, FMT_U16>(p, sm_count, s)
+                                  : launch_scan_f<A, K, W, FMT_F64>(p, sm_count, s);
 }
 
 template <int A>
diff --git a/poolgen_b200/csrc/pg_text.cu b/poolgen_b200/csrc/pg_text.cu
--- a/poolgen_b200/csrc/pg_text.cu
+++ b/poolgen_b200/csrc/pg_text.cu
@@ -186,6 +186,7 @@
         }
         const uint32_t end_rank = (l + 1 < n_lines) ? p.first_sep[l + 1] : (uint32_t)(p.tok_blk[p.n_tok_blocks] >> 32);
         uint32_t *out = p.counts + (size_t)ord * 6 * n;
+        uint32_t vmax = 0;
         for (int i = lane; i < n; i += 32) {
             if (first + 3 + i >= end_rank) break;
             uint32_t a = p.sep[first + 2 + i] + 1, b = p.sep[first + 3 + i];
@@ -197,7 +198,11 @@
                 const char c = (q < b) ? p.text[q] : ':';
                 if (c == ':') {
                     if (!digits) bad = true;
-                    if (j < 6) out[(size_t)j * n + i] = v > 0xFFFFFFFFull ? 0xFFFFFFFFu : (uint32_t)v;
+                    if (j < 6) {
+                        const uint32_t cv = v > 0xFFFFFFFFull ? 0xFFFFFFFFu : (uint32_t)v;
+                        out[(size_t)j * n + i] = cv;
+                        vmax = max(vmax, cv);
+                    }
                     j++;
                     v = 0;
                     digits = false;
@@ -214,6 +219,8 @@
             }
             if (bad || j < 6) text_error(p, TEXT_ERR_FIELD, a);
         }
+        vmax = __reduce_max_sync(PG_FULL_MASK, vmax);
+        if (lane == 0 && vmax) atomicMax(p.info + 4, vmax);
     }
 }
 
@@ -233,12 +240,12 @@
                                       int64_t max_loci, size_t line_cap, int sm_count, cudaStream_t s) {
     t->max_loci = max_loci;
     if (!t->parsed) TCK(cudaEventCreateWithFlags(&t->parsed, cudaEventDisableTiming));
-    TCK(t->d_info.reserve(4, s));
-    TCK(t->h_info.reserve(4, s));
-    TCK(cudaMemsetAsync(t->d_info.get(), 0, 16, s));
+    TCK(t->d_info.reserve(5, s));
+    TCK(t->h_info.reserve(5, s));
+    TCK(cudaMemsetAsync(t->d_info.get(), 0, 20, s));
     if (n_bytes >= 0xFFFFFFF0ull) return cudaErrorInvalidValue;
     if (n_bytes == 0) {
-        TCK(cudaMemcpyAsync(t->h_info.get(), t->d_info.get(), 16, cudaMemcpyDeviceToHost, s));
+        TCK(cudaMemcpyAsync(t->h_info.get(), t->d_info.get(), 20, cudaMemcpyDeviceToHost, s));
         return cudaEventRecord(t->parsed, s);
     }
     const bool add_nl = text[n_bytes - 1] != '\n';
@@ -301,7 +308,7 @@
     const int grid_parse = (int)std::min<uint64_t>(((uint64_t)line_cap * 32 + 255) / 256, (uint64_t)sm_count * 8);
     text_parse_kernel<<<grid_parse, 256, 0, s>>>(tp);
     TCK(cudaGetLastError());
-    TCK(cudaMemcpyAsync(t->h_info.get(), t->d_info.get(), 16, cudaMemcpyDeviceToHost, s));
+    TCK(cudaMemcpyAsync(t->h_info.get(), t->d_info.get(), 20, cudaMemcpyDeviceToHost, s));
     return cudaEventRecord(t->parsed, s);
 }
 #undef TCK
```
